# coveord/k8s-spot-rescheduler

Measured on AMD Instinct MI355X. Metric: reference-equivalent pod x spot-node feasibility checks/s (drain-plan latency: drain_plan_latency_ms), higher is better.
Workload: dtype int64

## Files before the change

### k8s-spot-rescheduler_amd/csrc/kernels.hip

```cpp
#include <algorithm>
#include <climits>

#include "kernels.hpp"

#include <hip/hip_ext.h>

namespace sr {
namespace {

__device__ __forceinline__ uint64_t ballot(bool p) { return __builtin_amdgcn_ballot_w64(p); }

__device__ __forceinline__ uint64_t readlane64(uint64_t v, int lane) {
  const uint32_t lo = static_cast<uint32_t>(__builtin_amdgcn_readlane(static_cast<int>(v & 0xffffffffu), lane));
  const uint32_t hi = static_cast<uint32_t>(__builtin_amdgcn_readlane(static_cast<int>(v >> 32), lane));
  return (static_cast<uint64_t>(hi) << 32) | lo;
}

template <int CTRL, int ROW_MASK = 0xf>
__device__ __forceinline__ int dpp_min(int v) {
  return min(v, __builtin_amdgcn_update_dpp(INT_MAX, v, CTRL, ROW_MASK, 0xf, false));
}
__device__ __forceinline__ int wave_min(int v) {
  v = dpp_min<0x111>(v);
  v = dpp_min<0x112>(v);
// ... 77 lines not shown
    if (has) acc &= any | cur;
    if (wv) w.S[static_cast<size_t>(cls) * Wp + word] = acc;
  }
}

__device__ __forceinline__ void k0_common(const DevWorkload& w, int local_first_fallback, int wave, int lane) {
  if (blockIdx.x == 0 && wave == 0 && w.n_node_patch > 0 && lane < 11) {
    for (int p = 0; p < w.n_node_patch; ++p) {
      const uint64_t* pr = w.node_patch + static_cast<size_t>(p) * kNodePatchU64;
      const size_t node = static_cast<size_t>(pr[0]);
      if (lane < 8) const_cast<uint64_t*>(w.node_rec)[node * 8 + lane] = pr[1 + lane];
      else const_cast<int64_t*>(w.node_free)[static_cast<size_t>(lane - 8) * w.n_pad + node] =
          static_cast<int64_t>(pr[1 + lane]);
    }
  }
  for (int i = static_cast<int>(blockIdx.x * blockDim.x + threadIdx.x); i < w.n_pod_patch;
       i += static_cast<int>(gridDim.x * blockDim.x)) {
    const uint64_t* pp = w.pod_patch + static_cast<size_t>(i) * kPodPatchU64;
    uint64_t* rec = const_cast<uint64_t*>(w.pod_rec) + static_cast<size_t>(pp[0]) * 6;
    rec[4] = pp[1];
    rec[5] = pp[2];
  }
  if (blockIdx.x == 0 && threadIdx.x == 0) {
    unsigned long long* dm = reinterpret_cast<unsigned long long*>(w.d_min);
    dm[0] = ~0ull;
    dm[1] = local_first_fallback < 0 ? ~0ull : static_cast<unsigned long long>(local_first_fallback) << 32;
    dm[2] = w.rank_next;
  }
}

__device__ __forceinline__ int64_t free_of(const DevWorkload& w, int d, int n) {
  int64_t v = w.node_free[static_cast<size_t>(d - 1) * w.n_pad + n];
  for (int p = 0; p < w.n_node_patch; ++p) {
    const uint64_t* pr = w.node_patch + static_cast<size_t>(p) * kNodePatchU64;
    if (static_cast<uint64_t>(n) == pr[0]) v = static_cast<int64_t>(pr[8 + d]);
  }
  return v;
}

__global__ __launch_bounds__(256) void k0_tables(DevWorkload w, int s_blocks, int local_first_fallback) {
  const int lane = threadIdx.x & 63;
  const int wave = __builtin_amdgcn_readfirstlane(static_cast<int>(threadIdx.x >> 6));
  const size_t pw = static_cast<size_t>(blockIdx.x) * 4 + wave;
  uint64_t* const prof = w.prof && pw < kK0ProfWaves ? w.prof + static_cast<size_t>(w.n_cand) * 16 + 2 * pw : nullptr;
  if (prof && lane == 0)
    prof[0] = __builtin_amdgcn_s_memrealtime() | (static_cast<int>(blockIdx.x) < s_blocks ? 1ull << 63 : 0ull);
  struct Stamp {
    uint64_t* p;
    int lane;
    __device__ ~Stamp() {
      if (p && lane == 0) p[1] = __builtin_amdgcn_s_memrealtime();
    }
  } stamp{prof, lane};
  k0_common(w, local_first_fallback, wave, lane);
  const size_t Wp = static_cast<size_t>(w.Wp);
  if (static_cast<int>(blockIdx.x) < s_blocks) {
    const int c0 = __builtin_amdgcn_readfirstlane((static_cast<int>(blockIdx.x) * 4 + wave) * kSClasses);
    int op[kSClasses][8];
#pragma unroll
    for (int q = 0; q < kSClasses; ++q) {
      const int cls = c0 + q;
      if (cls < w.n_classes) {
        const int4* p8 = reinterpret_cast<const int4*>(w.cls_prog8 + static_cast<size_t>(cls) * 8);
        const int4 a = p8[0], b = p8[1];
        op[q][0] = a.x; op[q][1] = a.y; op[q][2] = a.z; op[q][3] = a.w;
        op[q][4] = b.x; op[q][5] = b.y; op[q][6] = b.z; op[q][7] = b.w;
      } else {
        op[q][0] = -3;
#pragma unroll
        for (int u = 1; u < 8; ++u) op[q][u] = -1;
      }
    }
    const int s_words = w.s_head_only ? min(w.Wp, kSHead) : w.Wp;
    for (int wb = 0; wb < s_words; wb += 128) {
      const bool two = wb + 64 < s_words;
      uint64_t v[2][kSClasses][8];
#pragma unroll
      for (int h = 0; h < 2; ++h) {
        if (h == 1 && !two) break;
        const int word = wb + 64 * h + lane;
        const size_t wi = word < s_words ? static_cast<size_t>(word) : 0;
#pragma unroll
        for (int q = 0; q < kSClasses; ++q)
#pragma unroll
          for (int u = 0; u < 8; ++u)
            v[h][q][u] = op[q][u] >= 0 ? w.atoms[static_cast<size_t>(op[q][u] >> 2) * Wp + wi] : 0;
      }
#pragma unroll
      for (int h = 0; h < 2; ++h) {
        if (h == 1 && !two) break;
        const int word = wb + 64 * h + lane;
        const bool wv = word < s_words;
#pragma unroll
        for (int q = 0; q < kSClasses; ++q) {
          if (op[q][0] < 0 && op[q][0] != -1) continue;
          const uint64_t acc = eval_prog8(op[q], v[h][q]);
          if (wv) w.S[static_cast<size_t>(c0 + q) * Wp + word] = acc;
        }
      }
    }
#pragma unroll
    for (int q = 0; q < kSClasses; ++q)
      if (op[q][0] == -2) s_row_general(w, c0 + q, lane);
    return;
  }
  int tw = (static_cast<int>(blockIdx.x) - s_blocks) * 4 + wave;
  const int wgroups = (w.Wp + kTWords - 1) / kTWords;
  int d = 0;
  for (; d < 4; ++d) {
    const int waves_d = (w.t_off[d + 1] - w.t_off[d] + 63) / 64 * wgroups;
    if (tw < waves_d) break;
    tw -= waves_d;
  }
  if (d == 4) return;
  const int g = tw / wgroups;
  const int W0 = (tw - g * wgroups) * kTWords;
  const int r0 = w.t_off[d] + 64 * g;
  const int nr = min(64, w.t_off[d + 1] - r0);
  const int64_t thr = lane < nr ? w.t_thr[r0 + lane] : INT64_MAX;
#pragma unroll
  for (int ww = 0; ww < kTWords; ++ww) {
    const int W = W0 + ww;
    if (W >= w.Wp) break;
    uint64_t word;
    if (d == 0) {
      const int nvalid = max(0, min(64, w.n_spot - 64 * W));
      word = nvalid >= 64 ? ~0ull : (1ull << nvalid) - 1;
    } else {
      const uint64_t fv = static_cast<uint64_t>(free_of(w, d, 64 * W + lane));
      uint32_t lo = 0, hi = 0;
#pragma unroll
      for (int i = 0; i < 32; ++i) lo |= static_cast<uint32_t>(static_cast<int64_t>(readlane64(fv, i)) >= thr) << i;
#pragma unroll
      for (int i = 0; i < 32; ++i)
        hi |= static_cast<uint32_t>(static_cast<int64_t>(readlane64(fv, 32 + i)) >= thr) << i;
      word = static_cast<uint64_t>(hi) << 32 | lo;
    }
    if (lane < nr && thr != kTPad) w.T[static_cast<size_t>(r0 + lane) * Wp + W] = word;
  }
}


__global__ __launch_bounds__(256) void k0_incremental(DevWorkload w, int s_waves, int t_waves,
                                                      int local_first_fallback) {
  const int lane = threadIdx.x & 63;
  const int wave = __builtin_amdgcn_readfirstlane(static_cast<int>(threadIdx.x >> 6));
  k0_common(w, local_first_fallback, wave, lane);
  const int wv = static_cast<int>(blockIdx.x) * 4 + wave;
  const size_t Wp = static_cast<size_t>(w.Wp);
  if (wv < s_waves) {
    const int cls = wv * 64 + lane;
    if (cls >= w.n_classes) return;
    const int s_words = w.s_head_only ? min(w.Wp, kSHead) : w.Wp;
    const int4* p8 = reinterpret_cast<const int4*>(w.cls_prog8 + static_cast<size_t>(cls) * 8);
    const int4 a = p8[0], b = p8[1];
    const int op[8] = {a.x, a.y, a.z, a.w, b.x, b.y, b.z, b.w};
    for (int c = 0; c < w.n_k0_cols; ++c) {
      const int W = w.k0_cols[c];
      if (W >= s_words) continue;
      uint64_t acc;
      if (op[0] == -2) {
        acc = ~0ull;
        uint64_t any = 0, cur = 0;
        bool has = false;
        for (int o = w.cls_prog_off[cls]; o < w.cls_prog_off[cls + 1]; ++o) {
          const int x = w.cls_prog[o];
          const uint64_t v = w.atoms[static_cast<size_t>(x >> 2) * Wp + W];
          switch (x & 3) {
            case PROG_AND: acc &= v; break;
            case PROG_ANDNOT: acc &= ~v; break;
            case PROG_TERM_START:
              any |= has ? cur : 0;
              cur = v;
              has = true;
              break;
            default: cur &= v; break;
          }
        }
        if (has) acc &= any | cur;
      } else {
        uint64_t v[8];
#pragma unroll
        for (int u = 0; u < 8; ++u) v[u] = op[u] >= 0 ? w.atoms[static_cast<size_t>(op[u] >> 2) * Wp + W] : 0;
        acc = eval_prog8(op, v);
      }
      w.S[static_cast<size_t>(cls) * Wp + W] = acc;
    }
    return;
  }
  int tw = wv - s_waves;
  if (tw < t_waves) {
    int d = 1;
    for (; d < 4; ++d) {
      const int waves_d = (w.t_off[d + 1] - w.t_off[d] + 63) / 64;
      if (tw < waves_d) break;
      tw -= waves_d;
    }
    if (d == 4) return;
    const int r0 = w.t_off[d] + 64 * tw;
    const int nr = min(64, w.t_off[d + 1] - r0);
    const int64_t thr = lane < nr ? w.t_thr[r0 + lane] : INT64_MAX;
    for (int c = 0; c < w.n_k0_cols; ++c) {
      const int W = w.k0_cols[c];
      const uint64_t fv = static_cast<uint64_t>(free_of(w, d, 64 * W + lane));
      uint32_t lo = 0, hi = 0;
#pragma unroll
      for (int i = 0; i < 32; ++i) lo |= static_cast<uint32_t>(static_cast<int64_t>(readlane64(fv, i)) >= thr) << i;
#pragma unroll
      for (int i = 0; i < 32; ++i)
        hi |= static_cast<uint32_t>(static_cast<int64_t>(readlane64(fv, 32 + i)) >= thr) << i;
      if (lane < nr && thr != kTPad) w.T[static_cast<size_t>(r0 + lane) * Wp + W] = static_cast<uint64_t>(hi) << 32 | lo;
    }
    return;
  }
  const int mr = tw - t_waves;
  if (mr >= w.n_k0_rows) return;
  const int row = w.k0_rows[mr];
  const int d = row < w.t_off[2] ? 1 : row < w.t_off[3] ? 2 : 3;
  const int64_t thr = w.t_thr[row];
  for (int W = lane; W < w.Wp; W += 64) {
    uint64_t word = 0;
    for (int i = 0; i < 64; ++i) word |= static_cast<uint64_t>(free_of(w, d, 64 * W + i) >= thr) << i;
    w.T[static_cast<size_t>(row) * Wp + W] = word;
  }
}


typedef __attribute__((address_space(3))) void* lds_vp;
typedef __attribute__((address_space(1))) void* gbl_vp;
#define SR_WAIT_VM(n) asm volatile("s_waitcnt vmcnt(" #n ")" ::: "memory")

__device__ __forceinline__ void write_winner(const DevWorkload& w) {
  const int lane = threadIdx.x & 63;
  const unsigned long long* dm = reinterpret_cast<const unsigned long long*>(w.d_min);
  const unsigned long long ok = __hip_atomic_load(dm, __ATOMIC_RELAXED, __HIP_MEMORY_SCOPE_AGENT);
  const unsigned long long fb = __hip_atomic_load(dm + 1, __ATOMIC_RELAXED, __HIP_MEMORY_SCOPE_AGENT);
  const unsigned long long nx = __hip_atomic_load(dm + 2, __ATOMIC_RELAXED, __HIP_MEMORY_SCOPE_AGENT);
  uint64_t* r = w.result;
  const bool any = ok != ~0ull;
  const int g = any ? static_cast<int>(ok >> 32) : -1;
  const int li = any ? static_cast<int>(ok & 0xffffffffu) : -1;
  const bool local = any && li < w.n_cand && w.cand_global[li] == g;
  const int off = local ? w.cand_off[li] : 0;
  const int np = local ? w.cand_off[li + 1] - off : 0;
  const uint64_t tag = static_cast<uint64_t>(static_cast<uint32_t>(w.seq)) << 32;
  auto put = [&](int i, int v) {
    __hip_atomic_store(r + i, tag | static_cast<uint32_t>(v), __ATOMIC_RELAXED, __HIP_MEMORY_SCOPE_SYSTEM);
  };
  for (int q = lane; q < np; q += 64)
    put(kResultHeader + q, __hip_atomic_load(w.out_node + off + q, __ATOMIC_RELAXED, __HIP_MEMORY_SCOPE_AGENT));
  if (lane == 0) put(0, g);
  if (lane == 1) put(1, local ? 1 : 0);
  if (lane == 2) put(2, np);
  if (lane == 3) put(3, fb == ~0ull ? -1 : static_cast<int>(fb >> 32));
  if (lane == 4) put(4, nx == ~0ull ? -1 : static_cast<int>(nx));
}

__global__ __launch_bounds__(64) void k3_winner(DevWorkload w) { write_winner(w); }

__global__ __launch_bounds__(256) void k3_sequence(SeqRound r) {
  const unsigned long long ok = __hip_atomic_load(reinterpret_cast<const unsigned long long*>(r.d_min),
                                                  __ATOMIC_RELAXED, __HIP_MEMORY_SCOPE_AGENT);
  const int win = ok == ~0ull ? INT_MAX : static_cast<int>(ok >> 32);
  const int end = win < r.fb_stop ? win : r.fb_stop - 1;
  for (int ci = static_cast<int>(blockIdx.x * blockDim.x + threadIdx.x); ci < r.n_cand;
       ci += static_cast<int>(gridDim.x * blockDim.x)) {
    const int g = r.cand_global[ci];
    if (g <= r.floor || g > end) continue;
    r.seq_status[g] = r.out_status[ci];
    const int o = r.cand_off[ci], np = r.cand_off[ci + 1] - o;
    const int dst = r.in_off[g] - r.in_off[0];
    for (int k = 0; k < np; ++k) r.seq_node[dst + k] = r.out_node[o + k];
  }
}

__device__ __forceinline__ uint64_t swap_pairs(uint64_t x, uint64_t m) {
  const uint64_t y = x & m, e = 0x5555555555555555ull;
  return (x & ~m) | ((y & e) << 1) | ((y >> 1) & e);
}

constexpr int kHead = 32;
constexpr int kRing = 8;
constexpr int kPodWin = 128;
constexpr int kRecU64 = 6;
constexpr int kNodeCache = 16;
constexpr int kMaxPods = 512;

struct K2Lds {
  uint64_t ring[kRing][4 * kHead];
  uint64_t chunk[256];
  uint64_t pods[kPodWin][kRecU64];
  uint64_t cache[kNodeCache][8];
  uint64_t spec[8];
  uint64_t rec[8];
  int32_t omap[kMaxPods];
};

constexpr int kMapG = 4;

struct K2Stats {
  uint32_t n_spec_miss = 0, n_min = 0, n_far = 0;
  uint64_t cyc_a = 0, cyc_b = 0, cyc_c = 0, cyc_d = 0;
  uint64_t cyc_rec = 0;
  uint32_t narrow = 0;
  uint64_t cyc_res = 0;
  uint64_t cyc_win = 0;
  uint32_t cyc_a_ld = 0, cyc_res_ld = 0, n_res = 0, n_res_pods = 0;
};

template <int SPL, int CH, bool PROF, bool EXT = false>
__device__ __forceinline__ int k2_run(const DevWorkload& w, K2Lds& L, const int p0, const int np, int& status,
                                      K2Stats& st, uint32_t& nbytes, const int ebase = -1) {
  const int lane = threadIdx.x & 63;
  const int Wp = w.Wp;
  const uint64_t* __restrict__ tab = w.S;

  auto dma = [&](const uint64_t* src, uint64_t* dst) {
    __builtin_amdgcn_global_load_lds((gbl_vp)src, (lds_vp)dst, 16, 0, 0);
  };
  auto dma_rows = [&](uint64_t* dst, uint64_t r01, uint64_t r23, int base) {
    const uint32_t wi = static_cast<uint32_t>(min(base + 2 * (lane & 31), Wp - 2));
    const uint32_t ra = lane < 32 ? static_cast<uint32_t>(r01) : static_cast<uint32_t>(r01 >> 32);
    const uint32_t rb = lane < 32 ? static_cast<uint32_t>(r23) : static_cast<uint32_t>(r23 >> 32);
    dma(tab + (static_cast<uint64_t>(ra) + wi), dst);
    dma(tab + (static_cast<uint64_t>(rb) + wi), dst + 128);
  };
  auto dma_rows_of = [&](uint64_t* dst, int q, int base) {
    const uint64_t* pr = L.pods[q & (kPodWin - 1)];
    dma_rows(dst, pr[4], pr[5], base);
  };
  auto dma_head = [&](uint64_t* dst, uint64_t r01, uint64_t r23) {
    const int r = lane >> 4;
    const uint32_t wi = static_cast<uint32_t>(min(2 * (lane & 15), Wp - 2));
    const uint64_t rr = r < 2 ? r01 : r23;
    const uint32_t off = (r & 1) ? static_cast<uint32_t>(rr >> 32) : static_cast<uint32_t>(rr);
    dma(tab + (static_cast<uint64_t>(off) + wi), dst);
  };
  auto dma_head_of = [&](uint64_t* dst, int q) {
    const uint64_t* pr = L.pods[q & (kPodWin - 1)];
    dma_head(dst, pr[4], pr[5]);
  };
  auto dma_rec = [&](uint64_t* dst, int node) {
    if (lane < 4) dma(w.node_rec + static_cast<size_t>(node == INT_MAX ? 0 : node) * 8 + 2 * lane, dst);
  };
  auto dma_pods = [&](int m) {
    const uint64_t* src = w.pod_rec + static_cast<size_t>(p0 + 64 * m) * kRecU64 + 2 * lane;
    uint64_t* dst = L.pods[64 * (m & 1)];
#pragma unroll
    for (int j = 0; j < 3; ++j) dma(src + 128 * j, dst + 128 * j);
  };

  uint64_t touched[CH];
#pragma unroll
  for (int ch = 0; ch < CH; ++ch) touched[ch] = 0;
  int snode[SPL];
  int64_t scpu[SPL], smem[SPL], seph[SPL];
  int sleft[SPL];
  uint64_t sport[SPL];
  int64_t ss0[SPL], ss1[SPL];
#pragma unroll
  for (int s = 0; s < SPL; ++s) {
    snode[s] = INT_MAX;
    scpu[s] = smem[s] = seph[s] = 0;
    sleft[s] = 0;
    sport[s] = 0;
    ss0[s] = ss1[s] = 0;
  }
  const uint64_t erow = EXT ? w.pod_ext[static_cast<size_t>(ebase) * kDevExtU64 + 7] : ~0ull;
  const int erow0 = static_cast<int32_t>(static_cast<uint32_t>(erow)), erow1 = static_cast<int32_t>(erow >> 32);
  int nslots = 0;
  uint64_t cyc_t = 0;
  auto cyc = [&]() -> uint64_t { return PROF ? __builtin_amdgcn_s_memtime() : 0ull; };
  const uint64_t lane_mask = lane < min(Wp, kHead) ? ~0ull : 0ull;

  uint64_t word_next = 0;
  int cnode0 = INT_MAX;
  int64_t nrc = 0, nrm = 0, nre = 0;
  uint64_t npm = 0;
  int64_t nac = 0, nam = 0, nae = 0, nsr0 = INT64_MIN, nsr1 = INT64_MIN, nsa0 = 0, nsa1 = 0;
  bool sbit[SPL];
  auto gather_next = [&](int kn) {
    if (EXT) {
      const uint64_t* er = w.pod_ext + static_cast<size_t>(ebase + kn) * kDevExtU64;
      nac = static_cast<int64_t>(er[0]);
      nam = static_cast<int64_t>(er[1]);
      nae = static_cast<int64_t>(er[2]);
      nsr0 = static_cast<int64_t>(er[3]);
      nsr1 = static_cast<int64_t>(er[4]);
      nsa0 = static_cast<int64_t>(er[5]);
      nsa1 = static_cast<int64_t>(er[6]);
    }
    const uint64_t* img = L.ring[kn & (kRing - 1)];
    const uint64_t* pr = L.pods[kn & (kPodWin - 1)];
    uint64_t sw[SPL];
#pragma unroll
    for (int s = 0; s < SPL; ++s) sw[s] = img[snode[s] < 64 * kHead ? snode[s] >> 6 : 0];
    const int hl = lane & (kHead - 1);
    const uint64_t a = img[hl] & img[kHead + hl] & img[2 * kHead + hl] & img[3 * kHead + hl];
    nrc = static_cast<int64_t>(pr[0]);
    nrm = static_cast<int64_t>(pr[1]);
    nre = static_cast<int64_t>(pr[2]);
    npm = pr[3];
#pragma unroll
    for (int s = 0; s < SPL; ++s) sbit[s] = (sw[s] >> (snode[s] & 63)) & 1ull;
    word_next = a & lane_mask;
    const uint64_t clean0 = word_next & ~touched[0];
    const uint64_t mc0 = ballot(clean0 != 0);
    cnode0 = INT_MAX;
    if (mc0) {
      const int L0 = __builtin_ctzll(mc0);
      cnode0 = L0 * 64 + __builtin_ctzll(readlane64(clean0, L0));
    }
  };

  static_assert(kRing == 8, "the vmcnt immediates below assume an 8-deep ring");
  dma(w.node_rec + 2 * lane, L.cache[0]);
  dma_pods(0);
  if (np > 64) dma_pods(1);
  nbytes += 64u * kNodeCache + (48u + 4u) * static_cast<uint32_t>(np) + 4u;
  SR_WAIT_VM(0);
#pragma unroll
  for (int j = 0; j < kRing - 1; ++j) dma_head_of(L.ring[j], min(j, np - 1));
  SR_WAIT_VM(6);
  gather_next(0);
  dma_rec(L.spec, cnode0);
  dma_head_of(L.ring[kRing - 1], min(kRing - 1, np - 1));

  status = -1;
  int k = 0;
  for (; k < np; ++k) {
    if (PROF) cyc_t = cyc();
    nbytes += 4u * kHead * 8u + 64u + (EXT ? 64u : 0u);
    const int64_t rc = nrc, rm = nrm, re = nre;
    const int64_t ac = EXT ? nac : rc, am = EXT ? nam : rm, ae = EXT ? nae : re;
    const int64_t sr0 = nsr0, sr1 = nsr1, sa0 = nsa0, sa1 = nsa1;
    const uint64_t pm = npm;
    const uint64_t pin = swap_pairs(pm, w.swap_mask);
    const bool zero = (rc | rm | re) == 0;
    int ans;
    {
      const int hi = min(cnode0, 64 * kHead);
      int best = INT_MAX;
#pragma unroll
      for (int s = 0; s < SPL; ++s) {
        const int nd = snode[s];
        const bool fit = (zero | ((rc <= scpu[s]) & (rm <= smem[s]) & (re <= seph[s]))) &
                         (!EXT | ((sr0 <= ss0[s]) & (sr1 <= ss1[s])));
        const bool ok = (nd < hi) & sbit[s] & (sleft[s] >= 1) & ((sport[s] & pin) == 0) & fit;
        best = ok ? min(best, nd) : best;
      }
      const uint64_t hb = ballot(best != INT_MAX);
      int dnode = INT_MAX;
      if (hb) {
        dnode = (hb & (hb - 1)) ? wave_min(best) : __builtin_amdgcn_readlane(best, __builtin_ctzll(hb));
        if (PROF && (hb & (hb - 1))) ++st.n_min;
      }
      ans = min(cnode0, dnode);
    }
    if (ans == INT_MAX && Wp > kHead) {
#pragma unroll
      for (int ch = 0; ch < CH; ++ch) {
        const int base = ch * 64;
        if (ans != INT_MAX || base >= Wp) continue;
        if (PROF) ++st.n_far;
        nbytes += 4u * 64u * 8u;
        dma_rows_of(L.chunk, k, base);
        SR_WAIT_VM(0);
        const uint64_t* img = L.chunk;
        const uint64_t clean = (img[lane] & img[64 + lane] & img[128 + lane] & img[192 + lane]) &
                               ((base + lane < Wp) ? ~touched[ch] : 0ull);
        const uint64_t mc = ballot(clean != 0);
        int cnode = INT_MAX;
        if (mc) {
          const int L0 = __builtin_ctzll(mc);
          cnode = (base + L0) * 64 + __builtin_ctzll(readlane64(clean, L0));
        }
        const int lo = base * 64;
        const int hi = min(cnode, lo + 64 * 64);
        int best = INT_MAX;
#pragma unroll
        for (int s = 0; s < SPL; ++s) {
          const int nd = snode[s];
          const bool in = (nd >= lo) & (nd < hi);
          const uint64_t sw = img[in ? (nd >> 6) - base : 0];
          const bool fit = (zero | ((rc <= scpu[s]) & (rm <= smem[s]) & (re <= seph[s]))) &
                           (!EXT | ((sr0 <= ss0[s]) & (sr1 <= ss1[s])));
          const bool ok =
              in & (((sw >> (nd & 63)) & 1ull) != 0) & (sleft[s] >= 1) & ((sport[s] & pin) == 0) & fit;
          best = ok ? min(best, nd) : best;
        }
        ans = min(cnode, wave_min(best));
      }
    }
    if (PROF) {
      const uint64_t t = cyc();
      st.cyc_a += t - cyc_t;
      cyc_t = t;
    }
    if (ans == INT_MAX) {
      status = k;
      break;
    }
    if (lane == 0) L.omap[k] = ans;

    bool hit = false;
#pragma unroll
    for (int s = 0; s < SPL; ++s) {
      if (snode[s] == ans) {
        scpu[s] -= ac;
        smem[s] -= am;
        seph[s] -= ae;
        sleft[s] -= 1;
        sport[s] |= pm;
        if (EXT) {
          ss0[s] -= sa0;
          ss1[s] -= sa1;
        }
        hit = true;
      }
    }
    if (!(ballot(hit) != 0)) {
      const int ns = nslots++;
      if (ns >= 64 * SPL) {
        SR_WAIT_VM(0);
        return -1;
      }
      const int64_t b0 = EXT && erow0 >= 0 ? w.node_scal[static_cast<size_t>(erow0) * w.n_pad + ans] : 0;
      const int64_t b1 = EXT && erow1 >= 0 ? w.node_scal[static_cast<size_t>(erow1) * w.n_pad + ans] : 0;
      const uint64_t* rec;
      if (ans < kNodeCache) {
        rec = L.cache[ans];
      } else if (ans == cnode0) {
        SR_WAIT_VM(1);
        rec = L.spec;
      } else {
        if (PROF) ++st.n_spec_miss;
        nbytes += 64u;
        dma_rec(L.rec, ans);
        SR_WAIT_VM(0);
        rec = L.rec;
      }
      const int64_t fc = static_cast<int64_t>(rec[0]), fm = static_cast<int64_t>(rec[1]),
                    fe = static_cast<int64_t>(rec[2]);
      const uint64_t pb = rec[3];
      const int pl = static_cast<int>(static_cast<int64_t>(rec[4]));
#pragma unroll
      for (int s = 0; s < SPL; ++s) {
        if ((s == (ns >> 6)) & (lane == (ns & 63))) {
          snode[s] = ans;
          scpu[s] = fc - ac;
          smem[s] = fm - am;
          seph[s] = fe - ae;
          sleft[s] = pl - 1;
          sport[s] = pb | pm;
          if (EXT) {
            ss0[s] = b0 - sa0;
            ss1[s] = b1 - sa1;
          }
        }
      }
      const int tw = ans >> 6;
#pragma unroll
      for (int ch = 0; ch < CH; ++ch)
        if (tw == ch * 64 + lane) touched[ch] |= 1ull << (ans & 63);
    }
    if (PROF) {
      const uint64_t t = cyc();
      st.cyc_b += t - cyc_t;
      cyc_t = t;
    }
    if (k + 1 < np) {
      const int q = min(k + kRing, np - 1);
      const bool restage = q == k + kRing && (q & 63) == 0 && q >= kPodWin;
      if (restage) {
        dma_pods(q >> 6);
        SR_WAIT_VM(0);
      } else if (k >= 5) {
        SR_WAIT_VM(12);
      } else {
        SR_WAIT_VM(7);
      }
      if (PROF) {
        const uint64_t t = cyc();
        st.cyc_c += t - cyc_t;
        cyc_t = t;
      }
      const uint64_t* pq = L.pods[q & (kPodWin - 1)];
      const uint64_t r01 = pq[4], r23 = pq[5];
      gather_next(k + 1);
      dma_rec(L.spec, cnode0);
      dma_head(L.ring[k & (kRing - 1)], r01, r23);
      if (PROF) st.cyc_d += cyc() - cyc_t;
    }
  }
  SR_WAIT_VM(0);
  return status >= 0 ? status : np;
}

constexpr int kNH = 8;
static_assert(kNH == 2 || kNH == 4 || kNH == 8, "head words per pod: a power of two up to 8 (8-bit head masks)");
constexpr int kNHS = kNH + 1;
constexpr int kFar = 64 * kNH;

__device__ __forceinline__ uint64_t f_word_far(const uint64_t* __restrict__ tab, uint64_t r01, uint64_t r23, int wd) {
  return tab[static_cast<uint32_t>(r01) + wd] & tab[static_cast<uint32_t>(r01 >> 32) + wd] &
         tab[static_cast<uint32_t>(r23) + wd] & tab[static_cast<uint32_t>(r23 >> 32) + wd];
}

__device__ __forceinline__ uint64_t f_word_prog_s(const DevWorkload& w, const int32_t* pg, int wd) {
  int op[8];
  uint64_t v[8];
#pragma unroll
  for (int u = 0; u < 8; ++u) op[u] = pg[u];
#pragma unroll
  for (int u = 0; u < 8; ++u) v[u] = op[u] >= 0 ? w.atoms[static_cast<size_t>(op[u] >> 2) * w.Wp + wd] : 0ull;
  return eval_prog8(op, v);
}

__device__ __forceinline__ uint64_t f_word_prog(const DevWorkload& w, const uint64_t* __restrict__ tab,
                                                const int32_t* pg, uint64_t r01, uint64_t r23, int wd) {
  int op[8];
  uint64_t v[8];
#pragma unroll
  for (int u = 0; u < 8; ++u) op[u] = pg[u];
#pragma unroll
  for (int u = 0; u < 8; ++u) v[u] = op[u] >= 0 ? w.atoms[static_cast<size_t>(op[u] >> 2) * w.Wp + wd] : 0ull;
  return eval_prog8(op, v) & tab[static_cast<uint32_t>(r01 >> 32) + wd] & tab[static_cast<uint32_t>(r23) + wd] &
         tab[static_cast<uint32_t>(r23 >> 32) + wd];
}

__device__ __forceinline__ uint64_t fix_dirty(const DevWorkload& w, uint64_t f, uint64_t s, int wd, int64_t rc,
                                              int64_t rm, int64_t re, bool zero) {
  for (int p = 0; p < w.n_dirty; ++p) {
    const int n = w.dirty_node[p];
    if ((n >> 6) != wd) continue;
    const uint64_t bit = 1ull << (n & 63);
    const bool fits = zero || (w.dirty_free[p][0] >= rc && w.dirty_free[p][1] >= rm && w.dirty_free[p][2] >= re);
    f = fits ? (f | (s & bit)) : (f & ~bit);
  }
  return f;
}

__device__ __forceinline__ void window_patch(const DevWorkload& w, int W, int lane, int64_t& ncpu, int64_t& nmem,
                                             int64_t& neph, uint64_t& nport, int& nleft) {
  for (int p = 0; p < w.n_node_patch; ++p) {
    const uint64_t* pr = w.node_patch + static_cast<size_t>(p) * kNodePatchU64;
    if (static_cast<int>(pr[0]) != 64 * W + lane) continue;
    ncpu = static_cast<int64_t>(pr[1]);
    nmem = static_cast<int64_t>(pr[2]);
    neph = static_cast<int64_t>(pr[3]);
    nport = pr[4];
    nleft = static_cast<int>(static_cast<int64_t>(pr[5]));
  }
}

__device__ __forceinline__ uint32_t from_lane(uint32_t v, int src) {
  return static_cast<uint32_t>(__builtin_amdgcn_ds_bpermute(src << 2, static_cast<int>(v)));
}

#pragma clang diagnostic push
#pragma clang diagnostic ignored "-Winline-asm"
__device__ __forceinline__ int writelane(int v, int x, int k) {
  asm("s_mov_b32 m0, %2\n\tv_writelane_b32 %0, %1, m0" : "+v"(v) : "s"(x), "s"(k) : "m0");
  return v;
}
#pragma clang diagnostic pop
__device__ __forceinline__ int ff1(uint64_t x) {
  int r;
  asm("s_ff1_i32_b64 %0, %1" : "=s"(r) : "s"(x));
  return r;
}
__device__ __forceinline__ uint64_t bitclear(uint64_t x, int k) {
  asm("s_bitset0_b64 %0, %1" : "+s"(x) : "s"(k));
  return x;
}

template <bool E, bool O>
__device__ __forceinline__ uint64_t place_window(uint64_t todo, int kmax, int W, int lane, int64_t rc, int64_t rm,
                                                 int64_t re, uint64_t pm, uint64_t cur, uint64_t zm,
                                                 uint64_t swap_mask, uint64_t emask, int64_t& ncpu, int64_t& nmem,
                                                 int64_t& neph, uint64_t& nport, int& nleft, int& node) {
  int jv = 64;
  if (kmax < 64) todo &= kmax <= 0 ? 0ull : (1ull << kmax) - 1;
  while (todo != 0) {
    const int k = __builtin_ctzll(todo);
    todo = bitclear(todo, k);
    const int64_t c = static_cast<int64_t>(readlane64(static_cast<uint64_t>(rc), k));
    const int64_t m = static_cast<int64_t>(readlane64(static_cast<uint64_t>(rm), k));
    const int64_t e = E ? static_cast<int64_t>(readlane64(static_cast<uint64_t>(re), k)) : 0;
    const uint64_t q = O ? readlane64(pm, k) : 0ull;
    uint64_t fit = readlane64(cur, k) & ballot(nleft >= 1);
    const uint64_t res = ballot(ncpu >= c) & ballot(nmem >= m) & (E ? ballot(neph >= e) : emask);
    fit &= ((zm >> k) & 1) ? ~0ull : res;
    if (O) fit &= ballot((nport & q) == 0);
    if (O) {
      if (fit != 0) {
        const int j = __builtin_ctzll(fit);
        if (lane == j) {
          ncpu -= c;
          nmem -= m;
          if (E) neph -= e;
          nleft -= 1;
          nport |= swap_pairs(q, swap_mask);
        }
        jv = writelane(jv, j, k);
      }
      continue;
    }
    const int j = ff1(fit);
    const bool hit = lane == j;
    ncpu -= hit ? c : 0;
    nmem -= hit ? m : 0;
    if (E) neph -= hit ? e : 0;
    nleft -= hit ? 1 : 0;
    jv = writelane(jv, j, k);
  }
  const bool took = static_cast<unsigned>(jv) < 64u;
  node = took ? 64 * W + jv : node;
  return ballot(took);
}

template <typename T>
struct XVals {
  T ac, am, ae, r0, r1, a0, a1;
};

template <bool E, bool O>
__device__ __forceinline__ uint64_t place_window_x(uint64_t todo, int kmax, int W, int lane, int64_t rc, int64_t rm,
                                                   int64_t re, const XVals<int64_t>& x, uint64_t pm, uint64_t cur,
                                                   uint64_t zm, uint64_t swap_mask, uint64_t emask, int64_t& ncpu,
                                                   int64_t& nmem, int64_t& neph, uint64_t& nport, int& nleft,
                                                   int64_t& ns0, int64_t& ns1, int& node) {
  int jv = 64;
  if (kmax < 64) todo &= kmax <= 0 ? 0ull : (1ull << kmax) - 1;
  while (todo != 0) {
    const int k = __builtin_ctzll(todo);
    todo = bitclear(todo, k);
    const int64_t c = static_cast<int64_t>(readlane64(static_cast<uint64_t>(rc), k));
    const int64_t m = static_cast<int64_t>(readlane64(static_cast<uint64_t>(rm), k));
    const int64_t e = E ? static_cast<int64_t>(readlane64(static_cast<uint64_t>(re), k)) : 0;
    const int64_t r0 = static_cast<int64_t>(readlane64(static_cast<uint64_t>(x.r0), k));
    const int64_t r1 = static_cast<int64_t>(readlane64(static_cast<uint64_t>(x.r1), k));
    const uint64_t q = O ? readlane64(pm, k) : 0ull;
    uint64_t fit = readlane64(cur, k) & ballot(nleft >= 1) & ballot(ns0 >= r0) & ballot(ns1 >= r1);
    const uint64_t res = ballot(ncpu >= c) & ballot(nmem >= m) & (E ? ballot(neph >= e) : emask);
    fit &= ((zm >> k) & 1) ? ~0ull : res;
    if (O) fit &= ballot((nport & q) == 0);
    if (fit != 0) {
      const int j = __builtin_ctzll(fit);
      const int64_t ac = static_cast<int64_t>(readlane64(static_cast<uint64_t>(x.ac), k));
      const int64_t am = static_cast<int64_t>(readlane64(static_cast<uint64_t>(x.am), k));
      const int64_t ae = static_cast<int64_t>(readlane64(static_cast<uint64_t>(x.ae), k));
      const int64_t a0 = static_cast<int64_t>(readlane64(static_cast<uint64_t>(x.a0), k));
      const int64_t a1 = static_cast<int64_t>(readlane64(static_cast<uint64_t>(x.a1), k));
      if (lane == j) {
        ncpu -= ac;
        nmem -= am;
        neph -= ae;
        nleft -= 1;
        ns0 -= a0;
        ns1 -= a1;
        if (O) nport |= swap_pairs(q, swap_mask);
      }
      jv = writelane(jv, j, k);
    }
  }
  const bool took = static_cast<unsigned>(jv) < 64u;
  node = took ? 64 * W + jv : node;
  return ballot(took);
}

__device__ __forceinline__ int32_t scale32(int64_t f, int k) {
  const int64_t q = f >> k;
  return f < 0 ? -1 : (q > 0x7fffffffll ? 0x7fffffff : static_cast<int32_t>(q));
}

template <bool E, bool O>
__device__ __forceinline__ uint64_t fits32(int32_t c32, int32_t m32, int32_t e32, int nleft, uint64_t conflict,
                                           int32_t c, int32_t m, int32_t e) {
  int32_t t = __builtin_elementwise_sub_sat(c32, c) | __builtin_elementwise_sub_sat(m32, m) | (nleft - 1);
  if (E) t |= __builtin_elementwise_sub_sat(e32, e);
  if (O) {
    const uint32_t x = static_cast<uint32_t>(conflict) | static_cast<uint32_t>(conflict >> 32);
    t |= static_cast<int32_t>(x | (0u - x));
  }
  return ballot(t >= 0);
}

template <bool E, bool O, bool X = false>
__device__ __forceinline__ uint64_t place_window32(uint64_t todo, int kmax, int W, int lane, uint32_t nc, uint32_t nm,
                                                   uint32_t ne, uint64_t pm, uint64_t ps, uint64_t cur,
                                                   int32_t& c32, int32_t& m32, int32_t& e32,
                                                   uint64_t& nport, int& nleft, int& node) {
  if constexpr (X) {
    int jv = 64;
    if (kmax < 64) todo &= kmax <= 0 ? 0ull : (1ull << kmax) - 1;
    const uint64_t base = ballot(nleft >= 1);
    uint64_t taken = 0;
    while (todo != 0) {
      const int k = __builtin_ctzll(todo);
      todo = bitclear(todo, k);
      const int32_t c = __builtin_amdgcn_readlane(static_cast<int>(nc), k);
      const int32_t m = __builtin_amdgcn_readlane(static_cast<int>(nm), k);
      const int32_t e = E ? __builtin_amdgcn_readlane(static_cast<int>(ne), k) : 0;
      const uint64_t q = readlane64(pm, k);
      uint64_t fit = readlane64(cur, k) & base & ~taken & fits32<E, true>(c32, m32, e32, 1, nport & q, c, m, e);
      const int j = fit != 0 ? __builtin_ctzll(fit) : 64;
      taken |= fit & (0ull - fit);
      jv = writelane(jv, j, k);
    }
    const int dst = jv < 64 ? jv : (taken == ~0ull ? lane : __builtin_ctzll(~taken));
    const bool snd = jv < 64;
    auto send = [&](uint32_t v) {
      return static_cast<uint32_t>(__builtin_amdgcn_ds_permute(dst << 2, static_cast<int>(snd ? v : 0u)));
    };
    const uint32_t rc = send(static_cast<uint32_t>(max(static_cast<int32_t>(nc), 0)));
    const uint32_t rm = send(static_cast<uint32_t>(max(static_cast<int32_t>(nm), 0)));
    const uint32_t re = E ? send(static_cast<uint32_t>(max(static_cast<int32_t>(ne), 0))) : 0u;
    const uint32_t rs_lo = send(static_cast<uint32_t>(ps)), rs_hi = send(static_cast<uint32_t>(ps >> 32));
    const bool got = (taken >> lane) & 1;
    c32 -= got ? static_cast<int32_t>(rc) : 0;
    m32 -= got ? static_cast<int32_t>(rm) : 0;
    if (E) e32 -= got ? static_cast<int32_t>(re) : 0;
    nleft -= got ? 1 : 0;
    nport |= got ? (static_cast<uint64_t>(rs_hi) << 32 | rs_lo) : 0ull;
    node = jv < 64 ? 64 * W + jv : node;
    return ballot(jv < 64);
  }
  int jv = 64;
  if (kmax < 64) todo &= kmax <= 0 ? 0ull : (1ull << kmax) - 1;
  while (todo != 0) {
    const int k = __builtin_ctzll(todo);
    todo = bitclear(todo, k);
    const int32_t c = __builtin_amdgcn_readlane(static_cast<int>(nc), k);
    const int32_t m = __builtin_amdgcn_readlane(static_cast<int>(nm), k);
    const int32_t e = E ? __builtin_amdgcn_readlane(static_cast<int>(ne), k) : 0;
    const uint64_t q = O ? readlane64(pm, k) : 0ull;
    uint64_t fit = readlane64(cur, k) & fits32<E, O>(c32, m32, e32, nleft, nport & q, c, m, e);
    const int32_t cu = max(c, 0), mu = max(m, 0), eu = max(e, 0);
    if (O) {
      if (fit != 0) {
        const int j = __builtin_ctzll(fit);
        if (lane == j) {
          c32 -= cu;
          m32 -= mu;
          if (E) e32 -= eu;
          nleft -= 1;
          nport |= readlane64(ps, k);
        }
        jv = writelane(jv, j, k);
      }
      continue;
    }
    const int j = ff1(fit);
    const bool hit = lane == j;
    c32 -= hit ? cu : 0;
    m32 -= hit ? mu : 0;
    if (E) e32 -= hit ? eu : 0;
    nleft -= hit ? 1 : 0;
    jv = writelane(jv, j, k);
  }
  const bool took = static_cast<unsigned>(jv) < 64u;
  node = took ? 64 * W + jv : node;
  return ballot(took);
}

template <bool E, bool O>
__device__ __forceinline__ uint64_t place_window32_x(uint64_t todo, int kmax, int W, int lane, uint32_t nc, uint32_t nm,
                                                     uint32_t ne, const XVals<uint32_t>& x, uint64_t pm, uint64_t ps,
                                                     uint64_t cur, int32_t& c32, int32_t& m32, int32_t& e32,
                                                     int32_t& s0, int32_t& s1, uint64_t& nport, int& nleft,
                                                     int& node) {
  int jv = 64;
  if (kmax < 64) todo &= kmax <= 0 ? 0ull : (1ull << kmax) - 1;
  while (todo != 0) {
    const int k = __builtin_ctzll(todo);
    todo = bitclear(todo, k);
    const int32_t c = __builtin_amdgcn_readlane(static_cast<int>(nc), k);
    const int32_t m = __builtin_amdgcn_readlane(static_cast<int>(nm), k);
    const int32_t e = E ? __builtin_amdgcn_readlane(static_cast<int>(ne), k) : 0;
    const int32_t r0 = __builtin_amdgcn_readlane(static_cast<int>(x.r0), k);
    const int32_t r1 = __builtin_amdgcn_readlane(static_cast<int>(x.r1), k);
    const uint64_t q = O ? readlane64(pm, k) : 0ull;
    int32_t t = __builtin_elementwise_sub_sat(c32, c) | __builtin_elementwise_sub_sat(m32, m) | (nleft - 1) |
                __builtin_elementwise_sub_sat(s0, r0) | __builtin_elementwise_sub_sat(s1, r1);
    if (E) t |= __builtin_elementwise_sub_sat(e32, e);
    if (O) {
      const uint64_t cf = nport & q;
      const uint32_t u = static_cast<uint32_t>(cf) | static_cast<uint32_t>(cf >> 32);
      t |= static_cast<int32_t>(u | (0u - u));
    }
    const uint64_t fit = readlane64(cur, k) & ballot(t >= 0);
    if (fit != 0) {
      const int j = __builtin_ctzll(fit);
      const int32_t ac = __builtin_amdgcn_readlane(static_cast<int>(x.ac), k);
      const int32_t am = __builtin_amdgcn_readlane(static_cast<int>(x.am), k);
      const int32_t ae = __builtin_amdgcn_readlane(static_cast<int>(x.ae), k);
      const int32_t a0 = __builtin_amdgcn_readlane(static_cast<int>(x.a0), k);
      const int32_t a1 = __builtin_amdgcn_readlane(static_cast<int>(x.a1), k);
      if (lane == j) {
        c32 -= ac;
        m32 -= am;
        e32 -= ae;
        s0 -= a0;
        s1 -= a1;
        nleft -= 1;
        if (O) nport |= readlane64(ps, k);
      }
      jv = writelane(jv, j, k);
    }
  }
  const bool took = static_cast<unsigned>(jv) < 64u;
  node = took ? 64 * W + jv : node;
  return ballot(took);
}

struct Narrow {
  int kc, km, ke;
};

constexpr int kCoopWaves = 4;
constexpr int kCoopPods = 64;
struct CoopArea {
  int32_t cmd, n, sw, pad;
  uint64_t r01[kCoopPods], r23[kCoopPods];
  int64_t rq[kCoopPods][3];
  int32_t op[kCoopPods][8];
  uint32_t best[kCoopPods];
  uint32_t rk[kCoopWaves][kCoopPods];
  uint64_t rm[kCoopWaves][kCoopPods];
  uint64_t rf[kCoopWaves][kCoopPods];
};

template <bool HO>
__device__ __forceinline__ void coop_scan(const DevWorkload& w, CoopArea& A, int h) {
  const int lane = threadIdx.x & 63;
  const int n = __builtin_amdgcn_readfirstlane(A.n), sw = __builtin_amdgcn_readfirstlane(A.sw);
  const int Wp = w.Wp;
  const uint64_t* __restrict__ tab = w.S;
  if (lane < n) A.rk[h][lane] = 0xffffffffu;
  const int cb0 = (sw >> 6) << 6;
  const int nch = (Wp - cb0 + 63) >> 6;
  const uint64_t all = n >= 64 ? ~0ull : (1ull << n) - 1;
  uint64_t found = 0;
  constexpr int Q = HO ? 2 : 4;
  for (int k = h; k < nch; k += kCoopWaves) {
    const int cb = cb0 + 64 * k;
    const int word = cb + lane;
    const bool wv = word >= sw && word < Wp;
    const uint32_t wi = wv ? static_cast<uint32_t>(word) : 0u;
    const uint64_t vw = ballot(wv);
    uint64_t open = all & ~found & ballot(lane < n && __hip_atomic_load(&A.best[lane], __ATOMIC_RELAXED,
                                                                           __HIP_MEMORY_SCOPE_WORKGROUP) >
                                                        static_cast<uint32_t>(k));
    while (open != 0) {
      int js[Q];
      uint64_t a01[Q], a23[Q];
      int op[Q][8];
#pragma unroll
      for (int q = 0; q < Q; ++q) {
        js[q] = open != 0 ? __builtin_ctzll(open) : -1;
        open &= open - 1;
        const int j = js[q] < 0 ? 0 : js[q];
        a01[q] = readlane64(A.r01[j], 0);
        a23[q] = readlane64(A.r23[j], 0);
        if constexpr (HO) {
#pragma unroll
          for (int u = 0; u < 8; ++u) op[q][u] = __builtin_amdgcn_readfirstlane(A.op[j][u]);
        }
      }
      uint64_t x[Q][HO ? 11 : 4];
#pragma unroll
      for (int q = 0; q < Q; ++q) {
        if (js[q] < 0) continue;
        if constexpr (HO) {
#pragma unroll
          for (int u = 0; u < 8; ++u)
            x[q][u] = op[q][u] >= 0 ? w.atoms[static_cast<size_t>(op[q][u] >> 2) * Wp + wi] : 0ull;
          x[q][8] = tab[static_cast<uint32_t>(a01[q] >> 32) + wi];
          x[q][9] = tab[static_cast<uint32_t>(a23[q]) + wi];
          x[q][10] = tab[static_cast<uint32_t>(a23[q] >> 32) + wi];
        } else {
          x[q][0] = tab[static_cast<uint32_t>(a01[q]) + wi];
          x[q][1] = tab[static_cast<uint32_t>(a01[q] >> 32) + wi];
          x[q][2] = tab[static_cast<uint32_t>(a23[q]) + wi];
          x[q][3] = tab[static_cast<uint32_t>(a23[q] >> 32) + wi];
        }
      }
#pragma unroll
      for (int q = 0; q < Q; ++q) {
        if (js[q] < 0) continue;
        const int j = js[q];
        uint64_t f, sw0;
        if constexpr (HO) {
          uint64_t v8[8];
#pragma unroll
          for (int u = 0; u < 8; ++u) v8[u] = x[q][u];
          sw0 = eval_prog8(op[q], v8);
          f = sw0 & x[q][8] & x[q][9] & x[q][10];
        } else {
          sw0 = x[q][0];
          f = x[q][0] & x[q][1] & x[q][2] & x[q][3];
        }
        if (w.k0_skip) {
          const int64_t rc = A.rq[j][0], rm = A.rq[j][1], re = A.rq[j][2];
          f = fix_dirty(w, f, sw0, word, rc, rm, re, (rc | rm | re) == 0);
        }
        const uint64_t m = ballot(wv && f != 0) & vw;
        if (m == 0) continue;
        found |= 1ull << j;
        if (lane == 0) {
          A.rk[h][j] = static_cast<uint32_t>(k);
          A.rm[h][j] = m;
          atomicMin(&A.best[j], static_cast<uint32_t>(k));
        }
        const uint64_t fw = readlane64(f, __builtin_ctzll(m));
        if (lane == 0) A.rf[h][j] = fw;
      }
    }
  }
}

__device__ __forceinline__ void coop_helper(const DevWorkload& w, CoopArea& A, int h) {
  for (;;) {
    __syncthreads();
    if (__hip_atomic_load(&A.cmd, __ATOMIC_RELAXED, __HIP_MEMORY_SCOPE_WORKGROUP) != 0) break;
    if (w.s_head_only) coop_scan<true>(w, A, h);
    else coop_scan<false>(w, A, h);
    __syncthreads();
  }
}

__device__ __forceinline__ int wave_sum(int v) {
  v += __builtin_amdgcn_update_dpp(0, v, 0x111, 0xf, 0xf, false);
  v += __builtin_amdgcn_update_dpp(0, v, 0x112, 0xf, 0xf, false);
  v += __builtin_amdgcn_update_dpp(0, v, 0x114, 0xf, 0xf, false);
  v += __builtin_amdgcn_update_dpp(0, v, 0x118, 0xf, 0xf, false);
  v += __builtin_amdgcn_update_dpp(0, v, 0x142, 0xa, 0xf, false);
  v += __builtin_amdgcn_update_dpp(0, v, 0x143, 0xc, 0xf, false);
  return __builtin_amdgcn_readlane(v, 63);
}

template <int G, bool PROF, bool WIDE = false, bool XT = false, bool COOP = false>
__device__ __forceinline__ void k2_node_order(const DevWorkload& w, uint64_t* __restrict__ F, const int p0,
                                              const int np, int& status, K2Stats& st, uint32_t& nbytes,
                                              int (&mapv)[kMapG], const int ebase = -1, const int erow0_in = -2,
                                              const int erow1_in = -2, CoopArea* A = nullptr) {
  static_assert(64 * G * kNHS * 8 <= sizeof(K2Lds), "node-order LDS exceeds the wave's K2 region");
  static_assert(G <= kMapG, "a mapping register per pod group");
  const int lane = threadIdx.x & 63;
  const int Wp = w.Wp;
  const uint64_t* __restrict__ tab = w.S;
  int64_t rc[G], rm[G], re[G];
  uint64_t pm[G], ps[G], r01[G], r23[G], fmask[G], act[G];
  int fbase[G];
  bool unres[G];
  uint64_t cur[G];
  uint32_t hmask[G];
  bool zero[G];
  int ptr[G], node[G];
  int dead = np;
#pragma unroll
  for (int g = 0; g < G; ++g) {
    const uint64_t* pr = w.pod_rec + static_cast<size_t>(p0 + min(64 * g + lane, np - 1)) * kRecU64;
    rc[g] = static_cast<int64_t>(pr[0]);
    rm[g] = static_cast<int64_t>(pr[1]);
    re[g] = static_cast<int64_t>(pr[2]);
    pm[g] = swap_pairs(pr[3], w.swap_mask);
    ps[g] = pr[3];
    r01[g] = pr[4];
    r23[g] = pr[5];
    zero[g] = (rc[g] | rm[g] | re[g]) == 0;
    fmask[g] = 0;
    fbase[g] = 0;
    unres[g] = false;
    hmask[g] = 0;
    cur[g] = 0;
    ptr[g] = INT_MAX;
    node[g] = -1;
    const uint64_t e = ballot(64 * g + lane < np && static_cast<uint32_t>(r01[g]) == w.s_empty_off);
    if (e != 0) dead = min(dead, 64 * g + __builtin_ctzll(e));
  }
  XVals<int64_t> xv[G];
  int erow0 = -1, erow1 = -1;
  if constexpr (XT) {
#pragma unroll
    for (int g = 0; g < G; ++g) {
      const uint64_t* er = w.pod_ext + static_cast<size_t>(ebase + min(64 * g + lane, np - 1)) * kDevExtU64;
      xv[g] = {static_cast<int64_t>(er[0]), static_cast<int64_t>(er[1]), static_cast<int64_t>(er[2]),
               static_cast<int64_t>(er[3]), static_cast<int64_t>(er[4]), static_cast<int64_t>(er[5]),
               static_cast<int64_t>(er[6])};
    }
    if (erow0_in == -2) {
      const uint64_t erow = w.pod_ext[static_cast<size_t>(ebase) * kDevExtU64 + 7];
      erow0 = __builtin_amdgcn_readfirstlane(static_cast<int32_t>(static_cast<uint32_t>(erow)));
      erow1 = __builtin_amdgcn_readfirstlane(static_cast<int32_t>(erow >> 32));
    } else {
      erow0 = erow0_in;
      erow1 = erow1_in;
    }
    nbytes += 64u * static_cast<uint32_t>(np);
  }
  Narrow nk;
  bool narrow;
  uint32_t nc[G], nm[G], ne[G];
  XVals<uint32_t> nx[G];
  {
    auto tz = [](int64_t v) { return v == 0 ? 64 : __builtin_ctzll(static_cast<uint64_t>(v)); };
    int mc = 64, mm = 64, me = 64;
#pragma unroll
    for (int g = 0; g < G; ++g) {
      mc = min(mc, tz(rc[g]));
      mm = min(mm, tz(rm[g]));
      me = min(me, tz(re[g]));
      if (XT && 64 * g + lane < np) {
        mc = min(mc, tz(xv[g].ac));
        mm = min(mm, tz(xv[g].am));
        me = min(me, tz(xv[g].ae));
      }
    }
    nk.kc = min(wave_min(mc), 62);
    nk.km = min(wave_min(mm), 62);
    nk.ke = min(wave_min(me), 62);
    bool ok = true;
#pragma unroll
    for (int g = 0; g < G; ++g) {
      const uint64_t a = static_cast<uint64_t>(rc[g]) >> nk.kc, b = static_cast<uint64_t>(rm[g]) >> nk.km,
                     c = static_cast<uint64_t>(re[g]) >> nk.ke;
      ok = ok && (a | b | c) < (1ull << 23);
      nc[g] = zero[g] ? 0x80000000u : static_cast<uint32_t>(a);
      nm[g] = zero[g] ? 0x80000000u : static_cast<uint32_t>(b);
      ne[g] = zero[g] ? 0x80000000u : static_cast<uint32_t>(c);
      if constexpr (XT) {
        const XVals<int64_t>& v = xv[g];
        const uint64_t lim = 1ull << 23;
        const bool in = 64 * g + lane < np;
        ok = ok && (!in || ((v.ac | v.am | v.ae | v.a0 | v.a1) >= 0 &&
                            ((static_cast<uint64_t>(v.ac) >> nk.kc) | (static_cast<uint64_t>(v.am) >> nk.km) |
                             (static_cast<uint64_t>(v.ae) >> nk.ke) | static_cast<uint64_t>(v.a0) |
                             static_cast<uint64_t>(v.a1)) < lim &&
                            (v.r0 == INT64_MIN || (v.r0 >= 0 && v.r0 < static_cast<int64_t>(lim))) &&
                            (v.r1 == INT64_MIN || (v.r1 >= 0 && v.r1 < static_cast<int64_t>(lim))) &&
                            (!zero[g] || (v.ac | v.am | v.ae) == 0)));
        nx[g] = {static_cast<uint32_t>(static_cast<uint64_t>(v.ac) >> nk.kc),
                 static_cast<uint32_t>(static_cast<uint64_t>(v.am) >> nk.km),
                 static_cast<uint32_t>(static_cast<uint64_t>(v.ae) >> nk.ke),
                 v.r0 == INT64_MIN ? 0x80000000u : static_cast<uint32_t>(v.r0),
                 v.r1 == INT64_MIN ? 0x80000000u : static_cast<uint32_t>(v.r1), static_cast<uint32_t>(v.a0),
                 static_cast<uint32_t>(v.a1)};
      }
    }
    narrow = w.k2_narrow && ballot(!ok) == 0;
  }
  bool E, O;
  {
    uint64_t e = 0, o = 0;
#pragma unroll
    for (int g = 0; g < G; ++g) {
      e |= ballot(64 * g + lane < np && (re[g] != 0 || (XT && xv[g].ae != 0)));
      o |= ballot(64 * g + lane < np && pm[g] != 0);
    }
    E = e != 0;
    O = o != 0;
  }
  bool X = false;
  if (O && !XT) {
    const uint64_t m0 = readlane64(ps[0] & pm[0], 0);
    for (uint64_t bits = m0; bits != 0 && !X; bits &= bits - 1) {
      const int b = __builtin_ctzll(bits);
      bool all = true;
#pragma unroll
      for (int g = 0; g < G; ++g) all = all && ballot(64 * g + lane < np && !(((ps[g] & pm[g]) >> b) & 1)) == 0;
      X = all && w.k2_excl;
    }
  }
  int wcur = -1;
  int64_t ncpu = 0, nmem = 0, neph = 0;
  uint64_t nport = 0;
  int nleft = 0;
  int64_t ns0 = 0, ns1 = 0;
  auto load_scal = [&](int W) {
    if constexpr (XT) {
      const size_t n = static_cast<size_t>(64 * W + lane);
      ns0 = erow0 >= 0 ? w.node_scal[static_cast<size_t>(erow0) * w.n_pad + n] : 0;
      ns1 = erow1 >= 0 ? w.node_scal[static_cast<size_t>(erow1) * w.n_pad + n] : 0;
      nbytes += 64u * 16u;
    }
  };
  if (dead > 0) {
    const uint64_t* nr = w.node_rec + static_cast<size_t>(lane) * 8;
    ncpu = static_cast<int64_t>(nr[0]);
    nmem = static_cast<int64_t>(nr[1]);
    neph = static_cast<int64_t>(nr[2]);
    nport = nr[3];
    nleft = static_cast<int>(static_cast<int64_t>(nr[4]));
    if (w.k0_skip) window_patch(w, 0, lane, ncpu, nmem, neph, nport, nleft);
    load_scal(0);
    wcur = 0;
    nbytes += 64u * 40u;
  }
  if (PROF) {
    asm volatile("s_waitcnt vmcnt(0)" ::: "memory");
    st.cyc_rec = __builtin_amdgcn_s_memtime();
  }
  int32_t* PG = reinterpret_cast<int32_t*>(F + 64 * G * kNHS);
  if (w.s_head_only && dead > 0) {
#pragma unroll
    for (int g = 0; g < G; ++g) {
      if (64 * g >= dead) break;
      const uint32_t cls = static_cast<uint32_t>(r01[g]) / static_cast<uint32_t>(Wp);
      const int4* p8 = reinterpret_cast<const int4*>(w.cls_prog8 + static_cast<size_t>(cls) * 8);
      const int4 a = p8[0], b = p8[1];
      int4* dst = reinterpret_cast<int4*>(PG + (64 * g + lane) * 8);
      dst[0] = a;
      dst[1] = b;
    }
    nbytes += 32u * static_cast<uint32_t>(min(np, 64 * ((dead + 63) / 64)));
  }
  uint64_t cyc_t = PROF ? __builtin_amdgcn_s_memtime() : 0;
  nbytes += (48u + 4u) * static_cast<uint32_t>(np) + 4u + 32u * static_cast<uint32_t>(min(Wp, kNH)) * dead;

  uint32_t dirty_head = 0;
  uint32_t dfit[G];
  for (int p = 0; p < w.n_dirty; ++p) {
    const int wd0 = w.dirty_node[p] >> 6;
    dirty_head |= wd0 < kNH ? 1u << wd0 : 0u;
  }
#pragma unroll
  for (int g = 0; g < G; ++g) {
    dfit[g] = 0;
    if (dirty_head != 0)
      for (int p = 0; p < w.n_dirty; ++p) {
        const bool fits = zero[g] || (w.dirty_free[p][0] >= rc[g] && w.dirty_free[p][1] >= rm[g] &&
                                      w.dirty_free[p][2] >= re[g]);
        dfit[g] |= fits ? 1u << p : 0u;
      }
  }
  {
    constexpr int kPW = 64 / kNH;
    constexpr int kPB = (G == 1 || WIDE ? 64 : 32) / kPW;
    const int sub = lane / kNH, wd = lane % kNH;
    const bool wv = wd < Wp;
#pragma unroll
    for (int g = 0; g < G; ++g) {
      const int lim = min(dead, 64 * g + 64);
      for (int b0 = 64 * g; b0 < lim; b0 += kPW * kPB) {
        uint64_t x[kPB][4];
        int kk[kPB];
        uint32_t fm[kPB];
        const uint64_t cyc_ld0 = PROF ? __builtin_amdgcn_s_memtime() : 0;
#pragma unroll
        for (int h = 0; h < kPB; ++h) {
          kk[h] = b0 + kPW * h + sub;
          x[h][0] = x[h][1] = x[h][2] = x[h][3] = 0;
          fm[h] = 0;
          if (b0 + kPW * h >= lim) continue;
          const int src = min(kk[h], np - 1) - 64 * g;
          if (dirty_head != 0) fm[h] = from_lane(dfit[g], src);
          const uint32_t o0 = from_lane(static_cast<uint32_t>(r01[g]), src);
          const uint32_t o1 = from_lane(static_cast<uint32_t>(r01[g] >> 32), src);
          const uint32_t o2 = from_lane(static_cast<uint32_t>(r23[g]), src);
          const uint32_t o3 = from_lane(static_cast<uint32_t>(r23[g] >> 32), src);
          const uint32_t wi = wv ? wd : 0u;
          x[h][0] = tab[o0 + wi];
          x[h][1] = tab[o1 + wi];
          x[h][2] = tab[o2 + wi];
          x[h][3] = tab[o3 + wi];
        }
        if (PROF) {
          asm volatile("s_waitcnt vmcnt(0)" ::: "memory");
          st.cyc_a_ld += static_cast<uint32_t>(__builtin_amdgcn_s_memtime() - cyc_ld0);
        }
#pragma unroll
        for (int h = 0; h < kPB; ++h) {
          if (b0 + kPW * h >= lim) continue;
          uint64_t f = (wv && kk[h] < np) ? x[h][0] & x[h][1] & x[h][2] & x[h][3] : 0ull;
          if (dirty_head != 0) {
            for (int p = 0; p < w.n_dirty; ++p) {
              const int n = w.dirty_node[p];
              if ((n >> 6) != wd) continue;
              const uint64_t bit = 1ull << (n & 63);
              f = (fm[h] >> p) & 1 ? (f | (x[h][0] & bit)) : (f & ~bit);
            }
            f = (wv && kk[h] < np) ? f : 0ull;
          }
          if (kk[h] < np) F[kk[h] * kNHS + wd] = f;
          const uint64_t m = ballot(f != 0);
          const int rel = 64 * g + lane - (b0 + kPW * h);
          if (rel >= 0 && rel < kPW) hmask[g] = static_cast<uint32_t>(m >> (kNH * rel)) & ((1u << kNH) - 1u);
        }
      }
    }
  }

  uint64_t any = 0;
#pragma unroll
  for (int g = 0; g < G; ++g) {
    const int k = 64 * g + lane;
    if (k < dead) {
      if (hmask[g] != 0) {
        const int w0 = __builtin_ctz(hmask[g]);
        cur[g] = F[k * kNHS + w0];
        ptr[g] = w0 * 64 + __builtin_ctzll(cur[g]);
      } else {
        ptr[g] = Wp > kNH ? kFar : INT_MAX;
        unres[g] = Wp > kNH;
      }
    }
    const uint64_t gone = ballot(k < dead && ptr[g] == INT_MAX);
    if (gone != 0) dead = min(dead, 64 * g + __builtin_ctzll(gone));
  }
  uint64_t zm[G];
#pragma unroll
  for (int g = 0; g < G; ++g) {
    act[g] = ballot(64 * g + lane < dead);
    any |= act[g];
    zm[g] = ballot(zero[g]);
  }
  if (PROF) {
    const uint64_t t = __builtin_amdgcn_s_memtime();
    st.cyc_a += t - cyc_t;
    cyc_t = t;
  }

  int visits = 0, placements = 0, windows = wcur + 1;
  while (any != 0) {
    int mine = INT_MAX;
#pragma unroll
    for (int g = 0; g < G; ++g) mine = ((act[g] >> lane) & 1) ? min(mine, ptr[g]) : mine;
    const int n = wave_min(mine);
    if (n == INT_MAX) break;
    uint64_t unres_n = 0;
    if (n == kFar || (n & 4095) == 0) {
#pragma unroll
      for (int g = 0; g < G; ++g) {
        const uint64_t u = ballot(((act[g] >> lane) & 1) && ptr[g] == n && unres[g]);
        unres_n |= u;
        if (PROF) st.n_res_pods += static_cast<uint32_t>(__builtin_popcountll(u));
      }
    }
    if (unres_n != 0) {
      const uint64_t cyc_r0 = PROF ? __builtin_amdgcn_s_memtime() : 0;
      if (PROF) st.n_res += 1;
      const int sw = n >> 6;
      auto resolve = [&](auto qc, auto ho) {
        constexpr int Q = decltype(qc)::value;
        constexpr bool HO = decltype(ho)::value;
#pragma unroll
        for (int g = 0; g < G; ++g) {
          uint64_t pend = ballot(((act[g] >> lane) & 1) && ptr[g] == n && unres[g]);
          while (pend != 0) {
            int js[Q];
            uint64_t a01[Q], a23[Q];
            int64_t qr[Q][3];
            int op[Q][8];
            uint32_t nops[Q];
#pragma unroll
            for (int q = 0; q < Q; ++q) {
              js[q] = pend != 0 ? __builtin_ctzll(pend) : -1;
              pend &= pend - 1;
              const int j = js[q] < 0 ? 0 : js[q];
              a01[q] = readlane64(r01[g], j);
              a23[q] = readlane64(r23[g], j);
              qr[q][0] = static_cast<int64_t>(readlane64(static_cast<uint64_t>(rc[g]), j));
              qr[q][1] = static_cast<int64_t>(readlane64(static_cast<uint64_t>(rm[g]), j));
              qr[q][2] = static_cast<int64_t>(readlane64(static_cast<uint64_t>(re[g]), j));
              nops[q] = 0;
              if constexpr (HO) {
#pragma unroll
                for (int u = 0; u < 8; ++u) {
                  op[q][u] = __builtin_amdgcn_readfirstlane(PG[(64 * g + j) * 8 + u]);
                  nops[q] += op[q][u] >= 0 ? 1u : 0u;
                }
              }
            }
            int todo = 0;
#pragma unroll
            for (int q = 0; q < Q; ++q) todo |= js[q] >= 0 ? 1 << q : 0;
            for (int cb = (sw >> 6) << 6; todo != 0 && cb < Wp; cb += 64) {
              const int word = cb + lane;
              const bool wv = word >= sw && word < Wp;
              const uint32_t wi = wv ? static_cast<uint32_t>(word) : 0u;
              if (PROF) st.cyc_res += 1ull << 40;
              uint64_t x[Q][HO ? 11 : 4];
              const uint64_t cyc_ld0 = PROF ? __builtin_amdgcn_s_memtime() : 0;
#pragma unroll
              for (int q = 0; q < Q; ++q) {
                if (!((todo >> q) & 1)) continue;
                if constexpr (HO) {
#pragma unroll
                  for (int u = 0; u < 8; ++u)
                    x[q][u] = op[q][u] >= 0 ? w.atoms[static_cast<size_t>(op[q][u] >> 2) * Wp + wi] : 0ull;
                  x[q][8] = tab[static_cast<uint32_t>(a01[q] >> 32) + wi];
                  x[q][9] = tab[static_cast<uint32_t>(a23[q]) + wi];
                  x[q][10] = tab[static_cast<uint32_t>(a23[q] >> 32) + wi];
                } else {
                  x[q][0] = tab[static_cast<uint32_t>(a01[q]) + wi];
                  x[q][1] = tab[static_cast<uint32_t>(a01[q] >> 32) + wi];
                  x[q][2] = tab[static_cast<uint32_t>(a23[q]) + wi];
                  x[q][3] = tab[static_cast<uint32_t>(a23[q] >> 32) + wi];
                }
              }
              if (PROF) {
                asm volatile("s_waitcnt vmcnt(0)" ::: "memory");
                st.cyc_res_ld += static_cast<uint32_t>(__builtin_amdgcn_s_memtime() - cyc_ld0);
              }
              const uint64_t vw = ballot(wv);
#pragma unroll
              for (int q = 0; q < Q; ++q) {
                if (!((todo >> q) & 1)) continue;
                uint64_t f, sw0;
                if constexpr (HO) {
                  uint64_t v8[8];
#pragma unroll
                  for (int u = 0; u < 8; ++u) v8[u] = x[q][u];
                  sw0 = eval_prog8(op[q], v8);
                  f = sw0 & x[q][8] & x[q][9] & x[q][10];
                } else {
                  sw0 = x[q][0];
                  f = x[q][0] & x[q][1] & x[q][2] & x[q][3];
                }
                if (w.k0_skip)
                  f = fix_dirty(w, f, sw0, word, qr[q][0], qr[q][1], qr[q][2], (qr[q][0] | qr[q][1] | qr[q][2]) == 0);
                f = wv ? f : 0ull;
                const uint64_t m = ballot(f != 0);
                const int upto = m != 0 ? __builtin_ctzll(m) : 63;
                const uint64_t need = upto == 63 ? vw : vw & ((2ull << upto) - 1);
                nbytes += (HO ? 8u * (nops[q] + 3u) : 32u) * static_cast<uint32_t>(__builtin_popcountll(need));
                if (m == 0 && cb + 64 < Wp) continue;
                todo &= ~(1 << q);
                int nx = INT_MAX;
                uint64_t fw = 0;
                if (m != 0) {
                  const int w2 = __builtin_ctzll(m);
                  fw = readlane64(f, w2);
                  nx = (cb + w2) * 64 + __builtin_ctzll(fw);
                }
                if (lane == js[q]) {
                  fmask[g] = m;
                  fbase[g] = cb;
                  ptr[g] = nx;
                  cur[g] = fw;
                  unres[g] = false;
                }
                if (nx == INT_MAX) dead = min(dead, 64 * g + js[q]);
                if (PROF && nx == INT_MAX) st.cyc_res += 1ull << 56;
              }
            }
          }
        }
      };
      auto coop_resolve = [&]() {
#pragma unroll
        for (int g = 0; g < G; ++g) {
          const uint64_t pend = ballot(((act[g] >> lane) & 1) && ptr[g] == n && unres[g]);
          if (pend == 0) continue;
          const bool mine = (pend >> lane) & 1;
          const int slot = __builtin_popcountll(pend & ((1ull << lane) - 1));
          int nops = 0;
          if (mine) {
            A->r01[slot] = r01[g];
            A->r23[slot] = r23[g];
            A->rq[slot][0] = rc[g];
            A->rq[slot][1] = rm[g];
            A->rq[slot][2] = re[g];
            if (w.s_head_only)
#pragma unroll
              for (int u = 0; u < 8; ++u) {
                const int o = PG[(64 * g + lane) * 8 + u];
                A->op[slot][u] = o;
                nops += o >= 0 ? 1 : 0;
              }
            A->best[slot] = 0xffffffffu;
          }
          if (lane == 0) {
            A->cmd = 0;
            A->n = __builtin_popcountll(pend);
            A->sw = sw;
          }
          __syncthreads();
          if (w.s_head_only) coop_scan<true>(w, *A, 0);
          else coop_scan<false>(w, *A, 0);
          __syncthreads();
          if (PROF) st.cyc_res += static_cast<uint64_t>((Wp - ((sw >> 6) << 6) + 64 * kCoopWaves - 1) /
                                                        (64 * kCoopWaves)) << 40;
          uint32_t bytes = 0;
          if (mine) {
            uint32_t kb = 0xffffffffu;
            int hb = 0;
#pragma unroll
            for (int h = 0; h < kCoopWaves; ++h) {
              const uint32_t k = A->rk[h][slot];
              hb = k < kb ? h : hb;
              kb = k < kb ? k : kb;
            }
            int nx = INT_MAX, words = Wp - sw;
            if (kb != 0xffffffffu) {
              const uint64_t m = A->rm[hb][slot], fw = A->rf[hb][slot];
              const int cb = ((sw >> 6) << 6) + 64 * static_cast<int>(kb);
              const int w2 = __builtin_ctzll(m);
              nx = (cb + w2) * 64 + __builtin_ctzll(fw);
              fmask[g] = m;
              fbase[g] = cb;
              cur[g] = fw;
              words = cb + w2 + 1 - sw;
            } else {
              fmask[g] = 0;
              cur[g] = 0;
            }
            ptr[g] = nx;
            unres[g] = false;
            bytes = static_cast<uint32_t>(words) * (w.s_head_only ? 8u * (static_cast<uint32_t>(nops) + 3u) : 32u);
          }
          nbytes += static_cast<uint32_t>(wave_sum(static_cast<int>(bytes)));
          const uint64_t gone = ballot(mine && ptr[g] == INT_MAX);
          if (gone != 0) dead = min(dead, 64 * g + __builtin_ctzll(gone));
          if (PROF) st.cyc_res += static_cast<uint64_t>(__builtin_popcountll(gone)) << 56;
        }
      };
      constexpr int kResQ = 4;
      if constexpr (COOP) coop_resolve();
      else if (w.s_head_only) resolve(std::integral_constant<int, 2>{}, std::true_type{});
      else resolve(std::integral_constant<int, kResQ>{}, std::false_type{});
      if (PROF) st.cyc_res += __builtin_amdgcn_s_memtime() - cyc_r0;
      any = 0;
#pragma unroll
      for (int g = 0; g < G; ++g) {
        act[g] &= ballot(64 * g + lane < dead);
        any |= act[g];
      }
      continue;
    }
    ++visits;
    const int W = n >> 6;
    if (W != wcur) {
      const uint64_t cyc_w0 = PROF ? __builtin_amdgcn_s_memtime() : 0;
      const uint64_t* nr = w.node_rec + static_cast<size_t>(W * 64 + lane) * 8;
      ncpu = static_cast<int64_t>(nr[0]);
      nmem = static_cast<int64_t>(nr[1]);
      neph = static_cast<int64_t>(nr[2]);
      nport = nr[3];
      nleft = static_cast<int>(static_cast<int64_t>(nr[4]));
      if (w.k0_skip) window_patch(w, W, lane, ncpu, nmem, neph, nport, nleft);
      load_scal(W);
      wcur = W;
      ++windows;
      nbytes += 64u * 40u;
      if (PROF) {
        asm volatile("s_waitcnt vmcnt(0)" ::: "memory");
        st.cyc_win += __builtin_amdgcn_s_memtime() - cyc_w0;
      }
    }
    if (PROF) {
      const uint64_t t = __builtin_amdgcn_s_memtime();
      st.cyc_b += t - cyc_t;
      cyc_t = t;
    }
    uint64_t failed[G];
    {
      const uint64_t emask = E ? 0ull : ballot(neph >= 0);
      int32_t c32 = 0, m32 = 0, e32 = 0, s032 = 0, s132 = 0;
      st.narrow = narrow;
      if (narrow) {
        c32 = E || neph >= 0 ? scale32(ncpu, nk.kc) : INT_MIN;
        m32 = scale32(nmem, nk.km);
        e32 = scale32(neph, nk.ke);
        if (XT) {
          s032 = scale32(ns0, 0);
          s132 = scale32(ns1, 0);
        }
      }
#pragma unroll
      for (int g = 0; g < G; ++g) {
        const uint64_t cand = ballot(((act[g] >> lane) & 1) && (ptr[g] >> 6) == W);
        const uint64_t todo = 64 * g < dead ? cand : 0ull;
        uint64_t placed = 0;
        if (todo != 0) {
          const int kmax = dead - 64 * g;
#define SR_PW(e_, o_)                                                                                             \
  place_window<e_, o_>(todo, kmax, W, lane, rc[g], rm[g], re[g], pm[g], cur[g], zm[g], w.swap_mask, emask, ncpu, \
                       nmem, neph, nport, nleft, node[g])
#define SR_PW32(e_, o_)                                                                                           \
  place_window32<e_, o_>(todo, kmax, W, lane, nc[g], nm[g], ne[g], pm[g], ps[g], cur[g], c32, m32, e32, \
                         nport, nleft, node[g])
#define SR_PW32X(e_)                                                                                            \
  place_window32<e_, true, true>(todo, kmax, W, lane, nc[g], nm[g], ne[g], pm[g], ps[g], cur[g], c32, m32, e32, \
                                 nport, nleft, node[g])
#define SR_PWX(e_, o_)                                                                                          \
  place_window_x<e_, o_>(todo, kmax, W, lane, rc[g], rm[g], re[g], xv[g], pm[g], cur[g], zm[g], w.swap_mask, emask, \
                         ncpu, nmem, neph, nport, nleft, ns0, ns1, node[g])
#define SR_PW32XT(e_, o_)                                                                                       \
  place_window32_x<e_, o_>(todo, kmax, W, lane, nc[g], nm[g], ne[g], nx[g], pm[g], ps[g], cur[g], c32, m32, e32, \
                           s032, s132, nport, nleft, node[g])
          if (XT && narrow)
            placed = E ? (O ? SR_PW32XT(true, true) : SR_PW32XT(true, false))
                       : (O ? SR_PW32XT(false, true) : SR_PW32XT(false, false));
          else if (XT)
            placed = E ? (O ? SR_PWX(true, true) : SR_PWX(true, false)) : (O ? SR_PWX(false, true) : SR_PWX(false, false));
          else if (narrow && X)
            placed = E ? SR_PW32X(true) : SR_PW32X(false);
          else if (narrow)
            placed = E ? (O ? SR_PW32(true, true) : SR_PW32(true, false))
                       : (O ? SR_PW32(false, true) : SR_PW32(false, false));
          else
            placed = E ? (O ? SR_PW(true, true) : SR_PW(true, false)) : (O ? SR_PW(false, true) : SR_PW(false, false));
#undef SR_PW
#undef SR_PW32
#undef SR_PW32X
#undef SR_PWX
#undef SR_PW32XT
        }
        placements += __builtin_popcountll(placed);
        act[g] &= ~placed;
        failed[g] = cand & ~placed;
      }
    }
    if (PROF) {
      const uint64_t t = __builtin_amdgcn_s_memtime();
      st.cyc_c += t - cyc_t;
      cyc_t = t;
    }
#pragma unroll
    for (int g = 0; g < G; ++g) {
      if (failed[g] == 0) continue;
      const int k = 64 * g + lane;
      bool far_word = false;
      if ((failed[g] >> lane) & 1) {
        int nx = INT_MAX;
        if (W < kNH) {
          const uint32_t rem = hmask[g] & (0xffu << (W + 1)) & 0xffu;
          if (rem != 0) {
            const int w2 = __builtin_ctz(rem);
            cur[g] = F[k * kNHS + w2];
            nx = w2 * 64 + __builtin_ctzll(cur[g]);
          } else if (Wp > kNH) {
            nx = kFar;
            unres[g] = true;
          }
        } else {
          const int lw = W - fbase[g];
          const uint64_t rem = lw >= 63 ? 0ull : fmask[g] & (~0ull << (lw + 1));
          if (rem != 0) {
            const int w2 = fbase[g] + __builtin_ctzll(rem);
            cur[g] = w.s_head_only ? f_word_prog(w, tab, PG + (64 * g + lane) * 8, r01[g], r23[g], w2)
                                   : f_word_far(tab, r01[g], r23[g], w2);
            if (w.k0_skip) {
              const uint64_t sw0 = w.s_head_only ? f_word_prog_s(w, PG + (64 * g + lane) * 8, w2)
                                                 : tab[static_cast<uint32_t>(r01[g]) + w2];
              cur[g] = fix_dirty(w, cur[g], sw0, w2, rc[g], rm[g], re[g], zero[g]);
            }
            nx = w2 * 64 + __builtin_ctzll(cur[g]);
            far_word = true;
          } else if (fbase[g] + 64 < Wp) {
            nx = (fbase[g] + 64) * 64;
            unres[g] = true;
          }
        }
        ptr[g] = nx;
      }
      nbytes += 32u * static_cast<uint32_t>(__builtin_popcountll(ballot(far_word)));
      const uint64_t gone = ballot((((failed[g] >> lane) & 1) != 0) & (ptr[g] == INT_MAX));
      if (gone != 0) dead = min(dead, 64 * g + __builtin_ctzll(gone));
    }
    any = 0;
#pragma unroll
    for (int g = 0; g < G; ++g) {
      act[g] &= ballot(64 * g + lane < dead);
      any |= act[g];
    }
    if (PROF) {
      const uint64_t t = __builtin_amdgcn_s_memtime();
      st.cyc_d += t - cyc_t;
      cyc_t = t;
    }
  }
  if (PROF) {
    st.n_min = static_cast<uint32_t>(visits);
    st.n_far = static_cast<uint32_t>(windows);
    st.n_spec_miss = static_cast<uint32_t>(placements);
  }
  status = dead < np ? dead : -1;
#pragma unroll
  for (int g = 0; g < G; ++g) {
    const int k = 64 * g + lane;
    mapv[g] = k < dead ? node[g] : -1;
    if (k < np) w.out_node[p0 + k] = mapv[g];
  }
}

__device__ __forceinline__ uint64_t wave_or(uint64_t v) {
  v |= dpp_shifted<0x111>(v);
  v |= dpp_shifted<0x112>(v);
  v |= dpp_shifted<0x114>(v);
  v |= dpp_shifted<0x118>(v);
  v |= dpp_shifted<0x142, 0xa>(v);
  v |= dpp_shifted<0x143, 0xc>(v);
  return readlane64(v, 63);
}

__device__ __forceinline__ int dk_row_of(const DevWorkload& w, int k) {
  return k == 0 ? w.dk_row[0] : k == 1 ? w.dk_row[1] : k == 2 ? w.dk_row[2] : w.dk_row[3];
}

static_assert(64 * 32 * 8 <= sizeof(K2Lds), "domain path: touched bitmap of 2048 words in the wave's LDS");
template <int CH, int G, bool PROF>
__device__ __forceinline__ void k2_domain(const DevWorkload& w, uint64_t* __restrict__ tl, const int p0,
                                          const int np, const int dbase, int& status, uint32_t& nbytes,
                                          K2Stats& st, const int ebase = -1) {
  static_assert(kDevDomKeys == 4 && kDevDynTerms == 4, "the selects below unroll 4 key slots / terms");
  static_assert(G >= 1 && G <= kDevDynG, "pod groups of the domain-path record");
  const int lane = threadIdx.x & 63;
  const int Wp = w.Wp;
  const uint64_t* __restrict__ tab = w.S;
  const uint64_t* __restrict__ at = w.atoms;
  int snode[G], sleft[G], nslots = 0;
  int64_t scpu[G], smem[G], seph[G];
  uint64_t sport[G];
  int64_t ss0[G], ss1[G];
  const bool ext = ebase >= 0;
  const uint64_t erow = ext ? w.pod_ext[static_cast<size_t>(ebase) * kDevExtU64 + 7] : ~0ull;
  const int erow0 = static_cast<int32_t>(static_cast<uint32_t>(erow)), erow1 = static_cast<int32_t>(erow >> 32);
  int pnode[G];
  int pdom[G][kDevDomKeys];
#pragma unroll
  for (int g = 0; g < G; ++g) {
    snode[g] = INT_MAX;
    sleft[g] = 0;
    scpu[g] = smem[g] = seph[g] = 0;
    sport[g] = 0;
    ss0[g] = ss1[g] = 0;
    pnode[g] = -1;
#pragma unroll
    for (int kk = 0; kk < kDevDomKeys; ++kk) pdom[g][kk] = -1;
  }
  for (int i = lane; i < 64 * CH; i += 64) tl[i] = 0;
  nbytes += (48u + 8u * kDevDynU64 + 4u) * static_cast<uint32_t>(np) + 4u;
  status = -1;
  int k = 0;
  static_assert(kDevDynU64 <= 64 && kRecU64 <= 8 && kDevExtU64 <= 8, "record lanes of the domain path");
  auto records = [&](int q) -> uint64_t {
    if (q >= np) return 0ull;
    if (lane < kDevDynU64) return w.dyn_pod[static_cast<size_t>(dbase + q) * kDevDynU64 + lane];
    return 0ull;
  };
  auto records_pod = [&](int q) -> uint64_t {
    if (q >= np) return 0ull;
    if (lane < kRecU64) return w.pod_rec[static_cast<size_t>(p0 + q) * kRecU64 + lane];
    if (ext && lane >= 8 && lane < 8 + kDevExtU64)
      return w.pod_ext[static_cast<size_t>(ebase + q) * kDevExtU64 + (lane - 8)];
    return 0ull;
  };
  if (ext) nbytes += 8u * kDevExtU64 * static_cast<uint32_t>(np);
  uint64_t rv = records(0), rvp = records_pod(0);
  uint64_t cyc_t = PROF ? __builtin_amdgcn_s_memtime() : 0;
  auto stamp = [&](uint64_t& acc) {
    if (PROF) {
      const uint64_t t = __builtin_amdgcn_s_memtime();
      acc += t - cyc_t;
      cyc_t = t;
    }
  };
  for (; k < np; ++k) {
    const uint64_t cur = rv, curp = rvp;
    rv = records(k + 1);
    rvp = records_pod(k + 1);
    auto D = [&](int i) { return readlane64(cur, i); };
    auto PR = [&](int i) { return readlane64(curp, i); };
    const int64_t rc = static_cast<int64_t>(PR(0)), rm = static_cast<int64_t>(PR(1)), re = static_cast<int64_t>(PR(2));
    const uint64_t pm = PR(3), r01 = PR(4), r23 = PR(5);
    const uint64_t pin = swap_pairs(pm, w.swap_mask);
    const bool zero = (rc | rm | re) == 0;
    auto EX = [&](int i) { return static_cast<int64_t>(readlane64(curp, 8 + i)); };
    const int64_t ac = ext ? EX(0) : rc, am = ext ? EX(1) : rm, ae = ext ? EX(2) : re;
    const int64_t sr0 = ext ? EX(3) : INT64_MIN, sr1 = ext ? EX(4) : INT64_MIN;
    const int64_t sa0 = ext ? EX(5) : 0, sa1 = ext ? EX(6) : 0;
    uint64_t fdom[kDevDomKeys];
#pragma unroll
    for (int kk = 0; kk < kDevDomKeys; ++kk) {
      uint64_t any = 0, bits = 0;
#pragma unroll
      for (int g = 0; g < G; ++g) {
        const uint64_t m = kk < w.n_dk ? D(kk * kDevDynG + g) : 0ull;
        any |= m;
        const bool in = 64 * g + lane < k && ((m >> lane) & 1) && pdom[g][kk] >= 0;
        bits |= in ? 1ull << pdom[g][kk] : 0ull;
      }
      fdom[kk] = any != 0 ? wave_or(bits) : 0ull;
    }
    stamp(st.cyc_a);
    uint64_t nlref[G];
#pragma unroll
    for (int g = 0; g < G; ++g) nlref[g] = 0;
#pragma unroll
    for (int s2 = 0; s2 < kDevSpreadSlots; ++s2) {
      const int sw = 5 * kDevDynG + 1 + s2 * (kDevDynG + 3);
      const uint64_t i0 = D(sw + kDevDynG);
      if (i0 == ~0ull) continue;
      const int kk = static_cast<int>(i0 & 3);
      const bool nl = ((i0 >> 2) & 1) != 0;
      const int self = static_cast<int>((i0 >> 3) & 1);
      const int64_t skew = static_cast<int32_t>(static_cast<uint32_t>(i0 >> 32));
      const uint32_t off = static_cast<uint32_t>(D(sw + kDevDynG + 1));
      uint64_t rem[G];
      int pd[G];
#pragma unroll
      for (int g = 0; g < G; ++g) {
        rem[g] = D(sw + g) & ballot(64 * g + lane < k);
        int d = -1;
#pragma unroll
        for (int k2 = 0; k2 < kDevDomKeys; ++k2) d = k2 == kk ? pdom[g][k2] : d;
        pd[g] = d;
      }
      nbytes += 8u * (kDevDynG + 3) + 256u;
      if (!nl) {
        const int edom = static_cast<int32_t>(static_cast<uint32_t>(D(sw + kDevDynG + 1) >> 32));
        const uint64_t pm = D(sw + kDevDynG + 2);
#pragma unroll
        for (int g = 0; g < G; ++g) pd[g] = pd[g] >= 0 ? pd[g] : edom;
        int cv = w.sp_tab[off + lane];
        for (;;) {
          int gs = -1;
#pragma unroll
          for (int g = G - 1; g >= 0; --g) gs = rem[g] != 0 ? g : gs;
          if (gs < 0) break;
          int d = 0;
#pragma unroll
          for (int g = 0; g < G; ++g)
            if (g == gs) d = __builtin_amdgcn_readlane(pd[g], __builtin_ctzll(rem[g]));
          int n = 0;
#pragma unroll
          for (int g = 0; g < G; ++g) {
            const uint64_t same = rem[g] & ballot(pd[g] == d);
            rem[g] &= ~same;
            n += __builtin_popcountll(same);
          }
          if (d >= 0 && lane == d) cv += n;
        }
        const bool inp = ((pm >> lane) & 1) != 0;
        const int mn = wave_min(inp ? cv : INT_MAX);
        fdom[kk] |= ballot(inp && static_cast<int64_t>(cv) + self - mn > skew);
      } else {
        int capv[G];
#pragma unroll
        for (int g = 0; g < G; ++g) capv[g] = ((rem[g] >> lane) & 1) ? w.sp_tab[off + static_cast<uint32_t>(pnode[g])] : INT_MAX;
        for (;;) {
          int gs = -1;
#pragma unroll
          for (int g = G - 1; g >= 0; --g) gs = rem[g] != 0 ? g : gs;
          if (gs < 0) break;
          int y = 0, cap = 0;
#pragma unroll
          for (int g = 0; g < G; ++g)
            if (g == gs) {
              const int j = __builtin_ctzll(rem[g]);
              y = __builtin_amdgcn_readlane(pnode[g], j);
              cap = __builtin_amdgcn_readlane(capv[g], j);
            }
          uint64_t same[G];
          int n = 0;
#pragma unroll
          for (int g = 0; g < G; ++g) {
            same[g] = rem[g] & ballot(pnode[g] == y);
            rem[g] &= ~same[g];
            n += __builtin_popcountll(same[g]);
          }
          if (n > cap) {
#pragma unroll
            for (int g = 0; g < G; ++g) nlref[g] |= same[g];
          }
        }
      }
    }
    const uint64_t meta = D(5 * kDevDynG);
    int nt = 0;
    int tslot[kDevDynTerms] = {0, 0, 0, 0}, tbase[kDevDynTerms] = {0, 0, 0, 0};
    uint64_t adom[kDevDynTerms][G];
#pragma unroll
    for (int i = 0; i < kDevDynTerms; ++i)
#pragma unroll
      for (int g = 0; g < G; ++g) adom[i][g] = 0;
    if (meta != ~0ull) {
      const int set = static_cast<int>(meta >> 1);
      const bool self = (meta & 1) != 0;
      const int32_t* si = w.ds_info + set * (2 + 2 * kDevDynTerms);
      nt = si[0];
      bool map_has = si[1] == 0;
#pragma unroll
      for (int i = 0; i < kDevDynTerms; ++i) {
        if (i >= nt) continue;
        tslot[i] = si[2 + 2 * i];
        tbase[i] = si[3 + 2 * i];
        const bool table = dk_row_of(w, tslot[i]) >= 0;
        uint64_t bits = 0;
#pragma unroll
        for (int g = 0; g < G; ++g) {
          const uint64_t mm = D(4 * kDevDynG + g);
          int d = -1;
#pragma unroll
          for (int kk = 0; kk < kDevDomKeys; ++kk) d = kk == tslot[i] ? pdom[g][kk] : d;
          const bool in = 64 * g + lane < k && ((mm >> lane) & 1) && d >= 0;
          const uint64_t b = ballot(in);
          map_has = map_has || b != 0;
          bits |= in ? 1ull << d : 0ull;
          adom[i][g] = table ? 0ull : b;
        }
        if (table) adom[i][0] = wave_or(bits);
      }
      if (!map_has && self) nt = 0;
    }
    stamp(st.cyc_b);
    int ans = INT_MAX;
    for (int ch = 0; ch < CH && ans == INT_MAX && ch * 64 < Wp; ++ch) {
      const int wd = ch * 64 + lane;
      const bool wv = wd < Wp;
      const uint32_t wi = wv ? static_cast<uint32_t>(wd) : 0u;
      const uint64_t sv = tab[static_cast<uint32_t>(r01) + wi];
      const uint64_t tv = tab[static_cast<uint32_t>(r01 >> 32) + wi] & tab[static_cast<uint32_t>(r23) + wi] &
                          tab[static_cast<uint32_t>(r23 >> 32) + wi];
      nbytes += 64u * 32u;
      uint64_t dyn = ~0ull;
#pragma unroll
      for (int kk = 0; kk < kDevDomKeys; ++kk) {
        uint64_t m = fdom[kk];
        const int row0 = dk_row_of(w, kk);
        while (m != 0) {
          const int d = __builtin_ctzll(m);
          m &= m - 1;
          dyn &= ~at[static_cast<size_t>(row0 + d) * Wp + wi];
          nbytes += 64u * 8u;
        }
      }
#pragma unroll
      for (int i = 0; i < kDevDynTerms; ++i) {
        if (i >= nt) continue;
        uint64_t row = at[static_cast<size_t>(tbase[i]) * Wp + wi];
        nbytes += 64u * 8u;
        const int row0 = dk_row_of(w, tslot[i]);
        if (row0 >= 0) {
          uint64_t m = adom[i][0];
          while (m != 0) {
            const int x = __builtin_ctzll(m);
            m &= m - 1;
            row |= at[static_cast<size_t>(row0 + x) * Wp + wi];
            nbytes += 64u * 8u;
          }
        } else {
#pragma unroll
          for (int g = 0; g < G; ++g) {
            uint64_t m = adom[i][g];
            while (m != 0) {
              const int x = __builtin_ctzll(m);
              m &= m - 1;
              const int y = __builtin_amdgcn_readlane(pnode[g], x);
              if ((y >> 6) == wd) row |= 1ull << (y & 63);
            }
          }
        }
        dyn &= row;
      }
#pragma unroll
      for (int g = 0; g < G; ++g) {
        uint64_t m = nlref[g];
        while (m != 0) {
          const int x = __builtin_ctzll(m);
          m &= m - 1;
          const int y = __builtin_amdgcn_readlane(pnode[g], x);
          if ((y >> 6) == wd) dyn &= ~(1ull << (y & 63));
        }
      }
      const uint64_t sd = wv ? sv & dyn : 0ull;
      const uint64_t clean = sd & tv & ~tl[wd];
      const uint64_t mc = ballot(clean != 0);
      int cn = INT_MAX;
      if (mc != 0) {
        const int L0 = __builtin_ctzll(mc);
        cn = (ch * 64 + L0) * 64 + __builtin_ctzll(readlane64(clean, L0));
      }
      int best = INT_MAX;
#pragma unroll
      for (int g = 0; g < G; ++g) {
        const bool in = snode[g] >= ch * 4096 && snode[g] < min(cn, (ch + 1) * 4096);
        const int src = in ? (snode[g] >> 6) - ch * 64 : 0;
        const uint64_t ws = (static_cast<uint64_t>(from_lane(static_cast<uint32_t>(sd >> 32), src)) << 32) |
                            from_lane(static_cast<uint32_t>(sd), src);
        const bool fit = (zero | ((rc <= scpu[g]) & (rm <= smem[g]) & (re <= seph[g]))) & (sr0 <= ss0[g]) &
                         (sr1 <= ss1[g]);
        const bool ok = in & (((ws >> (snode[g] & 63)) & 1ull) != 0) & (sleft[g] >= 1) & ((sport[g] & pin) == 0) & fit;
        best = ok ? min(best, snode[g]) : best;
      }
      ans = min(cn, wave_min(best));
    }
    stamp(st.cyc_c);
    if (ans == INT_MAX) {
      status = k;
      break;
    }
    bool hit = false;
#pragma unroll
    for (int g = 0; g < G; ++g) {
      if (ballot(snode[g] == ans) != 0) {
        hit = true;
        if (snode[g] == ans) {
          scpu[g] -= ac;
          smem[g] -= am;
          seph[g] -= ae;
          sleft[g] -= 1;
          sport[g] |= pm;
          ss0[g] -= sa0;
          ss1[g] -= sa1;
        }
      }
    }
    if (!hit) {
      const uint64_t* rec = w.node_rec + static_cast<size_t>(ans) * 8;
      const int64_t fc = static_cast<int64_t>(rec[0]), fm = static_cast<int64_t>(rec[1]),
                    fe = static_cast<int64_t>(rec[2]);
      const uint64_t pb = rec[3];
      const int pl = static_cast<int>(static_cast<int64_t>(rec[4]));
      const int64_t b0 = ext && erow0 >= 0 ? w.node_scal[static_cast<size_t>(erow0) * w.n_pad + ans] : 0;
      const int64_t b1 = ext && erow1 >= 0 ? w.node_scal[static_cast<size_t>(erow1) * w.n_pad + ans] : 0;
      nbytes += 40u;
#pragma unroll
      for (int g = 0; g < G; ++g)
        if (lane + 64 * g == nslots) {
          snode[g] = ans;
          scpu[g] = fc - ac;
          smem[g] = fm - am;
          seph[g] = fe - ae;
          sleft[g] = pl - 1;
          sport[g] = pb | pm;
          ss0[g] = b0 - sa0;
          ss1[g] = b1 - sa1;
        }
      ++nslots;
      if (lane == 0) tl[ans >> 6] |= 1ull << (ans & 63);
    }
    int dn[kDevDomKeys];
#pragma unroll
    for (int kk = 0; kk < kDevDomKeys; ++kk)
      dn[kk] = kk < w.n_dk ? w.dk_dom[static_cast<size_t>(kk) * w.n_spot + ans] : -1;
#pragma unroll
    for (int g = 0; g < G; ++g)
      if (lane + 64 * g == k) {
        pnode[g] = ans;
#pragma unroll
        for (int kk = 0; kk < kDevDomKeys; ++kk) pdom[g][kk] = dn[kk];
      }
    stamp(st.cyc_d);
  }
#pragma unroll
  for (int g = 0; g < G; ++g) {
    const int kq = 64 * g + lane;
    if (kq < np) w.out_node[p0 + kq] = (status < 0 || kq < status) ? pnode[g] : -1;
  }
}

struct K2Entry {
  int ci, p0, np, g;
  uint64_t t_start, c_start, t_list;
};
template <bool PROF>
__device__ __forceinline__ K2Entry k2_entry(const DevWorkload& w, const int4* __restrict__ list, int li) {
  K2Entry x;
  x.t_start = PROF ? __builtin_amdgcn_s_memrealtime() : 0;
  x.c_start = PROF || w.out_cycles ? __builtin_amdgcn_s_memtime() : 0;
  const int4 e = li < w.n_list_head ? w.list_head[li] : list[li];
  x.ci = __builtin_amdgcn_readfirstlane(e.x);
  x.p0 = __builtin_amdgcn_readfirstlane(e.y);
  x.np = __builtin_amdgcn_readfirstlane(e.z) - x.p0;
  x.g = __builtin_amdgcn_readfirstlane(e.w);
  if (PROF) asm volatile("s_waitcnt lgkmcnt(0)" ::: "memory");
  x.t_list = PROF ? __builtin_amdgcn_s_memrealtime() : 0;
  return x;
}

__device__ __forceinline__ void k2_once(const DevWorkload& w) {
  unsigned long long* dn = reinterpret_cast<unsigned long long*>(w.d_min_next);
  unsigned long long* dm = reinterpret_cast<unsigned long long*>(w.d_min);
  dn[0] = ~0ull;
  dm[1] = w.first_fallback_local < 0 ? ~0ull : static_cast<unsigned long long>(w.first_fallback_local) << 32;
  dm[2] = w.rank_next;
}

__device__ __forceinline__ void k2_skipped(const DevWorkload& w, int ci) {
  if ((threadIdx.x & 63) != 0) return;
  if (ci == 0) k2_once(w);
  if (w.out_cycles) w.out_cycles[ci] = 0;
}

template <bool PROF>
__device__ __forceinline__ void k2_finish(const DevWorkload& w, const K2Entry& x, int status, int wide,
                                          uint32_t nbytes, const K2Stats& st, const int (&mapv)[kMapG],
                                          const bool in_regs = true, const int32_t* lmap = nullptr) {
  const int lane = threadIdx.x & 63;
  const int ci = x.ci, p0 = x.p0, np = x.np;
  int best = 0;
  if (lane == 0 && ci == 0) k2_once(w);
  if (lane == 0) {
    w.out_status[ci] = status;
    w.out_bytes[ci] = nbytes;
    if (w.out_cycles)
      w.out_cycles[ci] = static_cast<uint32_t>(min(__builtin_amdgcn_s_memtime() - x.c_start, 0xffffffffull));
    if (status < 0) {
      const unsigned long long key = (static_cast<unsigned long long>(x.g) << 32) | static_cast<unsigned>(ci);
      best = key < atomicMin(reinterpret_cast<unsigned long long*>(w.d_min), key);
    }
    if (PROF) {
      uint64_t* pr = w.prof + static_cast<size_t>(ci) * 16;
      pr[0] = x.t_start;
      pr[1] = x.t_list;
      pr[2] = __builtin_amdgcn_s_memrealtime();
      pr[3] = __builtin_amdgcn_s_memtime() - x.c_start;
      pr[4] = static_cast<uint64_t>(status >= 0 ? status + 1 : np);
      pr[5] = static_cast<uint64_t>(wide);
      pr[6] = st.n_spec_miss;
      pr[7] = static_cast<uint64_t>(st.n_min) | (static_cast<uint64_t>(st.n_far) << 32);
      pr[8] = st.cyc_a;
      pr[9] = st.cyc_b;
      pr[10] = st.cyc_c;
      pr[11] = st.cyc_d;
      if (wide == 2) {
        pr[8] |= static_cast<uint64_t>(st.cyc_a_ld) << 32;
        pr[10] |= static_cast<uint64_t>(st.n_res_pods) << 32 | static_cast<uint64_t>(st.n_res) << 48;
        pr[11] |= static_cast<uint64_t>(st.cyc_res_ld) << 32;
        pr[12] = st.cyc_res;
        pr[13] = st.cyc_win;
        pr[14] = st.cyc_rec - x.c_start;
        pr[15] = st.narrow | (status < 0 ? 16u : 0u);
      }
    }
  }
  if (w.res_stat) {
    const uint64_t tag = static_cast<uint64_t>(w.seq) << 32;
    if (__builtin_amdgcn_readfirstlane(best)) {
      if (in_regs && w.k2_map_regs) {
#pragma unroll
        for (int g = 0; g < kMapG; ++g)
          if (64 * g + lane < np)
            __hip_atomic_store(w.res_map + p0 + 64 * g + lane, tag | static_cast<uint32_t>(mapv[g]), __ATOMIC_RELAXED,
                               __HIP_MEMORY_SCOPE_SYSTEM);
      } else if (lmap && w.k2_map_regs) {
        for (int q = lane; q < np; q += 64)
          __hip_atomic_store(w.res_map + p0 + q, tag | static_cast<uint32_t>(lmap[q]), __ATOMIC_RELAXED,
                             __HIP_MEMORY_SCOPE_SYSTEM);
      } else {
        __builtin_amdgcn_fence(__ATOMIC_RELEASE, "agent");
        for (int q = lane; q < np; q += 64)
          __hip_atomic_store(w.res_map + p0 + q,
                             tag | static_cast<uint32_t>(__hip_atomic_load(w.out_node + p0 + q, __ATOMIC_RELAXED,
                                                                           __HIP_MEMORY_SCOPE_AGENT)),
                             __ATOMIC_RELAXED, __HIP_MEMORY_SCOPE_SYSTEM);
      }
    }
    if (lane == 0)
      __hip_atomic_store(w.res_stat + ci, tag | (status < 0 ? 1u : 0u), __ATOMIC_RELAXED, __HIP_MEMORY_SCOPE_SYSTEM);
  }
}

template <int CH, bool PROF>
__global__ __launch_bounds__(256) void k2_place(DevWorkload w_arg, const int4* __restrict__ list, int n_list) {
  const DevWorkload& w = *(const DevWorkload*)__builtin_amdgcn_kernarg_segment_ptr();
  (void)w_arg;
  extern __shared__ __attribute__((aligned(16))) uint64_t k2_lds[];
  const int lane = threadIdx.x & 63;
  const int wave = threadIdx.x >> 6;
  const int li = __builtin_amdgcn_readfirstlane(static_cast<int>(blockIdx.x * (blockDim.x >> 6)) + wave);
  if (li >= n_list) return;
  const K2Entry x = k2_entry<PROF>(w, list, li);
  if (x.g <= w.cand_floor) {
    k2_skipped(w, x.ci);
    return;
  }
  const int ci = x.ci, p0 = x.p0, np = x.np;
  K2Lds& L = *reinterpret_cast<K2Lds*>(k2_lds + static_cast<size_t>(wave) * (sizeof(K2Lds) / 8));

  K2Stats st;
  int status = -1;
  int wide = 0;
  uint32_t nbytes = 0;
  int mapv[kMapG] = {-1, -1, -1, -1};
  bool in_regs = false, in_lds = false;
  const int dbase = w.dyn_cand ? __builtin_amdgcn_readfirstlane(w.dyn_cand[ci]) : -1;
  const int ebase = w.ext_cand ? __builtin_amdgcn_readfirstlane(w.ext_cand[ci]) : -1;
  const bool node_order = np <= 4 * 64 && w.k2_mode == 0;
  if (dbase >= 0) {
    wide = 3;
    uint64_t* tl = reinterpret_cast<uint64_t*>(&L);
    if (np <= 64) k2_domain<CH, 1, PROF>(w, tl, p0, np, dbase, status, nbytes, st, ebase);
    else if (np <= 128) k2_domain<CH, 2, PROF>(w, tl, p0, np, dbase, status, nbytes, st, ebase);
    else if (np <= 256) k2_domain<CH, 4, PROF>(w, tl, p0, np, dbase, status, nbytes, st, ebase);
    else k2_domain<CH, kDevDynG, PROF>(w, tl, p0, np, dbase, status, nbytes, st, ebase);
  } else if (node_order && ebase >= 0) {
    uint64_t* F = reinterpret_cast<uint64_t*>(&L);
    wide = 2;
    if (np <= 64) k2_node_order<1, PROF, false, true>(w, F, p0, np, status, st, nbytes, mapv, ebase);
    else if (np <= 128) k2_node_order<2, PROF, false, true>(w, F, p0, np, status, st, nbytes, mapv, ebase);
    else k2_node_order<4, PROF, false, true>(w, F, p0, np, status, st, nbytes, mapv, ebase);
    in_regs = true;
  } else if (ebase >= 0) {
    int placed = k2_run<1, CH, PROF, true>(w, L, p0, np, status, st, nbytes, ebase);
    wide = placed < 0 ? 1 : 0;
    if (placed < 0) placed = k2_run<8, CH, PROF, true>(w, L, p0, np, status, st, nbytes, ebase);
    for (int i = lane; i < np; i += 64) w.out_node[p0 + i] = i < placed ? L.omap[i] : -1;
    in_lds = true;
  } else if (node_order) {
    uint64_t* F = reinterpret_cast<uint64_t*>(&L);
    wide = 2;
    if (np <= 64) k2_node_order<1, PROF>(w, F, p0, np, status, st, nbytes, mapv);
    else if (np <= 128) k2_node_order<2, PROF>(w, F, p0, np, status, st, nbytes, mapv);
    else k2_node_order<4, PROF>(w, F, p0, np, status, st, nbytes, mapv);
    in_regs = true;
  } else {
    int placed = k2_run<1, CH, PROF>(w, L, p0, np, status, st, nbytes);
    wide = placed < 0 ? 1 : 0;
    if (placed < 0) placed = k2_run<8, CH, PROF>(w, L, p0, np, status, st, nbytes);
    for (int i = lane; i < np; i += 64) w.out_node[p0 + i] = i < placed ? L.omap[i] : -1;
    in_lds = true;
  }
  k2_finish<PROF>(w, x, status, wide, nbytes, st, mapv, in_regs, in_lds ? L.omap : nullptr);
}

template <int GMAX, bool PROF, bool WIDE = false, bool XT = false>
__global__ __launch_bounds__(256) void k2_node(DevWorkload w_arg, const int4* __restrict__ list, int n_list) {
  const DevWorkload& w = *(const DevWorkload*)__builtin_amdgcn_kernarg_segment_ptr();
  (void)w_arg;
  extern __shared__ __attribute__((aligned(16))) uint64_t k2_lds[];
  const int wave = threadIdx.x >> 6;
  const size_t region = 64 * GMAX * kNHS + (w.s_head_only ? 64 * GMAX * 4 : 0);
  const int nco = XT ? 0 : w.n_coop;
  if constexpr (!XT) {
    static_assert(sizeof(CoopArea) <= (kCoopWaves - 1) * 64 * kNHS * 8, "the cooperative area fits the helpers' LDS");
    if (static_cast<int>(blockIdx.x) < nco) {
      if (w.cand_floor >= 0) {
        const int bi = static_cast<int>(blockIdx.x);
        const int4 e = bi < w.n_list_head ? w.list_head[bi] : list[bi];
        if (__builtin_amdgcn_readfirstlane(e.w) <= w.cand_floor) {
          if (wave == 0) k2_skipped(w, __builtin_amdgcn_readfirstlane(e.x));
          return;
        }
      }
      CoopArea* A = reinterpret_cast<CoopArea*>(k2_lds + region);
      if (wave != 0) {
        coop_helper(w, *A, wave);
        return;
      }
      const K2Entry x = k2_entry<PROF>(w, list, static_cast<int>(blockIdx.x));
      K2Stats st;
      int status = -1;
      uint32_t nbytes = 0;
      int mapv[kMapG] = {-1, -1, -1, -1};
      if (GMAX == 1 || x.np <= 64)
        k2_node_order<1, PROF, false, false, true>(w, k2_lds, x.p0, x.np, status, st, nbytes, mapv, -1, -2, -2, A);
      else if (GMAX == 2 || x.np <= 128)
        k2_node_order<(GMAX >= 2 ? 2 : 1), PROF, WIDE, false, true>(w, k2_lds, x.p0, x.np, status, st, nbytes, mapv, -1,
                                                                    -2, -2, A);
      else k2_node_order<GMAX, PROF, WIDE, false, true>(w, k2_lds, x.p0, x.np, status, st, nbytes, mapv, -1, -2, -2, A);
      if (threadIdx.x == 0) A->cmd = 1;
      __syncthreads();
      st.narrow |= 2;
      k2_finish<PROF>(w, x, status, 2, nbytes, st, mapv);
      return;
    }
  }
  const int li = __builtin_amdgcn_readfirstlane(nco + static_cast<int>((blockIdx.x - nco) * (blockDim.x >> 6)) + wave);
  if (li >= n_list) return;
  int4 xe = {-1, -1, -1, 0};
  if (XT) xe = w.list_ext[li];
  const K2Entry x = k2_entry<PROF>(w, list, li);
  if (x.g <= w.cand_floor) {
    k2_skipped(w, x.ci);
    return;
  }
  uint64_t* F = k2_lds + static_cast<size_t>(wave) * region;
  K2Stats st;
  int status = -1;
  uint32_t nbytes = 0;
  int mapv[kMapG] = {-1, -1, -1, -1};
  if constexpr (XT) {
    const int ebase = __builtin_amdgcn_readfirstlane(xe.x);
    const int er0 = __builtin_amdgcn_readfirstlane(xe.y), er1 = __builtin_amdgcn_readfirstlane(xe.z);
    if (ebase >= 0) {
      if (GMAX == 1 || x.np <= 64)
        k2_node_order<1, PROF, false, true>(w, F, x.p0, x.np, status, st, nbytes, mapv, ebase, er0, er1);
      else if (GMAX == 2 || x.np <= 128)
        k2_node_order<(GMAX >= 2 ? 2 : 1), PROF, WIDE, true>(w, F, x.p0, x.np, status, st, nbytes, mapv, ebase, er0, er1);
      else k2_node_order<GMAX, PROF, WIDE, true>(w, F, x.p0, x.np, status, st, nbytes, mapv, ebase, er0, er1);
      k2_finish<PROF>(w, x, status, 2, nbytes, st, mapv);
      return;
    }
  }
  if (GMAX == 1 || x.np <= 64) k2_node_order<1, PROF>(w, F, x.p0, x.np, status, st, nbytes, mapv);
  else if (GMAX == 2 || x.np <= 128)
    k2_node_order<(GMAX >= 2 ? 2 : 1), PROF, WIDE>(w, F, x.p0, x.np, status, st, nbytes, mapv);
  else k2_node_order<GMAX, PROF, WIDE>(w, F, x.p0, x.np, status, st, nbytes, mapv);
  k2_finish<PROF>(w, x, status, 2, nbytes, st, mapv);
}

template <typename K, typename... A>
void launch(K kernel, dim3 grid, dim3 block, size_t lds, hipStream_t s, hipEvent_t ev0, hipEvent_t ev1, A... args) {
  if (ev0 || ev1) hipExtLaunchKernelGGL(kernel, grid, block, static_cast<uint32_t>(lds), s, ev0, ev1, 0, args...);
  else hipLaunchKernelGGL(kernel, grid, block, lds, s, args...);
}

}

#ifndef SR_KPART
#define SR_KPART -1
#endif
template <bool PROF>
hipError_t launch_k2_node_g(const DevWorkload& w, int G, hipStream_t s, hipEvent_t ev0, hipEvent_t ev1);
template <bool PROF>
hipError_t launch_k2_node_xt_g(const DevWorkload& w, int G, hipStream_t s, hipEvent_t ev0, hipEvent_t ev1);
template <int CH, bool PROF>
hipError_t launch_k2_place_ch(const DevWorkload& w, hipStream_t s, hipEvent_t ev0, hipEvent_t ev1);

#if SR_KPART == -1 || SR_KPART == 1
template <bool PROF>
hipError_t launch_k2_node_g(const DevWorkload& w, int G, hipStream_t s, hipEvent_t ev0, hipEvent_t ev1) {
  const int n = w.n_list;
  const int wpb = k2_waves_per_block(w.k2_wpb, n);
  if (w.n_coop < 0 || w.n_coop > n || (w.n_coop > 0 && (wpb != kCoopWaves || w.ext_cand))) return hipErrorInvalidValue;
  const dim3 grid(w.n_coop + (n - w.n_coop + wpb - 1) / wpb), block(64 * wpb);
  const size_t lds = wpb * static_cast<size_t>(64 * G * kNHS + (w.s_head_only ? 64 * G * 4 : 0)) * 8;
  const bool wide = n <= 2048;
  if (w.ext_cand) return launch_k2_node_xt_g<PROF>(w, G, s, ev0, ev1);
  if (G == 1) launch(k2_node<1, PROF>, grid, block, lds, s, ev0, ev1, w, w.list, n);
  else if (G == 2 && wide) launch(k2_node<2, PROF, true>, grid, block, lds, s, ev0, ev1, w, w.list, n);
  else if (G == 2) launch(k2_node<2, PROF>, grid, block, lds, s, ev0, ev1, w, w.list, n);
  else launch(k2_node<4, PROF, true>, grid, block, lds, s, ev0, ev1, w, w.list, n);
  return hipGetLastError();
}
template hipError_t launch_k2_node_g<false>(const DevWorkload&, int, hipStream_t, hipEvent_t, hipEvent_t);
template hipError_t launch_k2_node_g<true>(const DevWorkload&, int, hipStream_t, hipEvent_t, hipEvent_t);
#endif

#if SR_KPART == -1 || SR_KPART == 8
template <bool PROF>
hipError_t launch_k2_node_xt_g(const DevWorkload& w, int G, hipStream_t s, hipEvent_t ev0, hipEvent_t ev1) {
  const int n = w.n_list;
  const int wpb = k2_waves_per_block(w.k2_wpb, n);
  const dim3 grid((n + wpb - 1) / wpb), block(64 * wpb);
  const size_t lds = wpb * static_cast<size_t>(64 * G * kNHS + (w.s_head_only ? 64 * G * 4 : 0)) * 8;
  const bool wide = n <= 2048;
  if (G == 1) launch(k2_node<1, PROF, false, true>, grid, block, lds, s, ev0, ev1, w, w.list, n);
  else if (G == 2 && wide) launch(k2_node<2, PROF, true, true>, grid, block, lds, s, ev0, ev1, w, w.list, n);
  else if (G == 2) launch(k2_node<2, PROF, false, true>, grid, block, lds, s, ev0, ev1, w, w.list, n);
  else launch(k2_node<4, PROF, true, true>, grid, block, lds, s, ev0, ev1, w, w.list, n);
  return hipGetLastError();
}
template hipError_t launch_k2_node_xt_g<false>(const DevWorkload&, int, hipStream_t, hipEvent_t, hipEvent_t);
template hipError_t launch_k2_node_xt_g<true>(const DevWorkload&, int, hipStream_t, hipEvent_t, hipEvent_t);
#endif

#if SR_KPART == -1 || SR_KPART >= 2
template <int CH, bool PROF>
hipError_t launch_k2_place_ch(const DevWorkload& w, hipStream_t s, hipEvent_t ev0, hipEvent_t ev1) {
  const int n = w.n_list;
  const int wpb = k2_waves_per_block(w.k2_wpb, n);
  const dim3 grid((n + wpb - 1) / wpb), block(64 * wpb);
  launch(k2_place<CH, PROF>, grid, block, wpb * sizeof(K2Lds), s, ev0, ev1, w, w.list, n);
  return hipGetLastError();
}
#define SR_PLACE_INST(CH)                                                                                      \
  template hipError_t launch_k2_place_ch<CH, false>(const DevWorkload&, hipStream_t, hipEvent_t, hipEvent_t); \
  template hipError_t launch_k2_place_ch<CH, true>(const DevWorkload&, hipStream_t, hipEvent_t, hipEvent_t);
#endif
#if SR_KPART == -1 || SR_KPART == 2
SR_PLACE_INST(1)
#endif
#if SR_KPART == -1 || SR_KPART == 3
SR_PLACE_INST(2)
#endif
#if SR_KPART == -1 || SR_KPART == 4
SR_PLACE_INST(4)
#endif
#if SR_KPART == -1 || SR_KPART == 5
SR_PLACE_INST(8)
#endif
#if SR_KPART == -1 || SR_KPART == 6
SR_PLACE_INST(16)
#endif
#if SR_KPART == -1 || SR_KPART == 7
SR_PLACE_INST(32)
#endif

#if SR_KPART == -1 || SR_KPART == 0
template <bool PROF>
hipError_t launch_k2(const DevWorkload& w, hipStream_t s, hipEvent_t ev0, hipEvent_t ev1) {
  const int n = w.n_list;
  if (n <= 0) return hipSuccess;
  if (k2_node_launch(w.dyn_cand != nullptr, w.k2_mode, w.max_np, w.k2_node_kernel))
    return launch_k2_node_g<PROF>(w, k2_node_groups(w.max_np), s, ev0, ev1);
  const int chunks = (w.Wp + 63) / 64;
  if (chunks <= 1) return launch_k2_place_ch<1, PROF>(w, s, ev0, ev1);
  if (chunks <= 2) return launch_k2_place_ch<2, PROF>(w, s, ev0, ev1);
  if (chunks <= 4) return launch_k2_place_ch<4, PROF>(w, s, ev0, ev1);
  if (chunks <= 8) return launch_k2_place_ch<8, PROF>(w, s, ev0, ev1);
  if (chunks <= 16) return launch_k2_place_ch<16, PROF>(w, s, ev0, ev1);
  return launch_k2_place_ch<32, PROF>(w, s, ev0, ev1);
}

hipError_t launch_tables(const DevWorkload& w, int32_t local_first_fallback, hipStream_t s, hipEvent_t ev0,
                         hipEvent_t ev1) {
  const int s_blocks = (w.n_classes + 4 * kSClasses - 1) / (4 * kSClasses);
  const int wgroups = (w.Wp + kTWords - 1) / kTWords;
  int t_waves = 0;
  for (int d = 0; d < 4; ++d) t_waves += (w.t_off[d + 1] - w.t_off[d] + 63) / 64 * wgroups;
  const unsigned blocks = static_cast<unsigned>(std::max(1, s_blocks + (t_waves + 3) / 4));
  if (w.k0_inc) {
    const int s_waves = w.n_k0_cols > 0 ? (w.n_classes + 63) / 64 : 0;
    int tw = 0;
    for (int d = 1; d < 4 && w.n_k0_cols > 0; ++d) tw += (w.t_off[d + 1] - w.t_off[d] + 63) / 64;
    const int waves = s_waves + tw + w.n_k0_rows;
    launch(k0_incremental, dim3(static_cast<unsigned>(std::max(1, (waves + 3) / 4))), dim3(256), 0, s, ev0, ev1, w,
           s_waves, tw, local_first_fallback);
    return hipGetLastError();
  }
  launch(k0_tables, dim3(blocks), dim3(256), 0, s, ev0, ev1, w, s_blocks, local_first_fallback);
  return hipGetLastError();
}

hipError_t launch_placement(const DevWorkload& w, hipStream_t s, hipEvent_t ev0, hipEvent_t ev1) {
  return w.prof ? launch_k2<true>(w, s, ev0, ev1) : launch_k2<false>(w, s, ev0, ev1);
}

hipError_t launch_winner(const DevWorkload& w, hipStream_t s, hipEvent_t ev0, hipEvent_t ev1) {
  launch(k3_winner, dim3(1), dim3(64), 0, s, ev0, ev1, w);
  return hipGetLastError();
}

hipError_t launch_sequence(const SeqRound& r, hipStream_t s) {
  if (r.n_cand <= 0) return hipSuccess;
  const unsigned blocks = static_cast<unsigned>(std::min(64, (r.n_cand + 255) / 256));
  hipLaunchKernelGGL(k3_sequence, dim3(blocks), dim3(256), 0, s, r);
  return hipGetLastError();
}
#endif

}
```

### k8s-spot-rescheduler_amd/csrc/kernels.hpp

```cpp
#pragma once

#include <hip/hip_runtime.h>

#include <cstdint>

#include "launch_shape.hpp"
#include "progops.hpp"

namespace sr {

constexpr int kResultHeader = 8;
constexpr size_t kK0ProfWaves = 32768;
constexpr int kDevDynG = 8;
constexpr int kDevSpreadSlots = 2;
constexpr int kDevDynU64 = 5 * kDevDynG + 1 + kDevSpreadSlots * (kDevDynG + 3);
constexpr int kDevDomKeys = 4;
constexpr int kNodePatchU64 = 12;
constexpr int kPodPatchU64 = 3;
constexpr int64_t kTPad = INT64_MAX - 1;
constexpr int kDevDynTerms = 4;
constexpr int kDevExtU64 = 8;
constexpr int kListInline = 128;

struct DevWorkload {
  int32_t n_spot, n_pad, Wp;
  const int64_t* node_free;
  const uint64_t* node_rec;
  const uint64_t* node_patch;
  int32_t n_node_patch;
  const uint64_t* pod_patch;
  int32_t n_pod_patch;
  int32_t k0_skip;
  int32_t n_dirty;
  int32_t dirty_node[16];
  int64_t dirty_free[16][3];
  int32_t* d_min_next;
  int32_t first_fallback_local;
  int32_t k0_inc;
  int32_t n_k0_cols, n_k0_rows;
  const int32_t* k0_cols;
  const int32_t* k0_rows;
  int32_t n_atoms;
  const uint64_t* atoms;
  const int32_t* cls_prog_off;
  const int32_t* cls_prog;
  const int32_t* cls_prog8;
  int32_t n_classes;
  uint32_t s_empty_off;
  int32_t n_t;
  int32_t t_off[5];
  const int64_t* t_thr;
  int32_t n_pods;
  uint64_t swap_mask;
  const uint64_t* pod_rec;
  int32_t n_cand;
  const int32_t* cand_off;
  const int32_t* cand_global;
  const int4* list;
  int32_t n_list;
  int32_t max_np;
  int32_t k2_node_kernel;
  int32_t s_head_only;
  const int32_t* dyn_cand;
  const uint64_t* dyn_pod;
  int32_t n_dk;
  const int32_t* dk_dom;
  int32_t dk_row[4];
  const int32_t* sp_tab;
  const int32_t* ds_info;
  const int32_t* ext_cand;
  const uint64_t* pod_ext;
  const int64_t* node_scal;
  const int4* list_ext;
  uint64_t* S;
  uint64_t* T;
  int32_t* out_node;
  int32_t* out_status;
  uint32_t* out_bytes;
  uint32_t* out_cycles;
  int32_t* d_min;
  uint64_t rank_next;
  uint64_t* result;
  uint64_t* res_stat;
  uint64_t* res_map;
  uint32_t seq;
  int32_t k2_narrow;
  int32_t k2_wpb;
  int32_t k2_excl;
  int32_t k2_map_regs;
  int32_t n_coop;
  int32_t cand_floor;
  int32_t k2_mode;
  uint64_t* prof;
  int32_t n_list_head;
  int4 list_head[kListInline];
};

hipError_t launch_tables(const DevWorkload& w, int32_t local_first_fallback, hipStream_t s,
                         hipEvent_t ev0 = nullptr, hipEvent_t ev1 = nullptr);
hipError_t launch_placement(const DevWorkload& w, hipStream_t s, hipEvent_t ev0 = nullptr, hipEvent_t ev1 = nullptr);
hipError_t launch_winner(const DevWorkload& w, hipStream_t s, hipEvent_t ev0 = nullptr, hipEvent_t ev1 = nullptr);

struct SeqRound {
  const int32_t* d_min;
  const int32_t* cand_global;
  const int32_t* cand_off;
  const int32_t* out_status;
  const int32_t* out_node;
  const int32_t* in_off;
  int32_t n_cand;
  int32_t floor;
  int32_t fb_stop;
  int32_t* seq_status;
  int32_t* seq_node;
};
hipError_t launch_sequence(const SeqRound& r, hipStream_t s);

constexpr int kPdbHeader = 2;
struct SeqPdbRound {
  SeqRound r;
  const int32_t* need_off;
  const int32_t* need_group;
  const int32_t* need_count;
  int32_t* remaining;
  uint8_t* refused;
  int32_t* win;
  uint64_t* words;
  uint32_t seq;
};
hipError_t launch_sequence_pdb(const SeqPdbRound& p, hipStream_t s);

}
```

### k8s-spot-rescheduler_amd/csrc/planner.cpp

```cpp
#include <hip/hip_runtime.h>
#include <rccl/rccl.h>

#include <algorithm>
#include <atomic>
#include <cerrno>
#include <chrono>
#include <climits>
#include <cstdio>
#include <cstdlib>
#include <cstring>
#include <memory>
#include <string>
#include <vector>

#include "explain_dev.hpp"
#include "host.hpp"
#include "kernels.hpp"
#include "residency.hpp"
#include "seq_pdb.hpp"

#include <dlfcn.h>
#include <fcntl.h>
#include <sys/mman.h>
#include <sys/stat.h>
// ... 260 lines not shown
sr_status shm_reduce(sr_ctx* ctx, int p) {
  auto& S = ctx->shm;
  const sr::Workload& w = ctx->cur->wl;
  const uint32_t tag = ctx->dw.seq;
  const int32_t N = ctx->nranks;
  auto ready = [tag](volatile uint64_t* x) { return static_cast<uint32_t>(*x >> 32) == tag; };
  std::vector<int64_t> n_r(static_cast<size_t>(N)), b_r(static_cast<size_t>(N));
  int64_t ff = -1, nx = -1;
  for (int32_t r = 0; r < N; ++r) {
    volatile uint64_t* hd = shm_region(ctx, r, p);
    for (int i : {0, 1, 2, 4}) {
      sr_status st = shm_wait(ctx, [&] { return ready(hd + i); }, false, r);
      if (st != SR_OK) return st;
    }
    std::atomic_thread_fence(std::memory_order_acquire);
    n_r[r] = static_cast<uint32_t>(hd[0]);
    b_r[r] = static_cast<int64_t>(static_cast<uint32_t>(hd[1])) - 1;
    const int64_t f = static_cast<int64_t>(static_cast<uint32_t>(hd[2])) - 1;
    if (f >= 0) ff = ff < 0 ? f : std::min(ff, f);
    const int64_t x = static_cast<int64_t>(static_cast<uint32_t>(hd[4])) - 1;
    if (x >= 0) nx = nx < 0 ? x : std::min(nx, x);
  }
  int64_t first_ok = -1;
  int32_t owner = -1, oci = -1;
  std::vector<int64_t> at(static_cast<size_t>(N), 0);
  for (;;) {
    int32_t r = -1;
    int64_t g = INT64_MAX;
    for (int32_t q = 0; q < N; ++q) {
      if (at[q] >= n_r[q]) continue;
      const int64_t gq = (b_r[q] + at[q]) * N + q;
      if (gq < g) g = gq, r = q;
    }
    if (r < 0) break;
    volatile uint64_t* reg = shm_region(ctx, r, p);
    volatile uint64_t* in = reg + kShmHdr + at[r]++;
    sr_status st = shm_wait(ctx, [&] { return ready(in); }, false, r);
    if (st != SR_OK) return st;
    const uint32_t v = static_cast<uint32_t>(*in);
    if ((v & 3u) != 0) continue;
    const int32_t ci = static_cast<int32_t>(v >> 2);
    volatile uint64_t* sw = reg + kShmHdr + S.max_cand + ci;
    st = shm_wait(ctx, [&] { return ready(sw); }, r == ctx->rank, r);
    if (st != SR_OK) return st;
    if (static_cast<uint32_t>(*sw) & 1u) {
      first_ok = g;
      owner = r;
      oci = ci;
      break;
    }
  }
  shm_region(ctx, ctx->rank, p)[3] = static_cast<uint64_t>(tag) << 32 | 1u;
  volatile uint64_t* res = static_cast<volatile uint64_t*>(ctx->h_result.p);
  const uint64_t T = static_cast<uint64_t>(tag) << 32;
  int32_t np = 0;
  if (owner == ctx->rank) {
    const int32_t off = w.cand_off[oci];
    np = w.cand_off[oci + 1] - off;
    volatile uint64_t* map = static_cast<volatile uint64_t*>(ctx->h_early.p) + ctx->dw.n_cand + off;
    for (int32_t q = 0; q < np; ++q) {
      sr_status st = shm_wait(ctx, [&] { return ready(map + q); }, true, ctx->rank);
      if (st != SR_OK) return st;
      res[sr::kResultHeader + q] = T | static_cast<uint32_t>(map[q]);
    }
  }
  res[0] = T | static_cast<uint32_t>(first_ok);
  res[1] = T | (owner == ctx->rank ? 1u : 0u);
  res[2] = T | static_cast<uint32_t>(np);
  res[3] = T | static_cast<uint32_t>(ff);
  res[4] = T | static_cast<uint32_t>(nx);
  return SR_OK;
}

sr_status allreduce_min_dev(sr_ctx* ctx, void* words, int32_t n) {
  if (ctx->comm) {
    ncclResult_t r = rccl().all_reduce(words, words, static_cast<size_t>(n), ncclUint64, ncclMin, ctx->comm,
                                       ctx->stream);
    if (r != ncclSuccess) {
      ctx->err = std::string("ncclAllReduce: ") + rccl().error_string(r);
      return SR_ERR_RCCL;
    }
    return SR_OK;
  }
  HIP_TRY(ctx, host_reserve(ctx->h_comm, 64));
  uint64_t* h = static_cast<uint64_t*>(ctx->h_comm.p);
  HIP_TRY(ctx, hipMemcpyAsync(h, words, sizeof(uint64_t) * n, hipMemcpyDeviceToHost, ctx->stream));
  HIP_TRY(ctx, hipStreamSynchronize(ctx->stream));
  if (ctx->host_fn(ctx->host_user, h, n) != 0) {
    ctx->err = "caller-provided allreduce(min) failed";
    return SR_ERR_RCCL;
  }
  HIP_TRY(ctx, hipMemcpyAsync(words, h, sizeof(uint64_t) * n, hipMemcpyHostToDevice, ctx->stream));
  return SR_OK;
}

Slot& pick_slot(sr_ctx* ctx, const sr_candidates* cands) {
  const int32_t n = cands->n_cand;
  uint64_t key = 0x5107ull + static_cast<uint64_t>(n);
  if (n > 0) {
    const int32_t b = cands->cand_pod_off[0], e = cands->cand_pod_off[n];
    auto mixin = [&](uint64_t x) { key = (key ^ x) * 0x100000001B3ull; };
    mixin(static_cast<uint32_t>(b));
    mixin(static_cast<uint32_t>(e));
    if (e > b) {
      mixin(static_cast<uint32_t>(cands->cand_pods[b]));
      mixin(static_cast<uint32_t>(cands->cand_pods[b + (e - b) / 2]));
      mixin(static_cast<uint32_t>(cands->cand_pods[e - 1]));
    }
    if (cands->cand_global) {
      mixin(static_cast<uint32_t>(cands->cand_global[0]));
      mixin(static_cast<uint32_t>(cands->cand_global[n - 1]));
    }
  }
  Slot* pick = nullptr;
  for (auto& sl : ctx->slots)
    if (sl->key == key) pick = sl.get();
  if (!pick && static_cast<int32_t>(ctx->slots.size()) < ctx->n_slots) {
    ctx->slots.push_back(std::make_unique<Slot>());
    pick = ctx->slots.back().get();
  }
  if (!pick) {
    pick = ctx->slots.front().get();
    for (auto& sl : ctx->slots)
      if (sl->used < pick->used) pick = sl.get();
  }
  pick->key = key;
  pick->used = ++ctx->slot_clock;
  return *pick;
}

sr_status check_shm_shards(sr_ctx* ctx, const sr_candidates* cands) {
  const int32_t n = cands->n_cand, N = ctx->nranks;
  if (n > ctx->shm.max_cand) {
    ctx->err = "more candidates than sr_comm_init_shm's max_cand";
    return SR_ERR_CAPACITY;
  }
  const int32_t* G = cands->cand_global;
  if (n > 0 && !G && N > 1) {
    ctx->err = "the shared-memory transport needs cand_global (interleaved shards)";
    return SR_ERR_INVALID_ARG;
  }
  const int64_t b = n > 0 && G ? G[0] / N : 0;
  for (int32_t i = 0; i < n; ++i)
    if ((G ? G[i] : i) != (b + i) * N + ctx->rank) {
      ctx->err = "the shared-memory transport needs interleaved shards: cand_global[i] = (first + i) * nranks + rank";
      return SR_ERR_INVALID_ARG;
    }
  ctx->shm.base = n > 0 ? static_cast<int32_t>(b) : -1;
  return SR_OK;
}

sr::ResidencySwitches switches(const sr_ctx* ctx) {
  sr::ResidencySwitches sw;
  sw.k0_skip = ctx->k0_skip;
  sw.k0_incremental = ctx->k0_incremental;
  sw.node_patch = ctx->node_patch;
  sw.list_cost = ctx->list_cost;
  sw.k2_mode = ctx->k2_mode;
  return sw;
}

sr_status reorder_list(sr_ctx* ctx, Slot& sl) {
  HIP_TRY(ctx, hipEventSynchronize(sl.ev_cost));
  sr::reorder_list_by_cost(sl.wl, static_cast<const uint32_t*>(sl.h_cycles.p), ctx->enc.list_head, ctx->k2_coop);
  return SR_OK;
}

sr_status reserve_buffers(sr_ctx* ctx, Slot& sl, size_t arena_bytes, bool moved[3]) {
  const sr::Workload& w = sl.wl;
  const int32_t na = static_cast<int32_t>(w.pod_src.size());
  const int32_t ncand = static_cast<int32_t>(w.cand_global.size());
  if (ctx->ev_upload) HIP_TRY(ctx, hipEventSynchronize(ctx->ev_upload));
  const size_t h_cap = sl.h_arena.cap;
  HIP_TRY(ctx, host_reserve(sl.h_arena, arena_bytes));
  moved[0] = sl.h_arena.cap != h_cap;
  const size_t arena_cap = sl.arena.cap;
  HIP_TRY(ctx, dev_reserve(sl.arena, arena_bytes));
  moved[1] = sl.arena.cap != arena_cap;
  const size_t n_rows = static_cast<size_t>(w.n_classes) + w.t_dim.size();
  const size_t row_bytes = static_cast<size_t>(w.Wp) * sizeof(uint64_t);
  const size_t t_cap = sl.tables.cap;
  HIP_TRY(ctx, dev_reserve(sl.tables, n_rows * row_bytes));
  moved[2] = sl.tables.cap != t_cap;
  HIP_TRY(ctx, dev_reserve(ctx->out_node, sizeof(int32_t) * std::max(1, na)));
  HIP_TRY(ctx, dev_reserve(ctx->out_status, sizeof(int32_t) * std::max(1, ncand)));
  HIP_TRY(ctx, dev_reserve(ctx->out_bytes, sizeof(uint32_t) * std::max(1, ncand)));
  HIP_TRY(ctx, dev_reserve(ctx->dmin, 64));
  const size_t res_bytes = sizeof(uint64_t) * (sr::kResultHeader + static_cast<size_t>(std::max(1, w.max_cand_pods)));
  HIP_TRY(ctx, host_reserve(ctx->h_result, res_bytes));
  HIP_TRY(ctx, host_reserve(ctx->h_early, sizeof(uint64_t) * (static_cast<size_t>(ncand) + na + 1)));
  return SR_OK;
}

sr_status queue_upload(sr_ctx* ctx, Slot& sl) {
  const char* hs = static_cast<const char*>(sl.h_arena.p);
  char* dv = static_cast<char*>(sl.arena.p);
  for (const sr::ArenaCopy& c : ctx->lists.copies)
    HIP_TRY(ctx, hipMemcpyAsync(dv + c.off, hs + c.off, c.bytes, hipMemcpyHostToDevice, ctx->stream));
  if (!ctx->ev_upload) HIP_TRY(ctx, hipEventCreateWithFlags(&ctx->ev_upload, hipEventDisableTiming));
  HIP_TRY(ctx, hipEventRecord(ctx->ev_upload, ctx->stream));
  return SR_OK;
}

sr_status fill_dev_workload(sr_ctx* ctx, Slot& sl) {
  const sr::Workload& w = sl.wl;
  const sr::TickPlan& p = ctx->plan;
  const sr::ArenaLayout& o = p.at;
  const sr::TickLists& tl = ctx->lists;
  const int32_t na = static_cast<int32_t>(w.pod_src.size());
  const int32_t ncand = static_cast<int32_t>(w.cand_global.size());
  char* base = static_cast<char*>(sl.arena.p);
  auto at = [base](size_t off) { return static_cast<void*>(base + off); };
  const bool dyn = o.dyn, ext = o.ext;
  sr::DevWorkload& d = ctx->dw;
  d = sr::DevWorkload{};
  d.n_spot = w.n_spot;
  d.n_pad = w.n_pad;
  d.Wp = w.Wp;
  d.node_rec = static_cast<const uint64_t*>(at(o.node_rec));
  d.node_free = static_cast<const int64_t*>(at(o.node_free));
  d.n_atoms = w.n_atoms;
  d.atoms = static_cast<const uint64_t*>(at(o.atoms));
  d.cls_prog_off = static_cast<const int32_t*>(at(o.cls_prog_off));
  d.cls_prog = static_cast<const int32_t*>(at(o.cls_prog));
  d.cls_prog8 = static_cast<const int32_t*>(at(o.cls_prog8));
  d.n_classes = w.n_classes;
  d.s_empty_off = w.empty_class >= 0 ? static_cast<uint32_t>(w.empty_class) * static_cast<uint32_t>(w.Wp) : 0xffffffffu;
  d.n_t = static_cast<int32_t>(w.t_dim.size());
  for (int i = 0; i < 5; ++i) d.t_off[i] = w.t_off[i];
  d.t_thr = static_cast<const int64_t*>(at(o.t_thr));
  d.n_pods = na;
  d.pod_rec = static_cast<const uint64_t*>(at(o.pod_rec));
  d.n_cand = ncand;
  d.cand_off = static_cast<const int32_t*>(at(o.cand_off));
  d.cand_global = static_cast<const int32_t*>(at(o.cand_global));
  d.list = static_cast<const int4*>(at(o.list));
  d.n_list = static_cast<int32_t>(w.list.size() / 4);
  d.n_list_head = std::min(d.n_list, sr::kListInline);
  for (int32_t i = 0; i < d.n_list_head; ++i)
    d.list_head[i] = int4{w.list[4 * i], w.list[4 * i + 1], w.list[4 * i + 2], w.list[4 * i + 3]};
  d.max_np = w.max_cand_pods;
  d.dyn_cand = dyn ? static_cast<const int32_t*>(at(o.dyn_cand)) : nullptr;
  d.dyn_pod = dyn ? static_cast<const uint64_t*>(at(o.dyn_pod)) : nullptr;
  d.dk_dom = dyn ? static_cast<const int32_t*>(at(o.dk_dom)) : nullptr;
  d.ds_info = dyn ? static_cast<const int32_t*>(at(o.ds_info)) : nullptr;
  d.sp_tab = dyn ? static_cast<const int32_t*>(at(o.sp_tab)) : nullptr;
  d.n_dk = w.n_dk;
  d.ext_cand = ext ? static_cast<const int32_t*>(at(o.ext_cand)) : nullptr;
  d.pod_ext = ext ? static_cast<const uint64_t*>(at(o.pod_ext)) : nullptr;
  d.list_ext = ext ? static_cast<const int4*>(at(o.list_ext)) : nullptr;
  d.node_scal = ext ? static_cast<const int64_t*>(at(o.node_scal)) : nullptr;
  static_assert(sr::kDevExtU64 == sr::kExtU64, "extension record layout shared by encode.cpp and kernels.hip");
  static_assert(sr::kDevDynU64 == sr::kDynU64 && sr::kDevDomKeys == sr::kDomKeys && sr::kDevDynTerms == sr::kDynTerms &&
                    sr::kDevSpreadSlots == sr::kSpreadSlots,
                "domain-path layout shared by encode.cpp and kernels.hip");
  for (int k = 0; k < sr::kDomKeys; ++k) d.dk_row[k] = w.dk_row[k];
  d.S = static_cast<uint64_t*>(sl.tables.p);
  d.T = d.S + static_cast<size_t>(w.n_classes) * w.Wp;
  d.out_node = static_cast<int32_t*>(ctx->out_node.p);
  d.out_status = static_cast<int32_t*>(ctx->out_status.p);
  d.out_bytes = static_cast<uint32_t*>(ctx->out_bytes.p);
  d.d_min = static_cast<int32_t*>(ctx->dmin.p);
  d.cand_floor = -1;
  d.k2_mode = ctx->k2_mode;
  d.k2_narrow = ctx->k2_narrow;
  d.k2_wpb = ctx->k2_wpb;
  d.k2_excl = ctx->k2_excl;
  d.k2_map_regs = ctx->k2_map_regs;
  d.k2_node_kernel = ctx->k2_node_kernel;
  d.s_head_only = 0;
  if (ctx->s_head_only && w.Wp > 64 && sr::k2_node_launch(dyn, ctx->k2_mode, w.max_cand_pods, ctx->k2_node_kernel)) {
    bool short_programs = true;
    for (int32_t k = 0; k < w.n_classes && short_programs; ++k)
      short_programs = w.cls_prog8[static_cast<size_t>(k) * 8] != -2;
    d.s_head_only = short_programs ? 1 : 0;
  }
  d.swap_mask = w.swap_mask;
  d.rank_next = ~0ull;
  d.prof = nullptr;
  if (ctx->prof_file) {
    const size_t pbytes = sizeof(uint64_t) * (16 * static_cast<size_t>(std::max(1, ncand)) + 2 * sr::kK0ProfWaves);
    HIP_TRY(ctx, dev_reserve(ctx->prof, pbytes));
    HIP_TRY(ctx, hipMemsetAsync(ctx->prof.p, 0, pbytes, ctx->stream));
    d.prof = static_cast<uint64_t*>(ctx->prof.p);
  }
  void* dres = nullptr;
  HIP_TRY(ctx, hipHostGetDevicePointer(&dres, ctx->h_result.p, 0));
  d.result = static_cast<uint64_t*>(dres);
  HIP_TRY(ctx, hipHostGetDevicePointer(&dres, ctx->h_early.p, 0));
  ctx->d_early = static_cast<uint64_t*>(dres);
  d.res_stat = d.res_map = nullptr;
  d.node_patch = p.n_node_patch ? static_cast<const uint64_t*>(at(o.node_patch)) : nullptr;
  d.n_node_patch = p.n_node_patch;
  d.k0_inc = p.k0_inc ? 1 : 0;
  d.n_k0_cols = static_cast<int32_t>(tl.k0_cols.size());
  d.n_k0_rows = static_cast<int32_t>(tl.k0_rows.size());
  d.k0_cols = tl.k0_cols.empty() ? nullptr : static_cast<const int32_t*>(at(o.k0_cols));
  d.k0_rows = tl.k0_rows.empty() ? nullptr : static_cast<const int32_t*>(at(o.k0_rows));
  d.pod_patch = p.n_pod_patch ? static_cast<const uint64_t*>(at(o.pod_patch)) : nullptr;
  d.n_pod_patch = p.n_pod_patch;
  d.k0_skip = p.skip ? 1 : 0;
  d.n_dirty = p.n_dirty;
  for (int32_t i = 0; i < p.n_dirty; ++i) {
    d.dirty_node[i] = p.dirty_node[i];
    for (int dm = 0; dm < 3; ++dm) d.dirty_free[i][dm] = p.dirty_free[i][dm];
  }
  static_assert(sizeof(d.dirty_node) / sizeof(d.dirty_node[0]) == sr::kSkipDirty, "kSkipDirty nodes in the kernel arguments");
  d.first_fallback_local = w.first_fallback;
  static_assert(sr::kPodPatchU64 == sr::kPodPatchWords && sr::kNodePatchU64 == sr::kNodePatchWords &&
                    sr::kTPad == sr::kTSpare,
                "patch layout shared with encode.cpp and residency.cpp");
  return SR_OK;
}

void account_prepare(sr_ctx* ctx, const sr::Workload& w, double ms_pack_host, double ms_upload) {
  const sr::DevWorkload& d = ctx->dw;
  const sr::TickPlan& p = ctx->plan;
  const std::vector<int32_t>& kcols = ctx->lists.k0_cols;
  const std::vector<int32_t>& krows = ctx->lists.k0_rows;
  ctx->t.bytes_uploaded = p.bytes_uploaded;
  const uint64_t row = static_cast<uint64_t>(w.Wp) * 8;
  uint64_t atom_reads = w.cls_prog.size();
  const uint64_t s_row = d.s_head_only ? static_cast<uint64_t>(std::min(w.Wp, 8)) * 8 : row;
  ctx->t.bytes_tables = static_cast<uint64_t>(w.n_classes) * s_row + w.t_dim.size() * row + atom_reads * s_row +
                        3ull * 8 * w.n_pad + 32ull * w.n_classes;
  if (p.k0_inc) {
    const int32_t s_words = d.s_head_only ? std::min(w.Wp, 8) : w.Wp;
    uint64_t s_cols = 0;
    for (int32_t col : kcols) s_cols += col < s_words ? 1 : 0;
    ctx->t.bytes_tables = (static_cast<uint64_t>(w.n_classes) + atom_reads) * 8 * s_cols +
                          (32ull * w.n_classes) * (s_cols > 0 ? 1 : 0) + w.t_dim.size() * 8 * kcols.size() +
                          3ull * 64 * 8 * kcols.size() + krows.size() * (row + 8ull * w.n_pad);
  }
  ctx->t.bytes_placement = 0;
  ctx->issued_known = false;
  ctx->issued_checks = 0;
  ctx->t.ms_pack_host = ms_pack_host;
  ctx->t.ms_upload = ms_upload;
  ctx->t.n_pods = d.n_pods;
  ctx->t.n_spot = w.n_spot;
  ctx->t.n_cand = d.n_cand;
  ctx->t.n_words = w.Wp;
  ctx->t.n_rows_static = d.n_classes;
  ctx->t.n_rows_threshold = d.n_t;
  ctx->t.n_classes = w.n_classes;
  ctx->t.enc_new_specs = ctx->enc.last_new_specs;
  ctx->t.enc_static_rebuilt = ctx->enc.last_static_changed;
  ctx->t.enc_state_nodes = ctx->enc.last_state_changed;
  ctx->t.enc_memo_pods = ctx->enc.last_memo_hits;
  ctx->t.enc_reused = ctx->enc.last_reused;
  ctx->t.enc_pod_patches = ctx->enc.last_pod_patches;
  ctx->t.k0_columns = p.skip ? -2 : p.k0_inc ? static_cast<int32_t>(kcols.size()) : -1;
  ctx->t.k0_rows_moved = p.k0_inc ? static_cast<int32_t>(krows.size()) : 0;
  ctx->t.k0_dirty_nodes = p.skip ? static_cast<int32_t>(ctx->lists.node_patch.size() / sr::kNodePatchWords) : 0;
  if (p.skip) ctx->t.bytes_tables = 0;
}

sr_status prepare(sr_ctx* ctx, const sr_snapshot* snap, const sr_cluster* c, const sr_candidates* cands) {
  using ms = std::chrono::duration<double, std::milli>;
  auto t0 = std::chrono::steady_clock::now();
  ctx->prepared = false;
  sr_status st = ctx->shm.host ? check_shm_shards(ctx, cands) : SR_OK;
  if (st != SR_OK) return st;
  Slot& sl = pick_slot(ctx, cands);
  ctx->cur = &sl;
  sr::Workload& w = sl.wl;
  std::string err;
  st = sr::encode_workload(&ctx->enc, snap, c, cands, &w, &err);
  if (st != SR_OK) {
    ctx->err = err;
    sl.res.encode_failed();
    return st;
  }
  const sr::ResidencySwitches sw = switches(ctx);
  sr::TickPlan& p = ctx->plan;
  sl.res.observe(w, ctx->enc, sw, &ctx->lists, &p);

  HIP_TRY(ctx, hipSetDevice(ctx->device));
  st = settle(ctx);
  if (st == SR_OK && p.reorder_due) st = reorder_list(ctx, sl);
  if (st != SR_OK) return st;
  bool moved[3] = {false, false, false};
  st = reserve_buffers(ctx, sl, p.at.bytes, moved);
  if (st != SR_OK) {
    sl.res.moved(moved[0], moved[1], moved[2]);
    return st;
  }
  auto t1 = std::chrono::steady_clock::now();
  sl.res.resolve(w, ctx->enc, sw, moved[0], moved[1], moved[2], p.reorder_due, static_cast<char*>(sl.h_arena.p),
                 &ctx->lists, &p);
  st = queue_upload(ctx, sl);
  if (st != SR_OK) return st;
  sl.res.upload_queued(w, p);
  ctx->t.k2_list_by_cost = sl.res.list_by_cost(w) ? 1 : 0;
  auto t2 = std::chrono::steady_clock::now();
  st = fill_dev_workload(ctx, sl);
  if (st != SR_OK) return st;
  account_prepare(ctx, w, ms(t1 - t0).count(), ms(t2 - t1).count());
  ctx->prepared = true;
  return SR_OK;
}

sr_status flush_timing(sr_ctx* ctx) {
  if (ctx->ev_used == 0) return SR_OK;
  HIP_TRY(ctx, hipEventSynchronize(ctx->ev_end[ctx->ev_used - 1]));
  double* sums[4] = {&ctx->t.ms_tables, &ctx->t.ms_placement, &ctx->t.ms_winner, &ctx->t.ms_collective};
  for (size_t i = 0; i < ctx->ev_used; ++i) {
    float ms = 0;
    HIP_TRY(ctx, hipEventElapsedTime(&ms, ctx->ev_start[i], ctx->ev_end[i]));
    *sums[ctx->ev_kernel[i]] += ms;
  }
  ctx->ev_used = 0;
  return SR_OK;
}

sr_status finish_early(sr_ctx* ctx, sr_plan_out* out) {
  const sr::Workload& w = ctx->cur->wl;
  const sr::DevWorkload& d = ctx->dw;
  if (ctx->timing_cur) ctx->t.n_runs += 1;
  volatile uint64_t* stat = static_cast<volatile uint64_t*>(ctx->h_early.p);
  volatile uint64_t* map = stat + d.n_cand;
  const uint32_t tag = d.seq;
  auto ready = [&](volatile uint64_t* p) { return static_cast<uint32_t>(*p >> 32) == tag; };
  const auto t0 = std::chrono::steady_clock::now();
  uint32_t spins = 0;
  bool synced = false;
  auto wait = [&](volatile uint64_t* p) -> sr_status {
    while (!ready(p)) {
      if (!synced && (++spins & 1023) == 0 && std::chrono::steady_clock::now() - t0 > std::chrono::milliseconds(100)) {
        HIP_TRY(ctx, hipStreamSynchronize(ctx->stream));
        synced = true;
      }
      if (synced && !ready(p)) {
        ctx->err = "K2 result word not written by this run";
        return SR_ERR_HIP;
      }
    }
    return SR_OK;
  };
  int32_t k = 0;
  for (; k < d.n_cand; ++k) {
    sr_status st = wait(stat + k);
    if (st != SR_OK) return st;
    if (static_cast<uint32_t>(stat[k]) == 1) break;
  }
  ctx->in_flight = !synced;
  out->first_fallback = w.first_fallback;
  out->first_ok = k < d.n_cand ? w.cand_global[k] : -1;
  out->winner = (out->first_ok >= 0 && (w.first_fallback < 0 || w.first_fallback > out->first_ok)) ? out->first_ok : -1;
  out->winner_npods = 0;
  if (k < d.n_cand) {
    const int32_t o = w.cand_off[k], np = w.cand_off[k + 1] - o;
    for (int32_t q = 0; q < np; ++q) {
      sr_status st = wait(map + o + q);
      if (st != SR_OK) return st;
    }
    std::atomic_thread_fence(std::memory_order_acquire);
    out->winner_npods = np;
    if (out->winner_map)
      for (int32_t q = 0; q < np; ++q) out->winner_map[q] = static_cast<int32_t>(static_cast<uint32_t>(map[o + q]));
  }
  out->checks_dense = static_cast<uint64_t>(d.n_pods) * static_cast<uint64_t>(w.n_spot);
  out->fallback_pods = w.fallback_pods;
  out->checks = ctx->issued_known ? ctx->issued_checks : 0;
  return SR_OK;
}

struct SeqWalk {
  int32_t floor = -1;
  int32_t winner = -1;
  int32_t fallback = -1;
  int32_t end = -1;
  std::vector<int32_t> map;
  sr::PdbLedger* pdb = nullptr;
  int32_t stop = INT32_MAX;
};

int32_t first_fallback_above(const sr::Workload& w, int32_t floor) {
  for (int32_t i = floor + 1; i < w.n_input_cand; ++i)
    if (w.status_host[i] == SR_CAND_FALLBACK) return i;
  return INT32_MAX;
}

sr_status finish_sequence(sr_ctx* ctx, SeqWalk* sq) {
  const sr::Workload& w = ctx->cur->wl;
  const sr::DevWorkload& d = ctx->dw;
  if (ctx->timing_cur) ctx->t.n_runs += 1;
  volatile uint64_t* stat = static_cast<volatile uint64_t*>(ctx->h_early.p);
  volatile uint64_t* map = stat + d.n_cand;
  const uint32_t tag = d.seq;
  auto ready = [&](volatile uint64_t* p) { return static_cast<uint32_t>(*p >> 32) == tag; };
  const auto t0 = std::chrono::steady_clock::now();
  uint32_t spins = 0;
  bool synced = false;
  auto wait = [&](volatile uint64_t* p) -> sr_status {
    while (!ready(p)) {
      if (!synced && (++spins & 1023) == 0 && std::chrono::steady_clock::now() - t0 > std::chrono::milliseconds(100)) {
        HIP_TRY(ctx, hipStreamSynchronize(ctx->stream));
        synced = true;
      }
      if (synced && !ready(p)) {
        ctx->err = "K2 result word not written by this run";
        return SR_ERR_HIP;
      }
    }
    return SR_OK;
  };
  ctx->in_flight = d.n_list > 0;
  sq->winner = sq->fallback = -1;
  sq->end = w.n_input_cand - 1;
  int32_t k = static_cast<int32_t>(std::upper_bound(w.cand_src.begin(), w.cand_src.end(), sq->floor) -
                                   w.cand_src.begin());
  for (int32_t i = sq->floor + 1; i < w.n_input_cand; ++i) {
    if (k < d.n_cand && w.cand_src[k] == i) {
      sr_status st = wait(stat + k);
      if (st != SR_OK) return st;
      if (static_cast<uint32_t>(stat[k]) == 1) {
        sq->winner = sq->end = i;
        break;
      }
      ++k;
    } else if (w.status_host[i] == SR_CAND_FALLBACK) {
      sq->fallback = i;
      sq->end = i - 1;
      break;
    }
  }
  if (sq->winner >= 0) {
    const int32_t o = w.cand_off[k], np = w.cand_off[k + 1] - o;
    for (int32_t q = 0; q < np; ++q) {
      sr_status st = wait(map + o + q);
      if (st != SR_OK) return st;
    }
    std::atomic_thread_fence(std::memory_order_acquire);
    sq->map.resize(static_cast<size_t>(np));
    for (int32_t q = 0; q < np; ++q) sq->map[q] = static_cast<int32_t>(static_cast<uint32_t>(map[o + q]));
  }
  if (synced) ctx->in_flight = false;
  return SR_OK;
}

sr_status finish_sequence_pdb(sr_ctx* ctx, SeqWalk* sq) {
  const sr::Workload& w = ctx->cur->wl;
  const sr::DevWorkload& d = ctx->dw;
  if (ctx->timing_cur) ctx->t.n_runs += 1;
  volatile uint64_t* res = static_cast<volatile uint64_t*>(ctx->h_result.p);
  const uint32_t tag = d.seq;
  auto ready = [&](size_t i) { return static_cast<uint32_t>(res[i] >> 32) == tag; };
  auto val = [&](size_t i) { return static_cast<int32_t>(static_cast<uint32_t>(res[i])); };
  const auto t0 = std::chrono::steady_clock::now();
  uint32_t spins = 0;
  bool synced = false;
  auto wait = [&](size_t i) -> sr_status {
    while (!ready(i)) {
      if (!synced && (++spins & 1023) == 0 && std::chrono::steady_clock::now() - t0 > std::chrono::milliseconds(100)) {
        HIP_TRY(ctx, hipStreamSynchronize(ctx->stream));
        synced = true;
      }
      if (synced && !ready(i)) {
        ctx->err = "ledger result word not written by this round";
        return SR_ERR_HIP;
      }
    }
    return SR_OK;
  };
  ctx->in_flight = true;
  sq->winner = sq->fallback = -1;
  sq->end = w.n_input_cand - 1;
  for (size_t i = 0; i < static_cast<size_t>(sr::kPdbHeader); ++i) {
    sr_status st = wait(i);
    if (st != SR_OK) return st;
  }
  const int32_t win = val(0), np = val(1);
  if (win >= 0) {
    if (win <= sq->floor || win >= w.n_input_cand || np < 0 || np > w.max_cand_pods) {
      ctx->err = "ledger result names no candidate of this round";
      return SR_ERR_HIP;
    }
    for (int32_t q = 0; q < np; ++q) {
      sr_status st = wait(static_cast<size_t>(sr::kPdbHeader + q));
      if (st != SR_OK) return st;
    }
    std::atomic_thread_fence(std::memory_order_acquire);
    sq->map.resize(static_cast<size_t>(np));
    for (int32_t q = 0; q < np; ++q) sq->map[q] = val(static_cast<size_t>(sr::kPdbHeader + q));
    sq->winner = sq->end = win;
  } else if (sq->stop != INT32_MAX) {
    sq->fallback = sq->stop;
    sq->end = sq->stop - 1;
  }
  if (synced) ctx->in_flight = false;
  return SR_OK;
}

#define SR_TRY(expr)                   \
  do {                                 \
    sr_status _st = (expr);            \
    if (_st != SR_OK) return _st;      \
  } while (0)

sr_status event_pair(sr_ctx* ctx, int k, hipEvent_t* a, hipEvent_t* b) {
  *a = *b = nullptr;
  if (!(ctx->timing_cur >> (k == 3 ? 2 : k) & 1)) return SR_OK;
  if (ctx->ev_used == ctx->ev_start.size()) {
    if (ctx->ev_used >= 3072) {
      SR_TRY(flush_timing(ctx));
    } else {
      hipEvent_t e0, e1;
      HIP_TRY(ctx, hipEventCreate(&e0));
      HIP_TRY(ctx, hipEventCreate(&e1));
// ... 1130 lines not shown
```

Measured before the change: 325.7 billion.

## Load kernel-argument header into lane registers and precompute dirty-node fit masks

Reorders DevWorkload so the fields the K2 node kernel uses sit in a 64-word header. Each lane loads one header word, and later reads are readlane instead of repeated scalar kernarg loads. The dirty-node free-capacity table and the node patch records are also packed into per-lane registers. Per-pod dirty fit masks replace per-call resource comparisons in fix_dirty, and window_patch becomes writelane updates with no global patch-record scan. This adds a host-side check that node patches match the dirty nodes, and it raises register and readlane pressure.

```diff
diff --git a/k8s-spot-rescheduler_amd/csrc/kernels.hip b/k8s-spot-rescheduler_amd/csrc/kernels.hip
--- a/k8s-spot-rescheduler_amd/csrc/kernels.hip
+++ b/k8s-spot-rescheduler_amd/csrc/kernels.hip
@@ -403,6 +403,7 @@
   uint32_t n_spec_miss = 0, n_min = 0, n_far = 0;
   uint64_t cyc_a = 0, cyc_b = 0, cyc_c = 0, cyc_d = 0;
   uint64_t cyc_rec = 0;
+  uint64_t cyc_fh = 0;
   uint32_t narrow = 0;
   uint64_t cyc_res = 0;
   uint64_t cyc_win = 0;
@@ -703,56 +704,104 @@
 constexpr int kNHS = kNH + 1;
 constexpr int kFar = 64 * kNH;
 
+#define SR_HW(f) static_cast<int>(offsetof(DevWorkload, f) / 4)
+struct K2W {
+  const DevWorkload& k;
+  uint32_t hdr;
+  uint64_t dt;
+  mutable uint64_t pt = 0;
+  __device__ __forceinline__ explicit K2W(const DevWorkload& kk) : k(kk) {
+    const int lane = threadIdx.x & 63;
+    hdr = reinterpret_cast<const uint32_t*>(&kk)[lane];
+    dt = static_cast<uint64_t>(kk.dirty_tab[lane]);
+  }
+  __device__ __forceinline__ void fetch_patches() const {
+    const int lane = threadIdx.x & 63, nd = n_dirty();
+    if (nd > 0 && (lane & 15) < nd)
+      pt = ptr<const uint64_t*>(SR_HW(node_patch))[(lane & 15) * kNodePatchU64 + 1 + (lane >> 4)];
+  }
+  __device__ __forceinline__ uint32_t word(int i) const {
+    return static_cast<uint32_t>(__builtin_amdgcn_readlane(static_cast<int>(hdr), i));
+  }
+  template <typename P>
+  __device__ __forceinline__ P ptr(int i) const {
+    typedef __attribute__((address_space(1))) std::remove_pointer_t<P>* G;
+    return (P)(G)(static_cast<uint64_t>(word(i)) | static_cast<uint64_t>(word(i + 1)) << 32);
+  }
+#define SR_HF_I(name)                                                     \
+  __device__ __forceinline__ int32_t name() const {                       \
+    static_assert(SR_HW(name) < kHdrWords, "a field of the wave header"); \
+    return static_cast<int32_t>(word(SR_HW(name)));                       \
+  }
+#define SR_HF_P(type, name)                                                   \
+  __device__ __forceinline__ type name() const {                              \
+    static_assert(SR_HW(name) + 1 < kHdrWords, "a field of the wave header"); \
+    return ptr<type>(SR_HW(name));                                            \
+  }
+  SR_HF_I(Wp) SR_HF_I(k0_skip) SR_HF_I(n_dirty) SR_HF_I(s_head_only) SR_HF_I(k2_narrow) SR_HF_I(k2_excl)
+  SR_HF_I(n_pad) SR_HF_I(k2_map_regs) SR_HF_I(n_coop) SR_HF_I(cand_floor) SR_HF_I(n_list_head)
+  SR_HF_P(const uint64_t*, pod_rec) SR_HF_P(const uint64_t*, node_rec) SR_HF_P(const uint64_t*, S)
+  SR_HF_P(const uint64_t*, atoms) SR_HF_P(const int32_t*, cls_prog8) SR_HF_P(const uint64_t*, pod_ext)
+  SR_HF_P(const int64_t*, node_scal) SR_HF_P(int32_t*, out_node) SR_HF_P(int32_t*, out_status)
+  SR_HF_P(uint32_t*, out_bytes) SR_HF_P(uint32_t*, out_cycles) SR_HF_P(int32_t*, d_min) SR_HF_P(uint64_t*, res_stat)
+  SR_HF_P(uint64_t*, res_map) SR_HF_P(uint64_t*, prof)
+#undef SR_HF_I
+#undef SR_HF_P
+  __device__ __forceinline__ uint32_t s_empty_off() const { return word(SR_HW(s_empty_off)); }
+  __device__ __forceinline__ uint32_t seq() const { return word(SR_HW(seq)); }
+  __device__ __forceinline__ uint64_t swap_mask() const {
+    return static_cast<uint64_t>(word(SR_HW(swap_mask))) | static_cast<uint64_t>(word(SR_HW(swap_mask) + 1)) << 32;
+  }
+  __device__ __forceinline__ int dirty_node(int p) const {
+    return __builtin_amdgcn_readlane(static_cast<int>(static_cast<uint32_t>(dt)), 48 + p);
+  }
+  __device__ __forceinline__ int dirty_left(int p) const {
+    return __builtin_amdgcn_readlane(static_cast<int>(static_cast<uint32_t>(dt >> 32)), 48 + p);
+  }
+  __device__ __forceinline__ int64_t dirty_free(int p, int d) const {
+    return static_cast<int64_t>(readlane64(dt, 16 * d + p));
+  }
+  __device__ __forceinline__ uint64_t patch_word(int p, int f) const { return readlane64(pt, 16 * f + p); }
+};
+static_assert(SR_HW(seq) < kHdrWords && SR_HW(swap_mask) + 1 < kHdrWords && SR_HW(s_empty_off) < kHdrWords,
+              "fields of the wave header");
+
 __device__ __forceinline__ uint64_t f_word_far(const uint64_t* __restrict__ tab, uint64_t r01, uint64_t r23, int wd) {
   return tab[static_cast<uint32_t>(r01) + wd] & tab[static_cast<uint32_t>(r01 >> 32) + wd] &
          tab[static_cast<uint32_t>(r23) + wd] & tab[static_cast<uint32_t>(r23 >> 32) + wd];
 }
 
-__device__ __forceinline__ uint64_t f_word_prog_s(const DevWorkload& w, const int32_t* pg, int wd) {
+__device__ __forceinline__ uint64_t f_word_prog_s(const K2W& w, const int32_t* pg, int wd) {
   int op[8];
   uint64_t v[8];
 #pragma unroll
   for (int u = 0; u < 8; ++u) op[u] = pg[u];
 #pragma unroll
-  for (int u = 0; u < 8; ++u) v[u] = op[u] >= 0 ? w.atoms[static_cast<size_t>(op[u] >> 2) * w.Wp + wd] : 0ull;
+  for (int u = 0; u < 8; ++u) v[u] = op[u] >= 0 ? w.atoms()[static_cast<size_t>(op[u] >> 2) * w.Wp() + wd] : 0ull;
   return eval_prog8(op, v);
 }
 
-__device__ __forceinline__ uint64_t f_word_prog(const DevWorkload& w, const uint64_t* __restrict__ tab,
+__device__ __forceinline__ uint64_t f_word_prog(const K2W& w, const uint64_t* __restrict__ tab,
                                                 const int32_t* pg, uint64_t r01, uint64_t r23, int wd) {
   int op[8];
   uint64_t v[8];
 #pragma unroll
   for (int u = 0; u < 8; ++u) op[u] = pg[u];
 #pragma unroll
-  for (int u = 0; u < 8; ++u) v[u] = op[u] >= 0 ? w.atoms[static_cast<size_t>(op[u] >> 2) * w.Wp + wd] : 0ull;
+  for (int u = 0; u < 8; ++u) v[u] = op[u] >= 0 ? w.atoms()[static_cast<size_t>(op[u] >> 2) * w.Wp() + wd] : 0ull;
   return eval_prog8(op, v) & tab[static_cast<uint32_t>(r01 >> 32) + wd] & tab[static_cast<uint32_t>(r23) + wd] &
          tab[static_cast<uint32_t>(r23 >> 32) + wd];
 }
 
-__device__ __forceinline__ uint64_t fix_dirty(const DevWorkload& w, uint64_t f, uint64_t s, int wd, int64_t rc,
-                                              int64_t rm, int64_t re, bool zero) {
-  for (int p = 0; p < w.n_dirty; ++p) {
-    const int n = w.dirty_node[p];
-    if ((n >> 6) != wd) continue;
+__device__ __forceinline__ uint64_t fix_dirty(const K2W& w, uint64_t f, uint64_t s, int wd, uint32_t fm) {
+  const int nd = w.n_dirty();
+  for (int p = 0; p < nd; ++p) {
+    const int n = w.dirty_node(p);
     const uint64_t bit = 1ull << (n & 63);
-    const bool fits = zero || (w.dirty_free[p][0] >= rc && w.dirty_free[p][1] >= rm && w.dirty_free[p][2] >= re);
-    f = fits ? (f | (s & bit)) : (f & ~bit);
+    const uint64_t g = (fm >> p) & 1 ? (f | (s & bit)) : (f & ~bit);
+    f = (n >> 6) == wd ? g : f;
   }
   return f;
-}
-
-__device__ __forceinline__ void window_patch(const DevWorkload& w, int W, int lane, int64_t& ncpu, int64_t& nmem,
-                                             int64_t& neph, uint64_t& nport, int& nleft) {
-  for (int p = 0; p < w.n_node_patch; ++p) {
-    const uint64_t* pr = w.node_patch + static_cast<size_t>(p) * kNodePatchU64;
-    if (static_cast<int>(pr[0]) != 64 * W + lane) continue;
-    ncpu = static_cast<int64_t>(pr[1]);
-    nmem = static_cast<int64_t>(pr[2]);
-    neph = static_cast<int64_t>(pr[3]);
-    nport = pr[4];
-    nleft = static_cast<int>(static_cast<int64_t>(pr[5]));
-  }
 }
 
 __device__ __forceinline__ uint32_t from_lane(uint32_t v, int src) {
@@ -766,6 +815,25 @@
   return v;
 }
 #pragma clang diagnostic pop
+__device__ __forceinline__ uint64_t writelane64(uint64_t v, uint64_t x, int k) {
+  const int lo = writelane(static_cast<int>(static_cast<uint32_t>(v)), static_cast<int>(static_cast<uint32_t>(x)), k);
+  const int hi = writelane(static_cast<int>(static_cast<uint32_t>(v >> 32)), static_cast<int>(static_cast<uint32_t>(x >> 32)), k);
+  return static_cast<uint64_t>(static_cast<uint32_t>(hi)) << 32 | static_cast<uint32_t>(lo);
+}
+__device__ __forceinline__ void window_patch(const K2W& w, int W, int64_t& ncpu, int64_t& nmem, int64_t& neph,
+                                             uint64_t& nport, int& nleft) {
+  const int nd = w.n_dirty();
+  for (int p = 0; p < nd; ++p) {
+    const int n = w.dirty_node(p);
+    if ((n >> 6) != W) continue;
+    const int k = n & 63;
+    ncpu = static_cast<int64_t>(writelane64(static_cast<uint64_t>(ncpu), w.patch_word(p, 0), k));
+    nmem = static_cast<int64_t>(writelane64(static_cast<uint64_t>(nmem), w.patch_word(p, 1), k));
+    neph = static_cast<int64_t>(writelane64(static_cast<uint64_t>(neph), w.patch_word(p, 2), k));
+    nport = writelane64(nport, w.patch_word(p, 3), k);
+    nleft = writelane(nleft, w.dirty_left(p), k);
+  }
+}
 __device__ __forceinline__ int ff1(uint64_t x) {
   int r;
   asm("s_ff1_i32_b64 %0, %1" : "=s"(r) : "s"(x));
@@ -1025,7 +1093,7 @@
 struct CoopArea {
   int32_t cmd, n, sw, pad;
   uint64_t r01[kCoopPods], r23[kCoopPods];
-  int64_t rq[kCoopPods][3];
+  uint32_t fm[kCoopPods];
   int32_t op[kCoopPods][8];
   uint32_t best[kCoopPods];
   uint32_t rk[kCoopWaves][kCoopPods];
@@ -1034,11 +1102,13 @@
 };
 
 template <bool HO>
-__device__ __forceinline__ void coop_scan(const DevWorkload& w, CoopArea& A, int h) {
+__device__ __forceinline__ void coop_scan(const K2W& w, CoopArea& A, int h) {
   const int lane = threadIdx.x & 63;
   const int n = __builtin_amdgcn_readfirstlane(A.n), sw = __builtin_amdgcn_readfirstlane(A.sw);
-  const int Wp = w.Wp;
-  const uint64_t* __restrict__ tab = w.S;
+  const int Wp = w.Wp();
+  const uint64_t* __restrict__ tab = w.S();
+  const uint64_t* __restrict__ atoms = w.atoms();
+  const bool k0_skip = w.k0_skip() != 0;
   if (lane < n) A.rk[h][lane] = 0xffffffffu;
   const int cb0 = (sw >> 6) << 6;
   const int nch = (Wp - cb0 + 63) >> 6;
@@ -1077,7 +1147,7 @@
         if constexpr (HO) {
 #pragma unroll
           for (int u = 0; u < 8; ++u)
-            x[q][u] = op[q][u] >= 0 ? w.atoms[static_cast<size_t>(op[q][u] >> 2) * Wp + wi] : 0ull;
+            x[q][u] = op[q][u] >= 0 ? atoms[static_cast<size_t>(op[q][u] >> 2) * Wp + wi] : 0ull;
           x[q][8] = tab[static_cast<uint32_t>(a01[q] >> 32) + wi];
           x[q][9] = tab[static_cast<uint32_t>(a23[q]) + wi];
           x[q][10] = tab[static_cast<uint32_t>(a23[q] >> 32) + wi];
@@ -1103,10 +1173,7 @@
           sw0 = x[q][0];
           f = x[q][0] & x[q][1] & x[q][2] & x[q][3];
         }
-        if (w.k0_skip) {
-          const int64_t rc = A.rq[j][0], rm = A.rq[j][1], re = A.rq[j][2];
-          f = fix_dirty(w, f, sw0, word, rc, rm, re, (rc | rm | re) == 0);
-        }
+        if (k0_skip) f = fix_dirty(w, f, sw0, word, static_cast<uint32_t>(__builtin_amdgcn_readfirstlane(A.fm[j])));
         const uint64_t m = ballot(wv && f != 0) & vw;
         if (m == 0) continue;
         found |= 1ull << j;
@@ -1122,11 +1189,12 @@
   }
 }
 
-__device__ __forceinline__ void coop_helper(const DevWorkload& w, CoopArea& A, int h) {
+__device__ __forceinline__ void coop_helper(const K2W& w, CoopArea& A, int h) {
+  const bool head_only = w.s_head_only() != 0;
   for (;;) {
     __syncthreads();
     if (__hip_atomic_load(&A.cmd, __ATOMIC_RELAXED, __HIP_MEMORY_SCOPE_WORKGROUP) != 0) break;
-    if (w.s_head_only) coop_scan<true>(w, A, h);
+    if (head_only) coop_scan<true>(w, A, h);
     else coop_scan<false>(w, A, h);
     __syncthreads();
   }
@@ -1143,15 +1211,17 @@
 }
 
 template <int G, bool PROF, bool WIDE = false, bool XT = false, bool COOP = false>
-__device__ __forceinline__ void k2_node_order(const DevWorkload& w, uint64_t* __restrict__ F, const int p0,
+__device__ __forceinline__ void k2_node_order(const K2W& w, uint64_t* __restrict__ F, const int p0,
                                               const int np, int& status, K2Stats& st, uint32_t& nbytes,
                                               int (&mapv)[kMapG], const int ebase = -1, const int erow0_in = -2,
                                               const int erow1_in = -2, CoopArea* A = nullptr) {
   static_assert(64 * G * kNHS * 8 <= sizeof(K2Lds), "node-order LDS exceeds the wave's K2 region");
   static_assert(G <= kMapG, "a mapping register per pod group");
   const int lane = threadIdx.x & 63;
-  const int Wp = w.Wp;
-  const uint64_t* __restrict__ tab = w.S;
+  const int Wp = w.Wp();
+  const uint64_t* __restrict__ tab = w.S();
+  const bool k0_skip = w.k0_skip() != 0, head_only = w.s_head_only() != 0;
+  const int n_dirty = w.n_dirty();
   int64_t rc[G], rm[G], re[G];
   uint64_t pm[G], ps[G], r01[G], r23[G], fmask[G], act[G];
   int fbase[G];
@@ -1161,13 +1231,15 @@
   bool zero[G];
   int ptr[G], node[G];
   int dead = np;
+  const uint64_t swap_mask = w.swap_mask();
+  const uint32_t s_empty_off = w.s_empty_off();
 #pragma unroll
   for (int g = 0; g < G; ++g) {
-    const uint64_t* pr = w.pod_rec + static_cast<size_t>(p0 + min(64 * g + lane, np - 1)) * kRecU64;
+    const uint64_t* pr = w.pod_rec() + static_cast<size_t>(p0 + min(64 * g + lane, np - 1)) * kRecU64;
     rc[g] = static_cast<int64_t>(pr[0]);
     rm[g] = static_cast<int64_t>(pr[1]);
     re[g] = static_cast<int64_t>(pr[2]);
-    pm[g] = swap_pairs(pr[3], w.swap_mask);
+    pm[g] = swap_pairs(pr[3], swap_mask);
     ps[g] = pr[3];
     r01[g] = pr[4];
     r23[g] = pr[5];
@@ -1179,21 +1251,22 @@
     cur[g] = 0;
     ptr[g] = INT_MAX;
     node[g] = -1;
-    const uint64_t e = ballot(64 * g + lane < np && static_cast<uint32_t>(r01[g]) == w.s_empty_off);
+    const uint64_t e = ballot(64 * g + lane < np && static_cast<uint32_t>(r01[g]) == s_empty_off);
     if (e != 0) dead = min(dead, 64 * g + __builtin_ctzll(e));
   }
+  if (k0_skip) w.fetch_patches();
   XVals<int64_t> xv[G];
   int erow0 = -1, erow1 = -1;
   if constexpr (XT) {
 #pragma unroll
     for (int g = 0; g < G; ++g) {
-      const uint64_t* er = w.pod_ext + static_cast<size_t>(ebase + min(64 * g + lane, np - 1)) * kDevExtU64;
+      const uint64_t* er = w.pod_ext() + static_cast<size_t>(ebase + min(64 * g + lane, np - 1)) * kDevExtU64;
       xv[g] = {static_cast<int64_t>(er[0]), static_cast<int64_t>(er[1]), static_cast<int64_t>(er[2]),
                static_cast<int64_t>(er[3]), static_cast<int64_t>(er[4]), static_cast<int64_t>(er[5]),
                static_cast<int64_t>(er[6])};
     }
     if (erow0_in == -2) {
-      const uint64_t erow = w.pod_ext[static_cast<size_t>(ebase) * kDevExtU64 + 7];
+      const uint64_t erow = w.pod_ext()[static_cast<size_t>(ebase) * kDevExtU64 + 7];
       erow0 = __builtin_amdgcn_readfirstlane(static_cast<int32_t>(static_cast<uint32_t>(erow)));
       erow1 = __builtin_amdgcn_readfirstlane(static_cast<int32_t>(erow >> 32));
     } else {
@@ -1251,7 +1324,7 @@
                  static_cast<uint32_t>(v.a1)};
       }
     }
-    narrow = w.k2_narrow && ballot(!ok) == 0;
+    narrow = w.k2_narrow() && ballot(!ok) == 0;
   }
   bool E, O;
   {
@@ -1272,7 +1345,7 @@
       bool all = true;
 #pragma unroll
       for (int g = 0; g < G; ++g) all = all && ballot(64 * g + lane < np && !(((ps[g] & pm[g]) >> b) & 1)) == 0;
-      X = all && w.k2_excl;
+      X = all && w.k2_excl();
     }
   }
   int wcur = -1;
@@ -1283,19 +1356,18 @@
   auto load_scal = [&](int W) {
     if constexpr (XT) {
       const size_t n = static_cast<size_t>(64 * W + lane);
-      ns0 = erow0 >= 0 ? w.node_scal[static_cast<size_t>(erow0) * w.n_pad + n] : 0;
-      ns1 = erow1 >= 0 ? w.node_scal[static_cast<size_t>(erow1) * w.n_pad + n] : 0;
+      ns0 = erow0 >= 0 ? w.node_scal()[static_cast<size_t>(erow0) * w.n_pad() + n] : 0;
+      ns1 = erow1 >= 0 ? w.node_scal()[static_cast<size_t>(erow1) * w.n_pad() + n] : 0;
       nbytes += 64u * 16u;
     }
   };
   if (dead > 0) {
-    const uint64_t* nr = w.node_rec + static_cast<size_t>(lane) * 8;
+    const uint64_t* nr = w.node_rec() + static_cast<size_t>(lane) * 8;
     ncpu = static_cast<int64_t>(nr[0]);
     nmem = static_cast<int64_t>(nr[1]);
     neph = static_cast<int64_t>(nr[2]);
     nport = nr[3];
     nleft = static_cast<int>(static_cast<int64_t>(nr[4]));
-    if (w.k0_skip) window_patch(w, 0, lane, ncpu, nmem, neph, nport, nleft);
     load_scal(0);
     wcur = 0;
     nbytes += 64u * 40u;
@@ -1305,12 +1377,12 @@
     st.cyc_rec = __builtin_amdgcn_s_memtime();
   }
   int32_t* PG = reinterpret_cast<int32_t*>(F + 64 * G * kNHS);
-  if (w.s_head_only && dead > 0) {
+  if (head_only && dead > 0) {
 #pragma unroll
     for (int g = 0; g < G; ++g) {
       if (64 * g >= dead) break;
       const uint32_t cls = static_cast<uint32_t>(r01[g]) / static_cast<uint32_t>(Wp);
-      const int4* p8 = reinterpret_cast<const int4*>(w.cls_prog8 + static_cast<size_t>(cls) * 8);
+      const int4* p8 = reinterpret_cast<const int4*>(w.cls_prog8() + static_cast<size_t>(cls) * 8);
       const int4 a = p8[0], b = p8[1];
       int4* dst = reinterpret_cast<int4*>(PG + (64 * g + lane) * 8);
       dst[0] = a;
@@ -1323,19 +1395,19 @@
 
   uint32_t dirty_head = 0;
   uint32_t dfit[G];
-  for (int p = 0; p < w.n_dirty; ++p) {
-    const int wd0 = w.dirty_node[p] >> 6;
+  for (int p = 0; p < n_dirty; ++p) {
+    const int wd0 = w.dirty_node(p) >> 6;
     dirty_head |= wd0 < kNH ? 1u << wd0 : 0u;
   }
 #pragma unroll
-  for (int g = 0; g < G; ++g) {
-    dfit[g] = 0;
-    if (dirty_head != 0)
-      for (int p = 0; p < w.n_dirty; ++p) {
-        const bool fits = zero[g] || (w.dirty_free[p][0] >= rc[g] && w.dirty_free[p][1] >= rm[g] &&
-                                      w.dirty_free[p][2] >= re[g]);
-        dfit[g] |= fits ? 1u << p : 0u;
-      }
+  for (int g = 0; g < G; ++g) dfit[g] = 0;
+  for (int p = 0; p < n_dirty; ++p) {
+    const int64_t f0 = w.dirty_free(p, 0), f1 = w.dirty_free(p, 1), f2 = w.dirty_free(p, 2);
+#pragma unroll
+    for (int g = 0; g < G; ++g) {
+      const bool fits = zero[g] | ((f0 >= rc[g]) & (f1 >= rm[g]) & (f2 >= re[g]));
+      dfit[g] |= fits ? 1u << p : 0u;
+    }
   }
   {
     constexpr int kPW = 64 / kNH;
@@ -1350,6 +1422,7 @@
         int kk[kPB];
         uint32_t fm[kPB];
         const uint64_t cyc_ld0 = PROF ? __builtin_amdgcn_s_memtime() : 0;
+        if (PROF && st.cyc_fh == 0) st.cyc_fh = cyc_ld0;
 #pragma unroll
         for (int h = 0; h < kPB; ++h) {
           kk[h] = b0 + kPW * h + sub;
@@ -1377,12 +1450,7 @@
           if (b0 + kPW * h >= lim) continue;
           uint64_t f = (wv && kk[h] < np) ? x[h][0] & x[h][1] & x[h][2] & x[h][3] : 0ull;
           if (dirty_head != 0) {
-            for (int p = 0; p < w.n_dirty; ++p) {
-              const int n = w.dirty_node[p];
-              if ((n >> 6) != wd) continue;
-              const uint64_t bit = 1ull << (n & 63);
-              f = (fm[h] >> p) & 1 ? (f | (x[h][0] & bit)) : (f & ~bit);
-            }
+            f = fix_dirty(w, f, x[h][0], wd, fm[h]);
             f = (wv && kk[h] < np) ? f : 0ull;
           }
           if (kk[h] < np) F[kk[h] * kNHS + wd] = f;
@@ -1424,6 +1492,7 @@
     cyc_t = t;
   }
 
+  if (k0_skip && wcur == 0) window_patch(w, 0, ncpu, nmem, neph, nport, nleft);
   int visits = 0, placements = 0, windows = wcur + 1;
   while (any != 0) {
     int mine = INT_MAX;
@@ -1453,7 +1522,7 @@
           while (pend != 0) {
             int js[Q];
             uint64_t a01[Q], a23[Q];
-            int64_t qr[Q][3];
+            uint32_t qf[Q];
             int op[Q][8];
             uint32_t nops[Q];
 #pragma unroll
@@ -1463,9 +1532,7 @@
               const int j = js[q] < 0 ? 0 : js[q];
               a01[q] = readlane64(r01[g], j);
               a23[q] = readlane64(r23[g], j);
-              qr[q][0] = static_cast<int64_t>(readlane64(static_cast<uint64_t>(rc[g]), j));
-              qr[q][1] = static_cast<int64_t>(readlane64(static_cast<uint64_t>(rm[g]), j));
-              qr[q][2] = static_cast<int64_t>(readlane64(static_cast<uint64_t>(re[g]), j));
+              qf[q] = static_cast<uint32_t>(__builtin_amdgcn_readlane(static_cast<int>(dfit[g]), j));
               nops[q] = 0;
               if constexpr (HO) {
 #pragma unroll
@@ -1491,7 +1558,7 @@
                 if constexpr (HO) {
 #pragma unroll
                   for (int u = 0; u < 8; ++u)
-                    x[q][u] = op[q][u] >= 0 ? w.atoms[static_cast<size_t>(op[q][u] >> 2) * Wp + wi] : 0ull;
+                    x[q][u] = op[q][u] >= 0 ? w.atoms()[static_cast<size_t>(op[q][u] >> 2) * Wp + wi] : 0ull;
                   x[q][8] = tab[static_cast<uint32_t>(a01[q] >> 32) + wi];
                   x[q][9] = tab[static_cast<uint32_t>(a23[q]) + wi];
                   x[q][10] = tab[static_cast<uint32_t>(a23[q] >> 32) + wi];
@@ -1521,8 +1588,7 @@
                   sw0 = x[q][0];
                   f = x[q][0] & x[q][1] & x[q][2] & x[q][3];
                 }
-                if (w.k0_skip)
-                  f = fix_dirty(w, f, sw0, word, qr[q][0], qr[q][1], qr[q][2], (qr[q][0] | qr[q][1] | qr[q][2]) == 0);
+                if (k0_skip) f = fix_dirty(w, f, sw0, word, qf[q]);
                 f = wv ? f : 0ull;
                 const uint64_t m = ballot(f != 0);
                 const int upto = m != 0 ? __builtin_ctzll(m) : 63;
@@ -1562,10 +1628,8 @@
           if (mine) {
             A->r01[slot] = r01[g];
             A->r23[slot] = r23[g];
-            A->rq[slot][0] = rc[g];
-            A->rq[slot][1] = rm[g];
-            A->rq[slot][2] = re[g];
-            if (w.s_head_only)
+            A->fm[slot] = dfit[g];
+            if (head_only)
 #pragma unroll
               for (int u = 0; u < 8; ++u) {
                 const int o = PG[(64 * g + lane) * 8 + u];
@@ -1580,7 +1644,7 @@
             A->sw = sw;
           }
           __syncthreads();
-          if (w.s_head_only) coop_scan<true>(w, *A, 0);
+          if (head_only) coop_scan<true>(w, *A, 0);
           else coop_scan<false>(w, *A, 0);
           __syncthreads();
           if (PROF) st.cyc_res += static_cast<uint64_t>((Wp - ((sw >> 6) << 6) + 64 * kCoopWaves - 1) /
@@ -1611,7 +1675,7 @@
             }
             ptr[g] = nx;
             unres[g] = false;
-            bytes = static_cast<uint32_t>(words) * (w.s_head_only ? 8u * (static_cast<uint32_t>(nops) + 3u) : 32u);
+            bytes = static_cast<uint32_t>(words) * (head_only ? 8u * (static_cast<uint32_t>(nops) + 3u) : 32u);
           }
           nbytes += static_cast<uint32_t>(wave_sum(static_cast<int>(bytes)));
           const uint64_t gone = ballot(mine && ptr[g] == INT_MAX);
@@ -1621,7 +1685,7 @@
       };
       constexpr int kResQ = 4;
       if constexpr (COOP) coop_resolve();
-      else if (w.s_head_only) resolve(std::integral_constant<int, 2>{}, std::true_type{});
+      else if (head_only) resolve(std::integral_constant<int, 2>{}, std::true_type{});
       else resolve(std::integral_constant<int, kResQ>{}, std::false_type{});
       if (PROF) st.cyc_res += __builtin_amdgcn_s_memtime() - cyc_r0;
       any = 0;
@@ -1636,13 +1700,13 @@
     const int W = n >> 6;
     if (W != wcur) {
       const uint64_t cyc_w0 = PROF ? __builtin_amdgcn_s_memtime() : 0;
-      const uint64_t* nr = w.node_rec + static_cast<size_t>(W * 64 + lane) * 8;
+      const uint64_t* nr = w.node_rec() + static_cast<size_t>(W * 64 + lane) * 8;
       ncpu = static_cast<int64_t>(nr[0]);
       nmem = static_cast<int64_t>(nr[1]);
       neph = static_cast<int64_t>(nr[2]);
       nport = nr[3];
       nleft = static_cast<int>(static_cast<int64_t>(nr[4]));
-      if (w.k0_skip) window_patch(w, W, lane, ncpu, nmem, neph, nport, nleft);
+      if (k0_skip) window_patch(w, W, ncpu, nmem, neph, nport, nleft);
       load_scal(W);
       wcur = W;
       ++windows;
@@ -1679,7 +1743,7 @@
         if (todo != 0) {
           const int kmax = dead - 64 * g;
 #define SR_PW(e_, o_)                                                                                             \
-  place_window<e_, o_>(todo, kmax, W, lane, rc[g], rm[g], re[g], pm[g], cur[g], zm[g], w.swap_mask, emask, ncpu, \
+  place_window<e_, o_>(todo, kmax, W, lane, rc[g], rm[g], re[g], pm[g], cur[g], zm[g], swap_mask, emask, ncpu, \
                        nmem, neph, nport, nleft, node[g])
 #define SR_PW32(e_, o_)                                                                                           \
   place_window32<e_, o_>(todo, kmax, W, lane, nc[g], nm[g], ne[g], pm[g], ps[g], cur[g], c32, m32, e32, \
@@ -1688,7 +1752,7 @@
   place_window32<e_, true, true>(todo, kmax, W, lane, nc[g], nm[g], ne[g], pm[g], ps[g], cur[g], c32, m32, e32, \
                                  nport, nleft, node[g])
 #define SR_PWX(e_, o_)                                                                                          \
-  place_window_x<e_, o_>(todo, kmax, W, lane, rc[g], rm[g], re[g], xv[g], pm[g], cur[g], zm[g], w.swap_mask, emask, \
+  place_window_x<e_, o_>(todo, kmax, W, lane, rc[g], rm[g], re[g], xv[g], pm[g], cur[g], zm[g], swap_mask, emask, \
                          ncpu, nmem, neph, nport, nleft, ns0, ns1, node[g])
 #define SR_PW32XT(e_, o_)                                                                                       \
   place_window32_x<e_, o_>(todo, kmax, W, lane, nc[g], nm[g], ne[g], nx[g], pm[g], ps[g], cur[g], c32, m32, e32, \
@@ -1743,12 +1807,12 @@
           const uint64_t rem = lw >= 63 ? 0ull : fmask[g] & (~0ull << (lw + 1));
           if (rem != 0) {
             const int w2 = fbase[g] + __builtin_ctzll(rem);
-            cur[g] = w.s_head_only ? f_word_prog(w, tab, PG + (64 * g + lane) * 8, r01[g], r23[g], w2)
-                                   : f_word_far(tab, r01[g], r23[g], w2);
-            if (w.k0_skip) {
-              const uint64_t sw0 = w.s_head_only ? f_word_prog_s(w, PG + (64 * g + lane) * 8, w2)
-                                                 : tab[static_cast<uint32_t>(r01[g]) + w2];
-              cur[g] = fix_dirty(w, cur[g], sw0, w2, rc[g], rm[g], re[g], zero[g]);
+            cur[g] = head_only ? f_word_prog(w, tab, PG + (64 * g + lane) * 8, r01[g], r23[g], w2)
+                               : f_word_far(tab, r01[g], r23[g], w2);
+            if (k0_skip) {
+              const uint64_t sw0 = head_only ? f_word_prog_s(w, PG + (64 * g + lane) * 8, w2)
+                                             : tab[static_cast<uint32_t>(r01[g]) + w2];
+              cur[g] = fix_dirty(w, cur[g], sw0, w2, dfit[g]);
             }
             nx = w2 * 64 + __builtin_ctzll(cur[g]);
             far_word = true;
@@ -1785,7 +1849,7 @@
   for (int g = 0; g < G; ++g) {
     const int k = 64 * g + lane;
     mapv[g] = k < dead ? node[g] : -1;
-    if (k < np) w.out_node[p0 + k] = mapv[g];
+    if (k < np) w.out_node()[p0 + k] = mapv[g];
   }
 }
 
@@ -2161,11 +2225,11 @@
   uint64_t t_start, c_start, t_list;
 };
 template <bool PROF>
-__device__ __forceinline__ K2Entry k2_entry(const DevWorkload& w, const int4* __restrict__ list, int li) {
+__device__ __forceinline__ K2Entry k2_entry(const K2W& w, const int4* __restrict__ list, int li) {
   K2Entry x;
   x.t_start = PROF ? __builtin_amdgcn_s_memrealtime() : 0;
-  x.c_start = PROF || w.out_cycles ? __builtin_amdgcn_s_memtime() : 0;
-  const int4 e = li < w.n_list_head ? w.list_head[li] : list[li];
+  x.c_start = __builtin_amdgcn_s_memtime();
+  const int4 e = li < w.n_list_head() ? w.k.list_head[li] : list[li];
   x.ci = __builtin_amdgcn_readfirstlane(e.x);
   x.p0 = __builtin_amdgcn_readfirstlane(e.y);
   x.np = __builtin_amdgcn_readfirstlane(e.z) - x.p0;
@@ -2190,72 +2254,82 @@
 }
 
 template <bool PROF>
-__device__ __forceinline__ void k2_finish(const DevWorkload& w, const K2Entry& x, int status, int wide,
+__device__ __forceinline__ void k2_finish(const K2W& w, const K2Entry& x, int status, int wide,
                                           uint32_t nbytes, const K2Stats& st, const int (&mapv)[kMapG],
                                           const bool in_regs = true, const int32_t* lmap = nullptr) {
+  const uint64_t cyc_fin = PROF ? __builtin_amdgcn_s_memtime() : 0;
   const int lane = threadIdx.x & 63;
   const int ci = x.ci, p0 = x.p0, np = x.np;
   int best = 0;
-  if (lane == 0 && ci == 0) k2_once(w);
+  unsigned long long* const dm = reinterpret_cast<unsigned long long*>(w.d_min());
+  uint64_t* const res_stat = w.res_stat();
+  if (lane == 0 && ci == 0) k2_once(w.k);
   if (lane == 0) {
-    w.out_status[ci] = status;
-    w.out_bytes[ci] = nbytes;
-    if (w.out_cycles)
-      w.out_cycles[ci] = static_cast<uint32_t>(min(__builtin_amdgcn_s_memtime() - x.c_start, 0xffffffffull));
+    uint32_t* const out_cycles = w.out_cycles();
+    w.out_status()[ci] = status;
+    w.out_bytes()[ci] = nbytes;
+    if (out_cycles) out_cycles[ci] = static_cast<uint32_t>(min(__builtin_amdgcn_s_memtime() - x.c_start, 0xffffffffull));
     if (status < 0) {
       const unsigned long long key = (static_cast<unsigned long long>(x.g) << 32) | static_cast<unsigned>(ci);
-      best = key < atomicMin(reinterpret_cast<unsigned long long*>(w.d_min), key);
-    }
-    if (PROF) {
-      uint64_t* pr = w.prof + static_cast<size_t>(ci) * 16;
-      pr[0] = x.t_start;
-      pr[1] = x.t_list;
-      pr[2] = __builtin_amdgcn_s_memrealtime();
-      pr[3] = __builtin_amdgcn_s_memtime() - x.c_start;
-      pr[4] = static_cast<uint64_t>(status >= 0 ? status + 1 : np);
-      pr[5] = static_cast<uint64_t>(wide);
-      pr[6] = st.n_spec_miss;
-      pr[7] = static_cast<uint64_t>(st.n_min) | (static_cast<uint64_t>(st.n_far) << 32);
-      pr[8] = st.cyc_a;
-      pr[9] = st.cyc_b;
-      pr[10] = st.cyc_c;
-      pr[11] = st.cyc_d;
-      if (wide == 2) {
-        pr[8] |= static_cast<uint64_t>(st.cyc_a_ld) << 32;
-        pr[10] |= static_cast<uint64_t>(st.n_res_pods) << 32 | static_cast<uint64_t>(st.n_res) << 48;
-        pr[11] |= static_cast<uint64_t>(st.cyc_res_ld) << 32;
-        pr[12] = st.cyc_res;
-        pr[13] = st.cyc_win;
-        pr[14] = st.cyc_rec - x.c_start;
-        pr[15] = st.narrow | (status < 0 ? 16u : 0u);
-      }
-    }
-  }
-  if (w.res_stat) {
-    const uint64_t tag = static_cast<uint64_t>(w.seq) << 32;
+      best = key < atomicMin(dm, key);
+    }
+  }
+  auto profile = [&]() {
+    const uint64_t cyc_end = __builtin_amdgcn_s_memtime();
+    uint64_t* pr = w.prof() + static_cast<size_t>(ci) * 16;
+    pr[0] = x.t_start;
+    pr[1] = x.t_list;
+    pr[2] = __builtin_amdgcn_s_memrealtime();
+    pr[3] = __builtin_amdgcn_s_memtime() - x.c_start;
+    pr[4] = static_cast<uint64_t>(status >= 0 ? status + 1 : np);
+    pr[5] = static_cast<uint64_t>(wide);
+    pr[6] = st.n_spec_miss;
+    pr[7] = static_cast<uint64_t>(st.n_min) | (static_cast<uint64_t>(st.n_far) << 32);
+    pr[8] = st.cyc_a;
+    pr[9] = st.cyc_b;
+    pr[10] = st.cyc_c;
+    pr[11] = st.cyc_d;
+    if (wide == 2) {
+      pr[8] |= static_cast<uint64_t>(st.cyc_a_ld) << 32;
+      pr[10] |= static_cast<uint64_t>(st.n_res_pods) << 32 | static_cast<uint64_t>(st.n_res) << 48;
+      pr[11] |= static_cast<uint64_t>(st.cyc_res_ld) << 32;
+      pr[12] = st.cyc_res;
+      pr[13] = st.cyc_win;
+      pr[14] = st.cyc_rec - x.c_start;
+      pr[15] = st.narrow | (status < 0 ? 16u : 0u);
+      pr[9] |= static_cast<uint64_t>(st.cyc_fh ? static_cast<uint32_t>(st.cyc_fh - st.cyc_rec) : 0u) << 32;
+      pr[13] |= static_cast<uint64_t>(static_cast<uint32_t>(cyc_end - cyc_fin)) << 32;
+    }
+  };
+  if (res_stat) {
+    const uint64_t tag = static_cast<uint64_t>(w.seq()) << 32;
+    uint64_t* const res_map = w.res_map();
+    const bool map_regs = w.k2_map_regs() != 0;
     if (__builtin_amdgcn_readfirstlane(best)) {
-      if (in_regs && w.k2_map_regs) {
+      if (in_regs && map_regs) {
 #pragma unroll
         for (int g = 0; g < kMapG; ++g)
           if (64 * g + lane < np)
-            __hip_atomic_store(w.res_map + p0 + 64 * g + lane, tag | static_cast<uint32_t>(mapv[g]), __ATOMIC_RELAXED,
+            __hip_atomic_store(res_map + p0 + 64 * g + lane, tag | static_cast<uint32_t>(mapv[g]), __ATOMIC_RELAXED,
                                __HIP_MEMORY_SCOPE_SYSTEM);
-      } else if (lmap && w.k2_map_regs) {
+      } else if (lmap && map_regs) {
         for (int q = lane; q < np; q += 64)
-          __hip_atomic_store(w.res_map + p0 + q, tag | static_cast<uint32_t>(lmap[q]), __ATOMIC_RELAXED,
+          __hip_atomic_store(res_map + p0 + q, tag | static_cast<uint32_t>(lmap[q]), __ATOMIC_RELAXED,
                              __HIP_MEMORY_SCOPE_SYSTEM);
       } else {
         __builtin_amdgcn_fence(__ATOMIC_RELEASE, "agent");
+        const int32_t* out_node = w.out_node();
         for (int q = lane; q < np; q += 64)
-          __hip_atomic_store(w.res_map + p0 + q,
-                             tag | static_cast<uint32_t>(__hip_atomic_load(w.out_node + p0 + q, __ATOMIC_RELAXED,
+          __hip_atomic_store(res_map + p0 + q,
+                             tag | static_cast<uint32_t>(__hip_atomic_load(out_node + p0 + q, __ATOMIC_RELAXED,
                                                                            __HIP_MEMORY_SCOPE_AGENT)),
                              __ATOMIC_RELAXED, __HIP_MEMORY_SCOPE_SYSTEM);
       }
     }
     if (lane == 0)
-      __hip_atomic_store(w.res_stat + ci, tag | (status < 0 ? 1u : 0u), __ATOMIC_RELAXED, __HIP_MEMORY_SCOPE_SYSTEM);
-  }
+      __hip_atomic_store(res_stat + ci, tag | (status < 0 ? 1u : 0u), __ATOMIC_RELAXED, __HIP_MEMORY_SCOPE_SYSTEM);
+  }
+  if (PROF && lane == 0) profile();
 }
 
 template <int CH, bool PROF>
@@ -2267,7 +2341,8 @@
   const int wave = threadIdx.x >> 6;
   const int li = __builtin_amdgcn_readfirstlane(static_cast<int>(blockIdx.x * (blockDim.x >> 6)) + wave);
   if (li >= n_list) return;
-  const K2Entry x = k2_entry<PROF>(w, list, li);
+  const K2W hw(w);
+  const K2Entry x = k2_entry<PROF>(hw, list, li);
   if (x.g <= w.cand_floor) {
     k2_skipped(w, x.ci);
     return;
@@ -2294,9 +2369,9 @@
   } else if (node_order && ebase >= 0) {
     uint64_t* F = reinterpret_cast<uint64_t*>(&L);
     wide = 2;
-    if (np <= 64) k2_node_order<1, PROF, false, true>(w, F, p0, np, status, st, nbytes, mapv, ebase);
-    else if (np <= 128) k2_node_order<2, PROF, false, true>(w, F, p0, np, status, st, nbytes, mapv, ebase);
-    else k2_node_order<4, PROF, false, true>(w, F, p0, np, status, st, nbytes, mapv, ebase);
+    if (np <= 64) k2_node_order<1, PROF, false, true>(hw, F, p0, np, status, st, nbytes, mapv, ebase);
+    else if (np <= 128) k2_node_order<2, PROF, false, true>(hw, F, p0, np, status, st, nbytes, mapv, ebase);
+    else k2_node_order<4, PROF, false, true>(hw, F, p0, np, status, st, nbytes, mapv, ebase);
     in_regs = true;
   } else if (ebase >= 0) {
     int placed = k2_run<1, CH, PROF, true>(w, L, p0, np, status, st, nbytes, ebase);
@@ -2307,9 +2382,9 @@
   } else if (node_order) {
     uint64_t* F = reinterpret_cast<uint64_t*>(&L);
     wide = 2;
-    if (np <= 64) k2_node_order<1, PROF>(w, F, p0, np, status, st, nbytes, mapv);
-    else if (np <= 128) k2_node_order<2, PROF>(w, F, p0, np, status, st, nbytes, mapv);
-    else k2_node_order<4, PROF>(w, F, p0, np, status, st, nbytes, mapv);
+    if (np <= 64) k2_node_order<1, PROF>(hw, F, p0, np, status, st, nbytes, mapv);
+    else if (np <= 128) k2_node_order<2, PROF>(hw, F, p0, np, status, st, nbytes, mapv);
+    else k2_node_order<4, PROF>(hw, F, p0, np, status, st, nbytes, mapv);
     in_regs = true;
   } else {
     int placed = k2_run<1, CH, PROF>(w, L, p0, np, status, st, nbytes);
@@ -2318,25 +2393,26 @@
     for (int i = lane; i < np; i += 64) w.out_node[p0 + i] = i < placed ? L.omap[i] : -1;
     in_lds = true;
   }
-  k2_finish<PROF>(w, x, status, wide, nbytes, st, mapv, in_regs, in_lds ? L.omap : nullptr);
+  k2_finish<PROF>(hw, x, status, wide, nbytes, st, mapv, in_regs, in_lds ? L.omap : nullptr);
 }
 
 template <int GMAX, bool PROF, bool WIDE = false, bool XT = false>
 __global__ __launch_bounds__(256) void k2_node(DevWorkload w_arg, const int4* __restrict__ list, int n_list) {
-  const DevWorkload& w = *(const DevWorkload*)__builtin_amdgcn_kernarg_segment_ptr();
+  const DevWorkload& wk = *(const DevWorkload*)__builtin_amdgcn_kernarg_segment_ptr();
   (void)w_arg;
+  const K2W w(wk);
   extern __shared__ __attribute__((aligned(16))) uint64_t k2_lds[];
   const int wave = threadIdx.x >> 6;
-  const size_t region = 64 * GMAX * kNHS + (w.s_head_only ? 64 * GMAX * 4 : 0);
-  const int nco = XT ? 0 : w.n_coop;
+  const size_t region = 64 * GMAX * kNHS + (w.s_head_only() ? 64 * GMAX * 4 : 0);
+  const int nco = XT ? 0 : w.n_coop();
   if constexpr (!XT) {
     static_assert(sizeof(CoopArea) <= (kCoopWaves - 1) * 64 * kNHS * 8, "the cooperative area fits the helpers' LDS");
     if (static_cast<int>(blockIdx.x) < nco) {
-      if (w.cand_floor >= 0) {
+      if (w.cand_floor() >= 0) {
         const int bi = static_cast<int>(blockIdx.x);
-        const int4 e = bi < w.n_list_head ? w.list_head[bi] : list[bi];
-        if (__builtin_amdgcn_readfirstlane(e.w) <= w.cand_floor) {
-          if (wave == 0) k2_skipped(w, __builtin_amdgcn_readfirstlane(e.x));
+        const int4 e = bi < w.n_list_head() ? wk.list_head[bi] : list[bi];
+        if (__builtin_amdgcn_readfirstlane(e.w) <= w.cand_floor()) {
+          if (wave == 0) k2_skipped(wk, __builtin_amdgcn_readfirstlane(e.x));
           return;
         }
       }
@@ -2366,10 +2442,10 @@
   const int li = __builtin_amdgcn_readfirstlane(nco + static_cast<int>((blockIdx.x - nco) * (blockDim.x >> 6)) + wave);
   if (li >= n_list) return;
   int4 xe = {-1, -1, -1, 0};
-  if (XT) xe = w.list_ext[li];
+  if (XT) xe = wk.list_ext[li];
   const K2Entry x = k2_entry<PROF>(w, list, li);
-  if (x.g <= w.cand_floor) {
-    k2_skipped(w, x.ci);
+  if (x.g <= w.cand_floor()) {
+    k2_skipped(wk, x.ci);
     return;
   }
   uint64_t* F = k2_lds + static_cast<size_t>(wave) * region;
diff --git a/k8s-spot-rescheduler_amd/csrc/kernels.hpp b/k8s-spot-rescheduler_amd/csrc/kernels.hpp
--- a/k8s-spot-rescheduler_amd/csrc/kernels.hpp
+++ b/k8s-spot-rescheduler_amd/csrc/kernels.hpp
@@ -2,6 +2,7 @@
 
 #include <hip/hip_runtime.h>
 
+#include <cstddef>
 #include <cstdint>
 
 #include "launch_shape.hpp"
@@ -20,20 +21,48 @@
 constexpr int64_t kTPad = INT64_MAX - 1;
 constexpr int kDevDynTerms = 4;
 constexpr int kDevExtU64 = 8;
+constexpr int kHdrWords = 64;
 constexpr int kListInline = 128;
 
 struct DevWorkload {
-  int32_t n_spot, n_pad, Wp;
-  const int64_t* node_free;
+  int32_t Wp;
+  int32_t k0_skip;
+  const uint64_t* pod_rec;
   const uint64_t* node_rec;
+  uint64_t* S;
+  uint64_t* T;
   const uint64_t* node_patch;
   int32_t n_node_patch;
+  int32_t n_dirty;
+  uint64_t swap_mask;
+  uint32_t s_empty_off;
+  int32_t s_head_only;
+  const uint64_t* atoms;
+  const int32_t* cls_prog8;
+  int32_t k2_narrow;
+  int32_t k2_excl;
+  int32_t n_pad;
+  int32_t k2_map_regs;
+  const uint64_t* pod_ext;
+  const int64_t* node_scal;
+  int32_t* out_node;
+  int32_t* out_status;
+  uint32_t* out_bytes;
+  uint32_t* out_cycles;
+  int32_t* d_min;
+  uint64_t* res_stat;
+  uint64_t* res_map;
+  uint64_t* prof;
+  uint32_t seq;
+  int32_t n_coop;
+  int32_t cand_floor;
+  int32_t n_list_head;
+  int32_t hdr_pad[kHdrWords - 50];
+  int64_t dirty_tab[64];
+  int32_t n_spot;
+  const int64_t* node_free;
   const uint64_t* pod_patch;
   int32_t n_pod_patch;
-  int32_t k0_skip;
-  int32_t n_dirty;
-  int32_t dirty_node[16];
-  int64_t dirty_free[16][3];
   int32_t* d_min_next;
   int32_t first_fallback_local;
   int32_t k0_inc;
@@ -41,18 +70,13 @@
   const int32_t* k0_cols;
   const int32_t* k0_rows;
   int32_t n_atoms;
-  const uint64_t* atoms;
   const int32_t* cls_prog_off;
   const int32_t* cls_prog;
-  const int32_t* cls_prog8;
   int32_t n_classes;
-  uint32_t s_empty_off;
   int32_t n_t;
   int32_t t_off[5];
   const int64_t* t_thr;
   int32_t n_pods;
-  uint64_t swap_mask;
-  const uint64_t* pod_rec;
   int32_t n_cand;
   const int32_t* cand_off;
   const int32_t* cand_global;
@@ -60,7 +84,6 @@
   int32_t n_list;
   int32_t max_np;
   int32_t k2_node_kernel;
-  int32_t s_head_only;
   const int32_t* dyn_cand;
   const uint64_t* dyn_pod;
   int32_t n_dk;
@@ -69,32 +92,15 @@
   const int32_t* sp_tab;
   const int32_t* ds_info;
   const int32_t* ext_cand;
-  const uint64_t* pod_ext;
-  const int64_t* node_scal;
   const int4* list_ext;
-  uint64_t* S;
-  uint64_t* T;
-  int32_t* out_node;
-  int32_t* out_status;
-  uint32_t* out_bytes;
-  uint32_t* out_cycles;
-  int32_t* d_min;
   uint64_t rank_next;
   uint64_t* result;
-  uint64_t* res_stat;
-  uint64_t* res_map;
-  uint32_t seq;
-  int32_t k2_narrow;
   int32_t k2_wpb;
-  int32_t k2_excl;
-  int32_t k2_map_regs;
-  int32_t n_coop;
-  int32_t cand_floor;
   int32_t k2_mode;
-  uint64_t* prof;
-  int32_t n_list_head;
   int4 list_head[kListInline];
 };
+static_assert(offsetof(DevWorkload, dirty_tab) == 4 * kHdrWords, "the wave header is kHdrWords words, the changed-node table follows");
+static_assert(sizeof(DevWorkload) <= 4096, "kernel arguments");
 
 hipError_t launch_tables(const DevWorkload& w, int32_t local_first_fallback, hipStream_t s,
                          hipEvent_t ev0 = nullptr, hipEvent_t ev1 = nullptr);
diff --git a/k8s-spot-rescheduler_amd/csrc/planner.cpp b/k8s-spot-rescheduler_amd/csrc/planner.cpp
--- a/k8s-spot-rescheduler_amd/csrc/planner.cpp
+++ b/k8s-spot-rescheduler_amd/csrc/planner.cpp
@@ -586,10 +586,16 @@
   d.k0_skip = p.skip ? 1 : 0;
   d.n_dirty = p.n_dirty;
   for (int32_t i = 0; i < p.n_dirty; ++i) {
-    d.dirty_node[i] = p.dirty_node[i];
-    for (int dm = 0; dm < 3; ++dm) d.dirty_free[i][dm] = p.dirty_free[i][dm];
-  }
-  static_assert(sizeof(d.dirty_node) / sizeof(d.dirty_node[0]) == sr::kSkipDirty, "kSkipDirty nodes in the kernel arguments");
+    for (int dm = 0; dm < 3; ++dm) d.dirty_tab[16 * dm + i] = p.dirty_free[i][dm];
+    const uint64_t* rec = tl.node_patch.data() + static_cast<size_t>(i) * sr::kNodePatchWords;
+    if (p.n_node_patch != p.n_dirty || rec[0] != static_cast<uint64_t>(p.dirty_node[i])) {
+      ctx->err = "K0-less run: the node patches are not the changed nodes";
+      return SR_ERR_STATE;
+    }
+    d.dirty_tab[48 + i] = static_cast<int64_t>(static_cast<uint64_t>(static_cast<uint32_t>(p.dirty_node[i])) |
+                                                 static_cast<uint64_t>(static_cast<uint32_t>(rec[5])) << 32);
+  }
+  static_assert(sr::kSkipDirty == 16 && sizeof(d.dirty_tab) == 64 * 8, "kSkipDirty nodes x 4 entries in the kernel arguments");
   d.first_fallback_local = w.first_fallback;
   static_assert(sr::kPodPatchU64 == sr::kPodPatchWords && sr::kNodePatchU64 == sr::kNodePatchWords &&
                     sr::kTPad == sr::kTSpare,
```

Result: faster. 362.0 billion, median of 6 (+11.1%).
